# 2noise/ChatTTS

Measured on NVIDIA H100. Metric: speech-tokens/sec (GPT decode loop, 4-codebook tokens; RTF = wall / audio seconds @ 24 kHz), higher is better.
Workload: dtype f32

## Files before the change

chattts_b200/_lib.py:

```python
from __future__ import annotations

import ctypes as C
import os
import threading

from . import build as _build

_lock = threading.Lock()
_lib = None


class GptConfig(C.Structure):
    _fields_ = [(n, C.c_int32) for n in (
        "hidden_size", "intermediate_size", "num_layers", "num_heads", "num_kv_heads", "head_dim", "num_vq",
        "num_audio_tokens", "num_text_tokens", "max_positions")] + [
        ("rms_eps", C.c_float), ("max_batch", C.c_int32), ("max_context", C.c_int32)]


class GptLayout(C.Structure):
    _fields_ = [(n, C.c_int64) for n in (
        "layer0", "layer_stride", "wqkv", "wo", "wgate_up", "wdown", "ln1", "ln2", "final_norm", "head_code",
        "head_text", "emb_code", "emb_text", "rope_cos", "rope_sin", "total")]


class SamplerConfig(C.Structure):
    _fields_ = [
        ("temperature", C.c_float * 8), ("top_p", C.c_float), ("top_k", C.c_int32),
        ("min_tokens_to_keep", C.c_int32), ("penalty_on", C.c_int32), ("penalty_lut", C.c_float * 32),
        ("past_window", C.c_int32), ("penalty_max_ids", C.c_int32), ("greedy", C.c_int32),
        ("eos_token", C.c_int32), ("min_new_token", C.c_int32), ("top_p_removed_max", C.c_float),
        ("has_removed_max", C.c_int32), ("philox_seed", C.c_uint64)]


class GptStatus(C.Structure):
    _fields_ = [("steps_done", C.c_int32), ("all_finished", C.c_int32),
                ("any_finished_first_step", C.c_int32), ("reserved", C.c_int32)]


ENGINE_FP16_WEIGHTS, ENGINE_FP16_KV = 1, 2


def engine_flags(dtype) -> int:
    import torch

    if dtype is None or dtype == torch.float32:
        return 0
    if dtype == torch.float16:
        return ENGINE_FP16_WEIGHTS | ENGINE_FP16_KV
    raise ValueError(f"slot engine dtype must be torch.float32 or torch.float16, not {dtype!r}")


PREFILL_CHUNK_ALIGN = 128


SLOT_IDLE, SLOT_RUNNING, SLOT_FINISHED = 0, 1, 2

ERR_POOL = -5
PAGE_TOKENS = 16


class SlotImage(C.Structure):
    _fields_ = [("magic", C.c_uint32)] + [(n, C.c_int32) for n in (
        "prec", "seq_len", "pos", "end_idx", "finish", "n_gen", "npages", "page_bytes", "num_vq", "hidden_size",
        "noise_floats", "has_hidden")] + [
        ("row", C.c_int32 * 8), ("reserved", C.c_int32 * 3), ("sampler", SamplerConfig)] + [
        (n, C.c_uint64) for n in ("off_noise", "off_ids", "off_hiddens", "off_kv", "bytes")]


class ConvStackConfig(C.Structure):
    _fields_ = [(n, C.c_int32) for n in (
        "idim", "odim", "hidden", "n_layer", "bn_dim", "kernel", "dilation", "out_dim", "vq_dim", "vq_groups",
        "vq_residual", "vq_levels")]


class VocosConfig(C.Structure):
    _fields_ = [(n, C.c_int32) for n in ("input_channels", "dim", "intermediate_dim", "num_layers", "n_fft",
                                         "hop_length")]


EXPORTS = (
    "ctb_abi_version", "ctb_last_error", "ctb_launch_count", "ctb_gpt_layout_query", "ctb_gpt_create",
    "ctb_gpt_destroy", "ctb_gpt_begin", "ctb_gpt_decode", "ctb_gpt_status_query", "ctb_gpt_profile_kernel", "ctb_gpt_debug_trace", "ctb_gpt_embed_prompt", "ctb_sample",
    "ctb_gpt_engine_begin", "ctb_gpt_engine_admit", "ctb_gpt_engine_admit_text", "ctb_gpt_engine_status",
    "ctb_gpt_engine_cancel", "ctb_gpt_engine_begin_ex", "ctb_gpt_engine_prefill_chunk",
    "ctb_gpt_engine_begin_paged", "ctb_gpt_engine_reserve", "ctb_gpt_engine_release", "ctb_gpt_engine_suspend_bytes",
    "ctb_gpt_engine_suspend", "ctb_gpt_engine_resume", "ctb_gpt_engine_share_prompt",
    "ctb_dvae_blob_floats", "ctb_vocos_blob_floats", "ctb_decoder_create", "ctb_decoder_destroy",
    "ctb_dvae_decode", "ctb_vocos_decode", "ctb_decode_rows",
    "ctb_dvae_encoder_blob_floats", "ctb_dvae_encoder_create", "ctb_dvae_encoder_destroy", "ctb_dvae_encode",
    "ctb_dvae_encode_rows",
)


class CtbError(RuntimeError):
    pass


def lib_path() -> str:
    return _build.LIB_PATH


def load(build_if_missing: bool = True):
    global _lib
    with _lock:
        if _lib is not None:
            return _lib
        path = lib_path()
        if build_if_missing:
            try:
                _build.build()
            except Exception:
                if not os.path.exists(path):
                    raise
        if not os.path.exists(path):
            raise CtbError(f"{path} missing: run `python -m chattts_b200.build`")
        lib = C.CDLL(path)
        vp, i32, i64 = C.c_void_p, C.c_int32, C.c_int64
        lib.ctb_abi_version.restype = C.c_int
        lib.ctb_last_error.restype = C.c_char_p
        lib.ctb_launch_count.restype = C.c_uint64
        lib.ctb_gpt_layout_query.argtypes = [C.POINTER(GptConfig), C.POINTER(GptLayout)]
        lib.ctb_gpt_create.argtypes = [C.POINTER(GptConfig), vp, C.POINTER(vp)]
        lib.ctb_gpt_destroy.argtypes = [vp]
        lib.ctb_gpt_begin.argtypes = [vp, i32, i32, vp, vp, C.POINTER(SamplerConfig), vp, i32, i32, vp, vp, vp]
        lib.ctb_gpt_decode.argtypes = [vp, i32, vp]
        lib.ctb_gpt_status_query.argtypes = [vp, C.POINTER(GptStatus), vp, vp, vp]
        lib.ctb_gpt_profile_kernel.argtypes = [vp, i32, vp]
        lib.ctb_gpt_debug_trace.argtypes = [vp, vp, i32]
        lib.ctb_gpt_embed_prompt.argtypes = [vp, vp, vp, i32, i32, vp, vp]
        lib.ctb_gpt_engine_begin.argtypes = [vp, i32, i32, vp, vp, vp]
        lib.ctb_gpt_engine_begin_ex.argtypes = [vp, i32, i32, i32, vp, vp, vp]
        lib.ctb_gpt_engine_admit.argtypes = [vp, i32, vp, i32, vp, vp, C.POINTER(SamplerConfig), vp, vp, vp]
        lib.ctb_gpt_engine_admit_text.argtypes = lib.ctb_gpt_engine_admit.argtypes
        lib.ctb_gpt_engine_status.argtypes = [vp, C.POINTER(GptStatus), vp, vp, vp, vp]
        lib.ctb_gpt_engine_cancel.argtypes = [vp, i32, vp, vp]
        lib.ctb_gpt_engine_prefill_chunk.argtypes = [vp, i32, i32, i32, i32, vp, i32, C.POINTER(SamplerConfig), vp, i32,
                                                     vp]
        lib.ctb_gpt_engine_begin_paged.argtypes = [vp, i32, i32, i32, i32, vp, vp, vp]
        lib.ctb_gpt_engine_reserve.argtypes = [vp, i32, vp, vp, vp]
        lib.ctb_gpt_engine_release.argtypes = [vp, i32, vp, vp]
        lib.ctb_gpt_engine_suspend_bytes.argtypes = [vp, i32, C.POINTER(C.c_uint64), vp]
        lib.ctb_gpt_engine_suspend.argtypes = [vp, i32, vp, C.c_uint64, vp]
        lib.ctb_gpt_engine_resume.argtypes = [vp, i32, vp, C.c_uint64, vp]
        lib.ctb_gpt_engine_share_prompt.argtypes = [vp, i32, i32, i32, i32, vp]
        lib.ctb_sample.argtypes = [vp, i32, i32, i32, C.POINTER(SamplerConfig), vp, vp, i32, i32, i32, vp, vp]
        lib.ctb_dvae_blob_floats.argtypes = [C.POINTER(ConvStackConfig)]
        lib.ctb_dvae_blob_floats.restype = i64
        lib.ctb_vocos_blob_floats.argtypes = [C.POINTER(VocosConfig)]
        lib.ctb_vocos_blob_floats.restype = i64
        lib.ctb_decoder_create.argtypes = [C.POINTER(ConvStackConfig), vp, C.POINTER(VocosConfig), vp, i32, i32,
                                           C.POINTER(vp)]
        lib.ctb_decoder_destroy.argtypes = [vp]
        lib.ctb_dvae_decode.argtypes = [vp, vp, i32, i32, i32, vp, vp]
        lib.ctb_vocos_decode.argtypes = [vp, vp, i32, i32, vp, vp]
        lib.ctb_decode_rows.argtypes = [vp, i32, i32, C.POINTER(vp), C.POINTER(i32), vp, i64, vp]
        lib.ctb_dvae_encoder_blob_floats.argtypes = [C.POINTER(ConvStackConfig)]
        lib.ctb_dvae_encoder_blob_floats.restype = i64
        lib.ctb_dvae_encoder_create.argtypes = [C.POINTER(ConvStackConfig), vp, i64, C.POINTER(vp)]
        lib.ctb_dvae_encoder_destroy.argtypes = [vp]
        lib.ctb_dvae_encode.argtypes = [vp, vp, i64, vp, i32, C.POINTER(i32), vp, vp, vp]
        lib.ctb_dvae_encode_rows.argtypes = [vp, i32, C.POINTER(vp), C.POINTER(i64), vp, i32, C.POINTER(i32), vp, vp]
        if lib.ctb_abi_version() != 3:
            raise CtbError("ABI version mismatch")
        _lib = lib
        return lib


def check(rc: int) -> None:
    if rc != 0:
        raise CtbError(f"chattts_b200 error {rc}: {load().ctb_last_error().decode()}")


def require_cuda():
    import torch

    if not torch.cuda.is_available():
        raise CtbError("chattts_b200 needs a CUDA device (sm_90a); there is no CPU path")
```

chattts_b200/csrc/flow.cuh:

```cuda
#pragma once
#include "gpt_kernels.cuh"
#include "tc_common.cuh"

namespace ctb {

constexpr int FL_THREADS = 256;
constexpr int FL_LAUNCH_THREADS = FL_THREADS;
constexpr int FL_WARPS = 8;
constexpr int FL_SLOTS = 4;
constexpr int FL_SLOT_BYTES = 6144;
constexpr int FL_SLOT_FLOATS = FL_SLOT_BYTES / 4;
constexpr int FL_RING_BYTES = FL_WARPS * FL_SLOTS * FL_SLOT_BYTES;
constexpr int FL_SMAX = 6;
constexpr int FL_CH = 64;
constexpr int FL_PW = 66;
constexpr int FL_BMAX = 4;
constexpr int FL_ROWS = 6;
constexpr int FL_GU = 3;
constexpr int FL_QR = 2;
constexpr int FL_HEADS = 12;
constexpr int FL_RMAX = 16;

constexpr int FL_A_X = 0;
constexpr int FL_A_XO = FL_A_X + FL_BMAX * KC;
constexpr int FL_A_ACT = FL_A_XO + FL_BMAX * KC;
constexpr int FL_A_P = FL_A_ACT + FL_BMAX * 4 * KC;
constexpr int FL_A_END = FL_A_P + FL_BMAX * FL_HEADS * FL_SMAX * FL_PW;
constexpr int FL_REP_STRIDE = ((FL_A_END + 1023) / 1024) * 1024;
constexpr int FL_A_Q = 0, FL_A_KN = FL_BMAX * KC, FL_A_VN = 2 * FL_BMAX * KC;
constexpr int FL_QKV_WORDS = 3 * FL_BMAX * KC;
constexpr int FL_SROWS = 16, FL_VPAD = 1024;
constexpr int FL_A_LOGITS = FL_QKV_WORDS, FL_A_IDX = FL_A_LOGITS + FL_SROWS * FL_VPAD;
constexpr int FL_TAIL_WORDS = FL_A_IDX + 64;
constexpr size_t FL_PARITY_WORDS = (size_t)FL_RMAX * FL_REP_STRIDE + FL_TAIL_WORDS;
constexpr size_t FL_ARENA_WORDS = 2 * FL_PARITY_WORDS;
constexpr unsigned FL_EPOCH_STEP = 256;
constexpr int FL_TR_EV = 4096, FL_TR_EVN = 32, FL_TR_WORDS = FL_TR_EV + 192 * FL_TR_EVN;

enum FlowTagKind { FT_X = 0, FT_QKV = 1, FT_P = 2, FT_XO = 3, FT_ACT = 4, FT_LOGITS = 5, FT_IDX = 6 };
enum FlowStage { FS_Q0 = 0, FS_Q1 = 1, FS_KV = 2, FS_O = 3, FS_GU0 = 4, FS_GU1 = 5, FS_GU2 = 6, FS_D0 = 7, FS_D1 = 8, FS_NLAYER = 9 };

__device__ __forceinline__ void fl_bar() { asm volatile("bar.sync 1, 256;" ::: "memory"); }

struct FlowP {
  const float* W;
  int64_t layer0, layer_stride, o_wqkv, o_wo, o_wgu, o_wd, o_ln1, o_ln2, o_final_norm, o_head, o_emb_code, o_emb_text,
      o_cos, o_sin;
  int L, I, Hq, hd;
  float eps, scaling;
  float *logits, *kv;
  size_t kv_layer_floats;
  const int* block_table; int pages_per_row;
  int* seq_len;
  LoopState* st;
  int decode, col, T0, sample;
  const float* emb; const uint8_t* mask; const int32_t* ids_out;
  int max_new, num_vq, num_audio, infer_text, B;
  float* hidden_out; int hidden_stride, rows_per_item, V;
  unsigned long long* arena;
  unsigned* epoch;
  int R;
  int l2_ahead;
  unsigned long long* trace;
  int nsteps;
  int ink;
  ctb_sampler_config samp;
  const float* q_noise;
  uint8_t* finish;
  int* end_idx;
  int32_t* ids_w;
};

__device__ __forceinline__ void ll_st(unsigned long long* p, float v, uint32_t tag) {
  const unsigned long long x = ((unsigned long long)tag << 32) | (unsigned long long)__float_as_uint(v);
  asm volatile("st.relaxed.gpu.global.u64 [%0], %1;" ::"l"(p), "l"(x) : "memory");
}
__device__ __forceinline__ unsigned long long ll_ld(const unsigned long long* p) {
  unsigned long long x;
  asm volatile("ld.global.cg.u64 %0, [%1];" : "=l"(x) : "l"(p) : "memory");
  return x;
}
__device__ __forceinline__ void ll_ld2(const unsigned long long* p, unsigned long long& a, unsigned long long& b) {
  asm volatile("ld.global.cg.v2.u64 {%0,%1}, [%2];" : "=l"(a), "=l"(b) : "l"(p) : "memory");
}
__device__ __forceinline__ uint32_t ll_tag(unsigned long long x) { return (uint32_t)(x >> 32); }
__device__ __forceinline__ float ll_val(unsigned long long x) { return __uint_as_float((uint32_t)x); }

struct FlowWd {
  int* err;
  int dead;
  int spins;
};
__device__ __forceinline__ bool fl_giveup(FlowWd& wd, int code) {
  if (wd.dead) return true;
  if (++wd.spins < (1 << 20)) {
    if ((wd.spins & 8191) == 0 && __ldcg(wd.err) != 0) { wd.dead = 1; return true; }
    return false;
  }
  atomicCAS(wd.err, 0, code);
  wd.dead = 1;
  return true;
}

__device__ __forceinline__ void fl_bulk(uint32_t dst, const void* src, uint32_t bytes, uint32_t bar, uint64_t pol) {
  asm volatile(
      "cp.async.bulk.shared::cluster.global.mbarrier::complete_tx::bytes.L2::cache_hint [%0], [%1], %2, [%3], %4;" ::"r"(dst),
      "l"(src), "r"(bytes), "r"(bar), "l"(pol)
      : "memory");
}
__device__ __forceinline__ bool fl_elect() {
  uint32_t pred;
  asm volatile("{\n\t.reg .pred p;\n\telect.sync _|p, 0xffffffff;\n\tselp.u32 %0, 1, 0, p;\n\t}" : "=r"(pred));
  return pred != 0;
}
__device__ __forceinline__ void fl_expect(uint32_t bar, uint32_t bytes) {
  asm volatile("mbarrier.arrive.expect_tx.shared::cta.b64 _, [%0], %1;" ::"r"(bar), "r"(bytes) : "memory");
}
__device__ __forceinline__ bool fl_try_wait(uint32_t bar, uint32_t parity) {
  uint32_t ok;
  asm volatile("{\n\t.reg .pred p;\n\tmbarrier.try_wait.parity.shared::cta.b64 p, [%1], %2;\n\tselp.u32 %0, 1, 0, p;\n\t}"
               : "=r"(ok) : "r"(bar), "r"(parity) : "memory");
  return ok != 0;
}

struct FlowGeo {
  int G, NW, gw, cta, warp, lane;
  int S;
  int u_on, u_b, u_h, u_split, u_n, u_nchunk;
  int nheads_tasks;
};

__device__ __forceinline__ bool fl_q_valid(const FlowGeo& g, int j) { return g.gw + j * g.NW < 3 * KC / 2; }
__device__ __forceinline__ bool fl_kv_more(const FlowGeo& g, int sub, int& chunk) {
  chunk = g.u_split + sub * g.S;
  return g.u_on && chunk < g.u_nchunk;
}
__device__ __forceinline__ bool fl_kv_valid(const FlowGeo& g, int chunk) { return FL_CH * chunk + 8 * g.warp < g.u_n; }
__device__ __forceinline__ bool fl_o_valid(const FlowGeo& g) { return g.warp < FL_ROWS && g.cta + g.G * g.warp < KC; }
__device__ __forceinline__ bool fl_gu_valid(const FlowGeo& g, int j, int I) { return g.gw + j * g.NW < I; }
__device__ __forceinline__ int fl_d_rows(const FlowGeo& g, int j0, int j1) {
  int n = 0;
  for (int j = j0; j < j1; ++j) n += (g.cta + g.G * j < KC);
  return n;
}
__device__ __forceinline__ bool fl_h_valid(const FlowGeo& g, int j) { return g.gw + j * g.NW < g.nheads_tasks; }

__device__ __forceinline__ void fl_qkv_rows(const FlowP& p, int task, int& r0, int& r1) {
  const int half = p.hd / 2, nq = p.Hq * half;
  int t = task, base = 0;
  if (t >= 2 * nq) { t -= 2 * nq; base = 2 * p.Hq * p.hd; }
  else if (t >= nq) { t -= nq; base = p.Hq * p.hd; }
  r0 = base + (t / half) * p.hd + (t % half);
  r1 = r0 + half;
}

constexpr int FL_TMAX = 40;
struct FlowIss {
  int l, k, n, ntab, hsub;
};

__device__ __noinline__ int fl_build_table(const FlowP& p, const FlowGeo* gs, int4* tab) {
  FlowGeo g = *gs;
  g.warp = threadIdx.x >> 5; g.lane = threadIdx.x & 31; g.gw = g.cta * FL_WARPS + g.warp;
  int n = 0;
  auto put = [&](int64_t off0, int64_t stride, int bytes, int ncopy, int kind) {
    if (g.lane == 0 && n < FL_TMAX) tab[n] = make_int4((int)off0, (int)stride, bytes | (ncopy << 16) | (kind << 20), 0);
    n++;
  };
  for (int j = 0; j < FL_QR; ++j)
    if (fl_q_valid(g, j)) {
      int r0, r1;
      fl_qkv_rows(p, g.gw + j * g.NW, r0, r1);
      put(p.o_wqkv + (int64_t)r0 * KC, (int64_t)(r1 - r0) * KC, KC * 4, 2, 0);
    }
  for (int sub = 0;; ++sub) {
    int chunk;
    if (!fl_kv_more(g, sub, chunk)) break;
    if (!fl_kv_valid(g, chunk)) continue;
    const int t0 = FL_CH * chunk + 8 * g.warp;
    const int page = __ldg(p.block_table + g.u_b * p.pages_per_row + t0 / kPageTokens);
    const int64_t k0 = (int64_t)kv_off(page, 0, g.u_h, t0 % kPageTokens, p.Hq, p.hd);
    const int64_t v0 = (int64_t)kv_off(page, 1, g.u_h, t0 % kPageTokens, p.Hq, p.hd);
    put(k0, v0 - k0, 8 * 64 * 4, 2, 1);
  }
  if (fl_o_valid(g)) put(p.o_wo + (int64_t)(g.cta + g.G * g.warp) * KC, 0, KC * 4, 1, 0);
  for (int j = 0; j < FL_GU; ++j)
    if (fl_gu_valid(g, j, p.I)) put(p.o_wgu + (int64_t)(g.gw + j * g.NW) * KC, (int64_t)p.I * KC, KC * 4, 2, 0);
  for (int half = 0; half < 2; ++half) {
    const int j0 = half ? 4 : 0, j1 = half ? FL_ROWS : 4;
    const int nr = fl_d_rows(g, j0, j1);
    if (nr > 0)
      put(p.o_wd + (int64_t)(g.cta + g.G * j0) * p.I + g.warp * (p.I / FL_WARPS), (int64_t)g.G * p.I, (p.I / FL_WARPS) * 4, nr, 0);
  }
  return n;
}

__device__ __forceinline__ void fl_issue_heads(const FlowP& p, const FlowGeo* gs, int w, int hsub, uint32_t dst, uint32_t bar, uint64_t pol_w) {
  const int gw = gs->cta * FL_WARPS + w;
  const int t = gw + hsub * gs->NW, nrows = p.rows_per_item * p.V;
  if (fl_elect()) {
    fl_expect(bar, 2u * KC * 4u);
    fl_bulk(dst, p.W + p.o_head + (size_t)(2 * t) * KC, KC * 4, bar, pol_w);
    fl_bulk(dst + KC * 4, p.W + p.o_head + (size_t)min(2 * t + 1, nrows - 1) * KC, KC * 4, bar, pol_w);
  }
}

__device__ __forceinline__ bool fl_issue(const FlowP& p, const FlowGeo* gs, const int4* tab, FlowIss& it, int w, uint32_t ring,
                                         uint32_t bars, uint64_t pol_w, uint64_t pol_kv) {
  const int slot = it.n % FL_SLOTS;
  const uint32_t bar = bars + slot * 8, dst = ring + slot * FL_SLOT_BYTES;
  if (it.l < p.L) {
    const int4 e = tab[it.k];
    if (fl_elect()) {
      const int bytes = e.z & 0xffff, ncopy = (e.z >> 16) & 0xf, kind = e.z >> 20;
      const float* src = (kind ? p.kv + (size_t)it.l * p.kv_layer_floats : p.W + p.layer0 + (int64_t)it.l * p.layer_stride) + e.x;
      fl_expect(bar, (uint32_t)(bytes * ncopy));
#pragma unroll
      for (int k = 0; k < 4; ++k)
        if (k < ncopy) fl_bulk(dst + k * bytes, src + (int64_t)k * e.y, (uint32_t)bytes, bar, kind ? pol_kv : pol_w);
      if (p.l2_ahead && kind == 0) {
        const float* nsrc = it.l + 1 < p.L ? src + p.layer_stride : src - (int64_t)(p.L - 1) * p.layer_stride;
#pragma unroll
        for (int k = 0; k < 4; ++k)
          if (k < ncopy)
            asm volatile("cp.async.bulk.prefetch.L2.global [%0], %1;" ::"l"(nsrc + (int64_t)k * e.y), "r"((uint32_t)bytes) : "memory");
      }
    }
    if (++it.k == it.ntab) { it.k = 0; it.l++; }
    it.n++;
    return true;
  }
  if (gs->cta * FL_WARPS + w + it.hsub * gs->NW < gs->nheads_tasks) {
    fl_issue_heads(p, gs, w, it.hsub, dst, bar, pol_w);
    it.hsub++;
    it.n++;
    return true;
  }
  return false;
}

struct FlowW {
  float* base;
  uint32_t ring;
  uint32_t bars;
  int n;
  int owed;
  FlowIss it;
  const int4* tab;
  const FlowGeo* gs;
  uint64_t pol_w, pol_kv;
};
__device__ __forceinline__ void fl_refill(const FlowP& p, FlowW& w) {
  if (w.owed > 0) {
    __syncwarp();
    fl_issue(p, w.gs, w.tab, w.it, (int)(threadIdx.x >> 5), w.ring, w.bars, w.pol_w, w.pol_kv);
    w.owed--;
  }
}
__device__ __forceinline__ const float* fl_ring_slot_at(const FlowW& w, int k) { return w.base + ((w.n + k) % FL_SLOTS) * FL_SLOT_FLOATS; }
__device__ __forceinline__ bool fl_ring_peek_n(const FlowP& p, FlowW& w, int cnt) {
  while (w.owed > FL_SLOTS - cnt) fl_refill(p, w);
  bool ok = true;
#pragma unroll
  for (int k = 0; k < 3; ++k)
    if (k < cnt) { const int n = w.n + k; ok = fl_try_wait(w.bars + (n % FL_SLOTS) * 8, (uint32_t)(n / FL_SLOTS) & 1u) && ok; }
  return ok;
}
__device__ __forceinline__ void fl_ring_wait_n(const FlowP& p, FlowW& w, int cnt, FlowWd& wd) {
  while (w.owed > FL_SLOTS - cnt) fl_refill(p, w);
  uint32_t bar[3], par[3];
#pragma unroll
  for (int k = 0; k < 3; ++k) {
    const int n = w.n + k;
    bar[k] = w.bars + (n % FL_SLOTS) * 8;
    par[k] = (uint32_t)(n / FL_SLOTS) & 1u;
  }
  wd.spins = 0;
  while (true) {
    bool ok[3];
#pragma unroll
    for (int k = 0; k < 3; ++k) ok[k] = k < cnt ? fl_try_wait(bar[k], par[k]) : true;
    if (ok[0] && ok[1] && ok[2]) break;
    if (__any_sync(0xffffffffu, fl_giveup(wd, 0x120))) { wd.dead = 1; break; }
  }
}
__device__ __forceinline__ const float* fl_ring_wait(const FlowP& p, FlowW& w, FlowWd& wd) {
  fl_ring_wait_n(p, w, 1, wd);
  return fl_ring_slot_at(w, 0);
}
__device__ __forceinline__ void fl_ring_release(const FlowP& p, FlowW& w) { w.n++; w.owed++; fl_refill(p, w); }
__device__ __forceinline__ void fl_refill_all(const FlowP& p, FlowW& w) {
  while (w.owed > 0) fl_refill(p, w);
}

template <int BT>
__device__ __forceinline__ void fl_stage768(const FlowP& p, const unsigned long long* src, uint32_t tag, float* xs, FlowWd& wd, FlowW& fw) {
  const int tid = threadIdx.x;
  unsigned long long v[BT][3];
  wd.spins = 0;
  while (true) {
    bool ok = true;
#pragma unroll
    for (int b = 0; b < BT; ++b)
      if (b < p.B) {
#pragma unroll
        for (int k = 0; k < 3; ++k) v[b][k] = ll_ld(src + b * KC + tid + 256 * k);
      }
#pragma unroll
    for (int b = 0; b < BT; ++b)
      if (b < p.B) {
#pragma unroll
        for (int k = 0; k < 3; ++k) ok = ok && (ll_tag(v[b][k]) == tag);
      }
    if (__all_sync(0xffffffffu, ok)) break;
    if (__any_sync(0xffffffffu, fl_giveup(wd, 0x200 + (tag & 0xff)))) { wd.dead = 1; break; }
  }
#pragma unroll
  for (int b = 0; b < BT; ++b) {
#pragma unroll
    for (int k = 0; k < 3; ++k) xs[b * KC + tid + 256 * k] = b < p.B ? ll_val(v[b][k]) : 0.f;
  }
  fl_bar();
}

template <int BT>
__device__ __forceinline__ void fl_stage_attn(const FlowP& p, const unsigned long long* P, uint32_t tag, float* xs, FlowWd& wd, int S,
                                              const int* s_pos, const int* s_active) {
  const int tid = threadIdx.x, lane = tid & 31, warp = tid >> 5;
  const int pk = lane / FL_SMAX, ps = lane % FL_SMAX, pbase = min(pk, 2) * FL_SMAX;
#pragma unroll 1
  for (int b = 0; b < BT; ++b) {
    if (b >= p.B) break;
    float v[3] = {0.f, 0.f, 0.f};
    if (s_active[b]) {
      const int ns = min((s_pos[b] + FL_CH) / FL_CH, S);
      const unsigned long long* Pb = P + (size_t)b * FL_HEADS * FL_SMAX * FL_PW + (size_t)(warp >> 1) * FL_SMAX * FL_PW;
      const bool pl = pk < 3 && ps < ns;
      float m = -INFINITY, lv = 0.f;
      wd.spins = 0;
      while (true) {
        bool ok = true;
        if (pl) {
          unsigned long long w1, w2;
          ll_ld2(Pb + (size_t)(4 * pk * FL_SMAX + ps) * FL_PW + 64, w1, w2);
          ok = ll_tag(w1) == tag && ll_tag(w2) == tag;
          m = ll_val(w1); lv = ll_val(w2);
        }
        if (__all_sync(0xffffffffu, ok)) break;
        if (__any_sync(0xffffffffu, fl_giveup(wd, 0x400))) { wd.dead = 1; break; }
      }
      float GM = -INFINITY;
#pragma unroll
      for (int s = 0; s < FL_SMAX; ++s) {
        const float ms = __shfl_sync(0xffffffffu, m, pbase + s);
        if (s < ns) GM = fmaxf(GM, ms);
      }
      const float wgt = pl ? expf(m - GM) : 0.f;
      unsigned long long w[3][FL_SMAX];
      while (true) {
        bool ok = true;
#pragma unroll
        for (int k = 0; k < 3; ++k)
#pragma unroll
          for (int s = 0; s < FL_SMAX; ++s)
            if (s < ns) w[k][s] = ll_ld(Pb + (size_t)(4 * k * FL_SMAX + s) * FL_PW + (tid & 63));
#pragma unroll
        for (int k = 0; k < 3; ++k)
#pragma unroll
          for (int s = 0; s < FL_SMAX; ++s)
            if (s < ns) ok = ok && ll_tag(w[k][s]) == tag;
        if (__all_sync(0xffffffffu, ok)) break;
        if (__any_sync(0xffffffffu, fl_giveup(wd, 0x401))) { wd.dead = 1; break; }
      }
#pragma unroll
      for (int k = 0; k < 3; ++k) {
        float GL = 0.f, GO = 0.f;
#pragma unroll
        for (int s = 0; s < FL_SMAX; ++s) {
          const float ws = __shfl_sync(0xffffffffu, wgt, k * FL_SMAX + s);
          const float ls = __shfl_sync(0xffffffffu, lv, k * FL_SMAX + s);
          if (s < ns) {
            GL = fmaf(ws, ls, GL);
            GO = fmaf(ws, ll_val(w[k][s]), GO);
          }
        }
        v[k] = GO / GL;
      }
    }
#pragma unroll
    for (int k = 0; k < 3; ++k) xs[b * KC + tid + 256 * k] = v[k];
  }
#pragma unroll
  for (int b = 0; b < BT; ++b)
    if (b >= p.B)
      for (int k = 0; k < 3; ++k) xs[b * KC + tid + 256 * k] = 0.f;
  fl_bar();
}

template <int BT>
__device__ __forceinline__ void fl_load_x(const float* xs, float (&x)[BT][24], int lane) {
#pragma unroll
  for (int b = 0; b < BT; ++b) {
#pragma unroll
    for (int i = 0; i < 6; ++i) {
      const float4 v = reinterpret_cast<const float4*>(xs)[b * (KC / 4) + i * 32 + lane];
      x[b][4 * i] = v.x; x[b][4 * i + 1] = v.y; x[b][4 * i + 2] = v.z; x[b][4 * i + 3] = v.w;
    }
  }
}

template <int BT>
__device__ __forceinline__ void fl_norm(float (&x)[BT][24], const float4 (&nw)[6], float eps) {
#pragma unroll
  for (int b = 0; b < BT; ++b) {
    float s4[4] = {0.f, 0.f, 0.f, 0.f};
#pragma unroll
    for (int j = 0; j < 24; ++j) s4[j & 3] = fmaf(x[b][j], x[b][j], s4[j & 3]);
    float ss = warp_sum((s4[0] + s4[1]) + (s4[2] + s4[3]));
    const float rinv = __fdiv_rn(1.0f, __fsqrt_rn(__fadd_rn(__fdiv_rn(ss, (float)KC), eps)));
#pragma unroll
    for (int i = 0; i < 6; ++i) {
      x[b][4 * i] = __fmul_rn(nw[i].x, __fmul_rn(x[b][4 * i], rinv));
      x[b][4 * i + 1] = __fmul_rn(nw[i].y, __fmul_rn(x[b][4 * i + 1], rinv));
      x[b][4 * i + 2] = __fmul_rn(nw[i].z, __fmul_rn(x[b][4 * i + 2], rinv));
      x[b][4 * i + 3] = __fmul_rn(nw[i].w, __fmul_rn(x[b][4 * i + 3], rinv));
    }
  }
}
__device__ __forceinline__ void fl_nw_fetch(float* dst, const float* src, uint64_t* bar, uint64_t pol) {
  if (threadIdx.x == 0) {
    fl_expect(smem_u32(bar), KC * 4);
    fl_bulk(smem_u32(dst), src, KC * 4, smem_u32(bar), pol);
  }
}
__device__ __forceinline__ void fl_nw_wait(uint64_t* bar, int& count, FlowWd& wd) {
  const uint32_t b = smem_u32(bar), parity = (uint32_t)count & 1u;
  wd.spins = 0;
  while (!fl_try_wait(b, parity))
    if (__any_sync(0xffffffffu, fl_giveup(wd, 0x800))) { wd.dead = 1; break; }
  count++;
}
__device__ __forceinline__ void fl_load_nw_s(const float* s_nw, float4 (&nw)[6], int lane) {
#pragma unroll
  for (int i = 0; i < 6; ++i) nw[i] = reinterpret_cast<const float4*>(s_nw)[i * 32 + lane];
}
__device__ __forceinline__ void fl_load_nw(const float* normw, float4 (&nw)[6], int lane) {
#pragma unroll
  for (int i = 0; i < 6; ++i) nw[i] = ldg_stream(reinterpret_cast<const float4*>(normw) + i * 32 + lane);
}

template <int BT>
__device__ __forceinline__ void fl_dot2(const float* slot, const float (&x)[BT][24], float (&a0)[BT], float (&a1)[BT], int lane) {
  const float4* w0 = reinterpret_cast<const float4*>(slot) + lane;
  const float4* w1 = w0 + KC / 4;
#pragma unroll
  for (int b = 0; b < BT; ++b) { a0[b] = 0.f; a1[b] = 0.f; }
#pragma unroll
  for (int i = 0; i < 6; ++i) {
    const float4 u = w0[i * 32], v = w1[i * 32];
#pragma unroll
    for (int b = 0; b < BT; ++b) {
      a0[b] = fmaf(u.x, x[b][4 * i], a0[b]); a0[b] = fmaf(u.y, x[b][4 * i + 1], a0[b]);
      a0[b] = fmaf(u.z, x[b][4 * i + 2], a0[b]); a0[b] = fmaf(u.w, x[b][4 * i + 3], a0[b]);
      a1[b] = fmaf(v.x, x[b][4 * i], a1[b]); a1[b] = fmaf(v.y, x[b][4 * i + 1], a1[b]);
      a1[b] = fmaf(v.z, x[b][4 * i + 2], a1[b]); a1[b] = fmaf(v.w, x[b][4 * i + 3], a1[b]);
    }
  }
}
template <int BT>
__device__ __forceinline__ void fl_dot1(const float* slot, const float (&x)[BT][24], float (&a0)[BT], int lane) {
  const float4* w0 = reinterpret_cast<const float4*>(slot) + lane;
#pragma unroll
  for (int b = 0; b < BT; ++b) a0[b] = 0.f;
#pragma unroll
  for (int i = 0; i < 6; ++i) {
    const float4 u = w0[i * 32];
#pragma unroll
    for (int b = 0; b < BT; ++b) {
      a0[b] = fmaf(u.x, x[b][4 * i], a0[b]); a0[b] = fmaf(u.y, x[b][4 * i + 1], a0[b]);
      a0[b] = fmaf(u.z, x[b][4 * i + 2], a0[b]); a0[b] = fmaf(u.w, x[b][4 * i + 3], a0[b]);
    }
  }
}

template <int BT>
__device__ __forceinline__ void fl_bcast_store(unsigned long long* rep0, int R, size_t idx, float v, uint32_t tag, int nb, int lane) {
  constexpr int LPB = 32 / BT;
  const float vb = __shfl_sync(0xffffffffu, v, (lane / LPB) * LPB);
  if (lane / LPB < nb)
    for (int r = lane % LPB; r < R; r += LPB) ll_st(rep0 + (size_t)r * FL_REP_STRIDE + idx, vb, tag);
}

struct __align__(16) FlowSamp {
  float x[FL_VPAD];
  uint32_t key[2][1024];
  double redd[32];
  double pre[32];
  int redi[8];
  float redf[8];
  float bv[8];
  int bi[8];
  int win[32];
  uint32_t thr;
  int out;
};
__device__ __forceinline__ double fl_vsum_d(const double (&v)[4], double* redd) {
  const int lane = threadIdx.x & 31, warp = threadIdx.x >> 5;
  double r[4];
#pragma unroll
  for (int k = 0; k < 4; ++k) r[k] = warp_sum_d(v[k]);
  fl_bar();
  if (lane == 0) {
#pragma unroll
    for (int k = 0; k < 4; ++k) redd[warp + 8 * k] = r[k];
  }
  fl_bar();
  double t = 0.0;
#pragma unroll 8
  for (int w = 0; w < 32; ++w) t += redd[w];
  return t;
}
__device__ __forceinline__ float fl_bmax(float v, float* redf) {
  const int lane = threadIdx.x & 31, warp = threadIdx.x >> 5;
  v = warp_max(v);
  fl_bar();
  if (lane == 0) redf[warp] = v;
  fl_bar();
  float t = -INFINITY;
#pragma unroll
  for (int w = 0; w < FL_WARPS; ++w) t = fmaxf(t, redf[w]);
  return t;
}
__device__ __forceinline__ int fl_bsum_i(int v, int* redi) {
  const int lane = threadIdx.x & 31, warp = threadIdx.x >> 5;
  v = __reduce_add_sync(0xffffffffu, v);
  fl_bar();
  if (lane == 0) redi[warp] = v;
  fl_bar();
  int t = 0;
#pragma unroll
  for (int w = 0; w < FL_WARPS; ++w) t += redi[w];
  return t;
}
__device__ __forceinline__ void fl_cx(uint32_t& a, uint32_t& b, bool up) {
  const uint32_t lo = min(a, b), hi = max(a, b);
  a = up ? lo : hi; b = up ? hi : lo;
}
__device__ __forceinline__ void fl_bitonic1024(uint32_t (&key)[4], uint32_t* buf0, uint32_t* buf1) {
  const int tid = threadIdx.x;
  int sb = 0;
#pragma unroll 1
  for (int k = 2; k <= 1024; k <<= 1) {
#pragma unroll 1
    for (int j = k >> 1; j > 0; j >>= 1) {
      if (j == 1) {
        fl_cx(key[0], key[1], ((4 * tid) & k) == 0);
        fl_cx(key[2], key[3], ((4 * tid + 2) & k) == 0);
      } else if (j == 2) {
        fl_cx(key[0], key[2], ((4 * tid) & k) == 0);
        fl_cx(key[1], key[3], ((4 * tid + 1) & k) == 0);
      } else {
        const int d = j >> 2;
        uint32_t other[4];
        if (d >= 32) {
          uint32_t* buf = sb ? buf1 : buf0;
          *reinterpret_cast<uint4*>(buf + 4 * tid) = make_uint4(key[0], key[1], key[2], key[3]);
          fl_bar();
          const uint4 o = *reinterpret_cast<const uint4*>(buf + 4 * (tid ^ d));
          other[0] = o.x; other[1] = o.y; other[2] = o.z; other[3] = o.w;
          sb ^= 1;
        } else {
#pragma unroll
          for (int e = 0; e < 4; ++e) other[e] = __shfl_xor_sync(0xffffffffu, key[e], d);
        }
        const bool up = ((4 * tid) & k) == 0, lower = (tid & d) == 0;
#pragma unroll
        for (int e = 0; e < 4; ++e) key[e] = (lower == up) ? min(key[e], other[e]) : max(key[e], other[e]);
      }
    }
  }
}

__device__ __noinline__ int fl_sample_row(const ctb_sampler_config& c, const float* q_noise, FlowSamp& sm, int V, int row, int qi,
                                          int nwin, int step, unsigned long long* dbg) {
  int dk = 0;
#define FL_SK() do { if (dbg && threadIdx.x == 0) dbg[dk++] = (unsigned long long)clock64(); } while (0)
  FL_SK();
  const int tid = threadIdx.x, lane = tid & 31, warp = tid >> 5;
  const bool pen = c.penalty_on && row < c.penalty_max_ids;
  const float temp = c.temperature[qi];
  float qn[4];
#pragma unroll
  for (int k = 0; k < 4; ++k) {
    const int v = tid + 256 * k;
    qn[k] = (q_noise != nullptr && v < V) ? __ldg(q_noise + (size_t)row * V + v) : 1.f;
  }
  {
    float xr[4];
    int cnt[4] = {0, 0, 0, 0};
#pragma unroll
    for (int k = 0; k < 4; ++k) { const int v = tid + 256 * k; xr[k] = v < V ? __fdiv_rn(sm.x[v], temp) : 0.f; }
    if (pen) {
#pragma unroll 4
      for (int w = 0; w < nwin; ++w) {
        const int id = sm.win[w];
#pragma unroll
        for (int k = 0; k < 4; ++k) cnt[k] += (id == tid + 256 * k);
      }
    }
    fl_bar();
#pragma unroll
    for (int k = 0; k < 4; ++k) {
      const int v = tid + 256 * k;
      if (v < V) {
        float x = xr[k];
        if (pen) { const float a = c.penalty_lut[cnt[k]]; x = (x < 0.f) ? __fmul_rn(x, a) : __fdiv_rn(x, a); }
        sm.x[v] = x;
      }
    }
  }
  fl_bar();
  float mx = -INFINITY;
  for (int v = tid; v < V; v += FL_THREADS) mx = fmaxf(mx, sm.x[v]);
  mx = fl_bmax(mx, sm.redf);
  FL_SK();

  const bool use_p = c.top_p >= 0.f;
  const int kk = c.top_k > 0 ? min(max(c.top_k, c.min_tokens_to_keep), V) : 0;
  const int min_keep = min(c.min_tokens_to_keep, V);
  uint32_t thr_key = 0;
  if (!c.greedy && (use_p || kk > 0)) {
    double den = 0.0;
    if (use_p) {
      double dv[4];
#pragma unroll
      for (int k = 0; k < 4; ++k) { const int vt = tid + 256 * k; dv[k] = vt < V ? (double)expf(sm.x[vt] - mx) : 0.0; }
      den = fl_vsum_d(dv, sm.redd);
    }
    FL_SK();
    const float denf = (float)den;
    const float pthr = c.has_removed_max ? c.top_p_removed_max : (float)(1.0 - (double)c.top_p);
    uint32_t key[4];
#pragma unroll
    for (int k = 0; k < 4; ++k) { const int vt = tid + 256 * k; key[k] = vt < V ? float_key(sm.x[vt]) : 0u; }
    fl_bitonic1024(key, sm.key[0], sm.key[1]);
    FL_SK();
    fl_bar();
    uint32_t* skey = sm.key[0];
    *reinterpret_cast<uint4*>(skey + 4 * tid) = make_uint4(key[0], key[1], key[2], key[3]);
    fl_bar();
#pragma unroll
    for (int k = 0; k < 4; ++k) key[k] = skey[tid + 256 * k];
    uint32_t t_p = 0;
    if (use_p) {
      double inc[4];
#pragma unroll
      for (int k = 0; k < 4; ++k) {
        const uint32_t ky = key[k];
        double a = ky ? (double)__fdiv_rn(expf(key_float(ky) - mx), denf) : 0.0;
#pragma unroll
        for (int o = 1; o < 32; o <<= 1) {
          const double n = __shfl_up_sync(0xffffffffu, a, o);
          if (lane >= o) a += n;
        }
        inc[k] = a;
      }
      fl_bar();
      if (lane == 31) {
#pragma unroll
        for (int k = 0; k < 4; ++k) sm.redd[warp + 8 * k] = inc[k];
      }
      fl_bar();
      if (tid == 0) {
        double run = 0.0;
        for (int w = 0; w < 32; ++w) { const double t = sm.redd[w]; sm.pre[w] = run; run += t; }
      }
      fl_bar();
      int removed = 0;
#pragma unroll
      for (int k = 0; k < 4; ++k) {
        const int vw = warp + 8 * k, vt = tid + 256 * k;
        const double base = sm.pre[vw];
        const float cum = (float)(base + inc[k]);
        removed += ((cum <= pthr) && (vt < 1024 - min_keep)) ? 1 : 0;
      }
      const int nrem = fl_bsum_i(removed, sm.redi);
      t_p = skey[nrem];
      FL_SK();
    }
    const uint32_t t_k = kk > 0 ? skey[1024 - kk] : 0u;
    thr_key = max(t_p, t_k);
  }
  if (c.greedy) {
    float gm = -INFINITY;
    for (int v = tid; v < V; v += FL_THREADS)
      if (!(c.greedy == 2 && v == c.eos_token)) gm = fmaxf(gm, sm.x[v]);
    gm = fl_bmax(gm, sm.redf);
    thr_key = float_key(gm);
  }
  fl_bar();
  const bool ban = step < c.min_new_token;
  float mx2 = -INFINITY;
  for (int v = tid; v < V; v += FL_THREADS) {
    float x = sm.x[v];
    if (float_key(x) < thr_key || ((ban || c.greedy == 2) && v == c.eos_token)) x = -INFINITY;
    sm.x[v] = x;
    mx2 = fmaxf(mx2, x);
  }
  mx2 = fl_bmax(mx2, sm.redf);
  double dv2[4];
#pragma unroll
  for (int k = 0; k < 4; ++k) { const int vt = tid + 256 * k; dv2[k] = vt < V ? (double)expf(sm.x[vt] - mx2) : 0.0; }
  const float den2f = (float)fl_vsum_d(dv2, sm.redd);
  FL_SK();
  float best = -1.f;
  int besti = 0x7fffffff;
#pragma unroll
  for (int k = 0; k < 4; ++k) {
    const int v = tid + 256 * k;
    if (v < V) {
      const float pr = __fdiv_rn(expf(sm.x[v] - mx2), den2f);
      const float qv = q_noise ? qn[k] : philox_exp1(c.philox_seed, (uint32_t)row, (uint32_t)v, (uint32_t)step);
      const float r = __fdiv_rn(pr, qv);
      if (r > best) { best = r; besti = v; }
    }
  }
  for (int o = 16; o > 0; o >>= 1) {
    const float ob = __shfl_xor_sync(0xffffffffu, best, o);
    const int oi = __shfl_xor_sync(0xffffffffu, besti, o);
    if (ob > best || (ob == best && oi < besti)) { best = ob; besti = oi; }
  }
  fl_bar();
  if (lane == 0) { sm.bv[warp] = best; sm.bi[warp] = besti; }
  fl_bar();
  if (tid == 0) {
    for (int w = 1; w < FL_WARPS; ++w)
      if (sm.bv[w] > best || (sm.bv[w] == best && sm.bi[w] < besti)) { best = sm.bv[w]; besti = sm.bi[w]; }
    sm.out = besti < V ? besti : 0;
  }
  fl_bar();
  FL_SK();
#undef FL_SK
  return sm.out;
}

template <int BT>
__global__ void __launch_bounds__(FL_THREADS, 1) k_flow(const __grid_constant__ FlowP p) {
  extern __shared__ __align__(128) unsigned char fl_smem[];
  float* xs = reinterpret_cast<float*>(fl_smem + FL_RING_BYTES);
  __shared__ __align__(8) uint64_t s_bar[FL_WARPS * FL_SLOTS];
  __shared__ __align__(8) uint64_t s_nwbar[2];
  __shared__ int s_pos[BT], s_active[BT], s_page[BT];
  __shared__ float s_cos[BT * 64], s_sin[BT * 64];
  __shared__ float s_red[FL_ROWS][FL_WARPS][BT];
  __shared__ float s_resd[FL_ROWS * BT];
  __shared__ float s_am[FL_WARPS], s_al[FL_WARPS];
  __shared__ __align__(16) float s_ao[FL_WARPS][64];
  __shared__ FlowGeo s_geo;
  __shared__ __align__(16) float s_nw1[KC], s_nw2[KC];
  __shared__ int4 s_tab[FL_WARPS][FL_TMAX];
  __shared__ FlowSamp s_samp_store[BT <= 2 ? 1 : 0 + (BT > 2)];
  FlowSamp& s_samp = s_samp_store[0];

  const int tid = threadIdx.x, lane = tid & 31, warp = tid >> 5;
  constexpr int LPB = 32 / BT;
  if (tid < FL_WARPS * FL_SLOTS) mbar_init(&s_bar[tid], 1);
  if (tid < 2) mbar_init(&s_nwbar[tid], 1);
  asm volatile("fence.mbarrier_init.release.cluster;" ::: "memory");
  __syncthreads();
  pdl_trigger();
  pdl_wait();
  if (p.decode && ldg_cg(&p.st->all_finished)) return;

  constexpr bool INK = BT <= 2;
  __shared__ int s_ids[BT * 8];
  __shared__ int s_fin[BT], s_end[BT];
  __shared__ int s_allfin;
  FlowWd wd{&p.st->err, 0, 0};
  uint32_t base = (uint32_t)ldg_cg(reinterpret_cast<const int*>(p.epoch));
  int tr = 0;
#define FL_TRACE() do { if (p.trace && blockIdx.x == 0 && tid == 0 && tr < 250) p.trace[tr++] = globaltimer_ns(); } while (0)
#define FL_EV(k) do { if (p.trace && l == 10 && tid == 0) p.trace[FL_TR_EV + blockIdx.x * FL_TR_EVN + (k)] = globaltimer_ns(); } while (0)
#define FL_CK(k) do { if (p.trace && l == 10 && tid == 0 && blockIdx.x == 0) p.trace[3000 + (k)] = (unsigned long long)clock64(); } while (0)

  int ngen = p.decode ? ldg_cg(&p.st->n_gen) : 0;
  int lstep = p.decode ? ldg_cg(&p.st->step) : 0;
  if (tid < BT) {
    int act = 0, pos = 0;
    if (tid < p.B) {
      pos = ldg_cg(&p.seq_len[tid]);
      act = p.decode ? 1 : (p.mask[(size_t)tid * p.T0 + p.col] != 0);
    }
    s_pos[tid] = pos; s_active[tid] = act;
    s_fin[tid] = (tid < p.B && p.ink) ? (int)p.finish[tid] : 0;
    s_end[tid] = (tid < p.B && p.ink) ? ldg_cg(&p.end_idx[tid]) : 0;
  }
  const bool ink = INK && p.ink != 0;
  const int nrows_s = p.B * p.rows_per_item;
  const int R = p.R;
  uint64_t pol_w, pol_kv;
  asm volatile("createpolicy.fractional.L2::evict_first.b64 %0, 1.0;" : "=l"(pol_w));
  asm volatile("createpolicy.fractional.L2::evict_normal.b64 %0, 1.0;" : "=l"(pol_kv));
  int nw1_cnt = 0, nw2_cnt = 0;
  FlowW fw;
  fw.base = reinterpret_cast<float*>(fl_smem) + (size_t)warp * FL_SLOTS * FL_SLOT_FLOATS;
  fw.ring = smem_u32(fw.base);
  fw.bars = smem_u32(&s_bar[warp * FL_SLOTS]);
  fw.n = 0; fw.owed = 0;
  fw.it = FlowIss{0, 0, 0, 0, 0};
  fw.tab = s_tab[warp]; fw.gs = &s_geo; fw.pol_w = pol_w; fw.pol_kv = pol_kv;
  FlowGeo g;
  g.G = gridDim.x; g.NW = g.G * FL_WARPS; g.cta = blockIdx.x; g.warp = warp; g.lane = lane; g.gw = g.cta * FL_WARPS + warp;
  g.S = max(1, min(FL_SMAX, g.G / (p.Hq * p.B)));
  g.nheads_tasks = p.sample ? (p.rows_per_item * p.V + 1) / 2 : 0;
  const int myrep = g.cta % R;
  const int o_row = g.cta + g.G * warp;
  unsigned long long* tailw = p.arena + (size_t)FL_RMAX * FL_REP_STRIDE;
  fl_bar();

  int nwin = 0;
  if constexpr (INK) {
    if (ink && g.cta < nrows_s) {
      const int item = g.cta / p.rows_per_item, qi = g.cta % p.rows_per_item;
      const bool pen = p.samp.penalty_on && g.cta < p.samp.penalty_max_ids;
      nwin = pen ? min(ngen, p.samp.past_window) : 0;
      if (tid < nwin) s_samp.win[tid] = ldg_cg(&p.ids_out[((size_t)item * p.max_new + (ngen - nwin + tid)) * p.num_vq + qi]);
    }
  }

#define FL_PREP_STEP()                                                                                                  \
  do {                                                                                                                  \
    if (tid < BT) s_page[tid] = tid < p.B ? __ldg(p.block_table + tid * p.pages_per_row + s_pos[tid] / kPageTokens) : 0; \
    {                                                                                                                   \
      const int u = g.cta;                                                                                              \
      g.u_on = 0; g.u_b = 0; g.u_h = 0; g.u_split = 0; g.u_n = 0; g.u_nchunk = 0;                                       \
      if (u < p.B * p.Hq * g.S) {                                                                                       \
        g.u_split = u % g.S; g.u_h = (u / g.S) % p.Hq; g.u_b = u / (g.S * p.Hq);                                        \
        g.u_n = s_pos[g.u_b] + 1;                                                                                       \
        g.u_nchunk = (g.u_n + FL_CH - 1) / FL_CH;                                                                       \
        g.u_on = s_active[g.u_b] && g.u_split < min(g.u_nchunk, g.S);                                                   \
      }                                                                                                                 \
    }                                                                                                                   \
    if (tid == 0) s_geo = g;                                                                                            \
    fl_bar();                                                                                                           \
    fw.it.l = 0; fw.it.k = 0; fw.it.hsub = 0; fw.owed = 0;                                                              \
    fw.it.ntab = fl_build_table(p, &s_geo, s_tab[warp]);                                                                \
    __syncwarp();                                                                                                       \
    for (int k_ = 0; k_ < FL_SLOTS; ++k_) fl_issue(p, fw.gs, fw.tab, fw.it, warp, fw.ring, fw.bars, pol_w, pol_kv);     \
    for (int i = tid; i < BT * 64; i += FL_THREADS) {                                                                   \
      const int b = i / 64;                                                                                             \
      s_cos[i] = b < p.B ? __ldg(p.W + p.o_cos + (size_t)s_pos[b] * 64 + (i % 64)) : 0.f;                               \
      s_sin[i] = b < p.B ? __ldg(p.W + p.o_sin + (size_t)s_pos[b] * 64 + (i % 64)) : 0.f;                               \
    }                                                                                                                   \
  } while (0)

  FL_PREP_STEP();
  FL_TRACE();
#pragma unroll 1
  for (int sidx = 0;; ++sidx) {
  FL_TRACE();
  fl_nw_fetch(s_nw1, p.W + p.layer0 + p.o_ln1, &s_nwbar[0], pol_w);
  fl_nw_fetch(s_nw2, p.W + p.layer0 + p.o_ln2, &s_nwbar[1], pol_w);
  {
    float ev[BT * 3][8];
#pragma unroll
    for (int it_ = 0; it_ < BT * 3; ++it_) {
      const int i = tid + it_ * FL_THREADS, b = i / KC, k = i % KC;
#pragma unroll
      for (int q = 0; q < 8; ++q) ev[it_][q] = 0.f;
      if (b < p.B) {
        if (!p.decode) {
          ev[it_][0] = s_active[b] ? p.emb[((size_t)b * p.T0 + p.col) * KC + k] : 0.f;
        } else if (p.infer_text) {
          const int id0 = ldg_cg(p.ids_out + ((size_t)b * p.max_new + (ngen - 1)) * p.num_vq);
          ev[it_][0] = p.W[p.o_emb_text + (size_t)id0 * KC + k];
        } else {
#pragma unroll
          for (int q = 0; q < 8; ++q)
            if (q < p.num_vq) {
              const int id = sidx > 0 ? s_ids[b * 8 + q] : ldg_cg(p.ids_out + ((size_t)b * p.max_new + (ngen - 1)) * p.num_vq + q);
              ev[it_][q] = p.W[p.o_emb_code + ((size_t)q * p.num_audio + id) * KC + k];
            }
        }
      }
    }
#pragma unroll
    for (int it_ = 0; it_ < BT * 3; ++it_) {
      float v = 0.f;
#pragma unroll
      for (int q = 0; q < 8; ++q) v += ev[it_][q];
      xs[tid + it_ * FL_THREADS] = v;
    }
  }
  fl_bar();
  FL_TRACE();

  for (int l = 0; l < p.L; ++l) {
    const float* Wl = p.W + p.layer0 + (int64_t)l * p.layer_stride;
    unsigned long long* par = p.arena + (size_t)(l & 1) * FL_PARITY_WORDS;
    unsigned long long* parn = p.arena + (size_t)((l + 1) & 1) * FL_PARITY_WORDS;
    unsigned long long* qkvw = par + (size_t)FL_RMAX * FL_REP_STRIDE;
    const unsigned long long* myr = par + (size_t)myrep * FL_REP_STRIDE;
    const uint32_t tagl = base + 8u * (uint32_t)l;

    {
      float4 nw[6];
      FL_EV(0);
      fl_nw_wait(&s_nwbar[0], nw1_cnt, wd);
      const bool q_rdy = fl_ring_peek_n(p, fw, 1);
      if (l > 0) fl_stage768<BT>(p, myr + FL_A_X, tagl + FT_X, xs, wd, fw);
      else fl_bar();
      FL_EV(1);
      fl_refill_all(p, fw);
      fl_load_nw_s(s_nw1, nw, lane);
      float x[BT][24];
      fl_load_x<BT>(xs, x, lane);
      float res_o = 0.f;
      if (fl_o_valid(g)) res_o = xs[(lane / LPB) * KC + o_row];
      fl_norm<BT>(x, nw, p.eps);
      float res_keep = res_o;
#pragma unroll 1
      for (int j = 0; j < FL_QR; ++j) {
        if (!fl_q_valid(g, j)) continue;
        if (!(j == 0 && q_rdy)) fl_ring_wait_n(p, fw, 1, wd);
        const float* slot = fl_ring_slot_at(fw, 0);
        FL_EV(2);
        float a0[BT], a1[BT];
        fl_dot2<BT>(slot, x, a0, a1, lane);
        warp_reduce_scatter<BT>(a0);
        warp_reduce_scatter<BT>(a1);
        const int b = lane / LPB;
        if ((lane % LPB) == 0 && b < p.B && s_active[b]) {
          const int half = p.hd / 2, nq = p.Hq * half;
          int t = g.gw + j * g.NW, which = 0;
          if (t >= 2 * nq) { which = 2; t -= 2 * nq; }
          else if (t >= nq) { which = 1; t -= nq; }
          const int h = t / half, jj = t % half;
          const float v0 = a0[0], v1 = a1[0];
          float o0 = v0, o1 = v1;
          if (which < 2) {
            const float* cs = s_cos + b * 64;
            const float* sn = s_sin + b * 64;
            o0 = __fadd_rn(__fmul_rn(v0, cs[jj]), __fmul_rn(-v1, sn[jj]));
            o1 = __fadd_rn(__fmul_rn(v1, cs[jj + half]), __fmul_rn(v0, sn[jj + half]));
          }
          unsigned long long* dst = qkvw + (which == 0 ? FL_A_Q : which == 1 ? FL_A_KN : FL_A_VN) + b * KC + h * 64;
          ll_st(dst + jj, o0, tagl + FT_QKV);
          ll_st(dst + jj + half, o1, tagl + FT_QKV);
          if (which > 0) {
            float* kd = p.kv + (size_t)l * p.kv_layer_floats + kv_off(s_page[b], which - 1, h, s_pos[b] % kPageTokens, p.Hq, p.hd);
            kd[jj] = o0; kd[jj + half] = o1;
          }
        }
        fl_ring_release(p, fw);
      }
      FL_TRACE();
      FL_EV(3);

      if (g.u_on) {
        const int sub = lane & 7, grp = lane >> 3;
        const int b = g.u_b, h = g.u_h, n = g.u_n, pos = n - 1;
        float q[8];
        float M = -INFINITY, L = 0.f, O = 0.f;
        int pend_kv = 0;
        for (int sb = 0;; ++sb) {
          int chunk;
          if (!fl_kv_more(g, sb, chunk)) break;
          const bool have = fl_kv_valid(g, chunk);
          const float* slot = have ? fl_ring_wait(p, fw, wd) : nullptr;
          const int tbase = chunk * FL_CH + warp * 8 + grp;
          float4 k0[2], k1[2], v0[2], v1[2];
#pragma unroll
          for (int i = 0; i < 2; ++i) {
            const int t = tbase + 4 * i;
            k0[i] = k1[i] = v0[i] = v1[i] = make_float4(0.f, 0.f, 0.f, 0.f);
            if (have && t < pos) {
              const float* kr = slot + (grp + 4 * i) * 64 + sub * 8;
              const float* vr = kr + 8 * 64;
              k0[i] = *reinterpret_cast<const float4*>(kr); k1[i] = *reinterpret_cast<const float4*>(kr + 4);
              v0[i] = *reinterpret_cast<const float4*>(vr); v1[i] = *reinterpret_cast<const float4*>(vr + 4);
            }
          }
          if (sb == 0) {
            const unsigned long long* qp = qkvw + FL_A_Q + b * KC + h * 64 + sub * 8;
            unsigned long long w[8];
            wd.spins = 0;
            while (true) {
              bool ok = true;
#pragma unroll
              for (int k = 0; k < 4; ++k) ll_ld2(qp + 2 * k, w[2 * k], w[2 * k + 1]);
#pragma unroll
              for (int k = 0; k < 8; ++k) ok = ok && (ll_tag(w[k]) == tagl + FT_QKV);
              if (__all_sync(0xffffffffu, ok)) break;
              if (__any_sync(0xffffffffu, fl_giveup(wd, 0x300))) { wd.dead = 1; break; }
            }
#pragma unroll
            for (int k = 0; k < 8; ++k) q[k] = ll_val(w[k]);
          }
          if (sb == 0) { FL_EV(4); fl_refill_all(p, fw); }
          {
            const bool mine0 = (tbase == pos), mine1 = (tbase + 4 == pos);
            if (__any_sync(0xffffffffu, mine0 || mine1)) {
              const unsigned long long* kp = qkvw + FL_A_KN + b * KC + h * 64 + sub * 8;
              const unsigned long long* vp = qkvw + FL_A_VN + b * KC + h * 64 + sub * 8;
              unsigned long long kw[8], vw[8];
              wd.spins = 0;
              while (true) {
                bool ok = true;
                if (mine0 || mine1) {
#pragma unroll
                  for (int k = 0; k < 4; ++k) { ll_ld2(kp + 2 * k, kw[2 * k], kw[2 * k + 1]); ll_ld2(vp + 2 * k, vw[2 * k], vw[2 * k + 1]); }
#pragma unroll
                  for (int k = 0; k < 8; ++k) ok = ok && (ll_tag(kw[k]) == tagl + FT_QKV) && (ll_tag(vw[k]) == tagl + FT_QKV);
                }
                if (__all_sync(0xffffffffu, ok)) break;
                if (__any_sync(0xffffffffu, fl_giveup(wd, 0x301))) { wd.dead = 1; break; }
              }
              if (mine0 || mine1) {
                const int i = mine0 ? 0 : 1;
                const float4 a = make_float4(ll_val(kw[0]), ll_val(kw[1]), ll_val(kw[2]), ll_val(kw[3]));
                const float4 bq = make_float4(ll_val(kw[4]), ll_val(kw[5]), ll_val(kw[6]), ll_val(kw[7]));
                const float4 cq = make_float4(ll_val(vw[0]), ll_val(vw[1]), ll_val(vw[2]), ll_val(vw[3]));
                const float4 dq = make_float4(ll_val(vw[4]), ll_val(vw[5]), ll_val(vw[6]), ll_val(vw[7]));
                if (i == 0) { k0[0] = a; k1[0] = bq; v0[0] = cq; v1[0] = dq; }
                else { k0[1] = a; k1[1] = bq; v0[1] = cq; v1[1] = dq; }
              }
            }
          }
          float sc[2], m = -INFINITY;
#pragma unroll
          for (int i = 0; i < 2; ++i) {
            float s = q[0] * k0[i].x + q[1] * k0[i].y + q[2] * k0[i].z + q[3] * k0[i].w + q[4] * k1[i].x + q[5] * k1[i].y +
                      q[6] * k1[i].z + q[7] * k1[i].w;
            s += __shfl_xor_sync(0xffffffffu, s, 1);
            s += __shfl_xor_sync(0xffffffffu, s, 2);
            s += __shfl_xor_sync(0xffffffffu, s, 4);
            sc[i] = (tbase + 4 * i < n) ? s * p.scaling : -INFINITY;
            m = fmaxf(m, sc[i]);
          }
          m = fmaxf(m, __shfl_xor_sync(0xffffffffu, m, 8));
          m = fmaxf(m, __shfl_xor_sync(0xffffffffu, m, 16));
          float lsum = 0.f, o[8] = {0.f, 0.f, 0.f, 0.f, 0.f, 0.f, 0.f, 0.f};
          if (m > -INFINITY) {
#pragma unroll
            for (int i = 0; i < 2; ++i) {
              const float e = expf(sc[i] - m);
              lsum += e;
              o[0] = fmaf(e, v0[i].x, o[0]); o[1] = fmaf(e, v0[i].y, o[1]); o[2] = fmaf(e, v0[i].z, o[2]);
              o[3] = fmaf(e, v0[i].w, o[3]); o[4] = fmaf(e, v1[i].x, o[4]); o[5] = fmaf(e, v1[i].y, o[5]);
              o[6] = fmaf(e, v1[i].z, o[6]); o[7] = fmaf(e, v1[i].w, o[7]);
            }
          }
          lsum += __shfl_xor_sync(0xffffffffu, lsum, 8);
          lsum += __shfl_xor_sync(0xffffffffu, lsum, 16);
#pragma unroll
          for (int j = 0; j < 8; ++j) {
            o[j] += __shfl_xor_sync(0xffffffffu, o[j], 8);
            o[j] += __shfl_xor_sync(0xffffffffu, o[j], 16);
          }
          if (have) {
            int nxt;
            if (fl_kv_more(g, sb + 1, nxt)) fl_ring_release(p, fw);
            else pend_kv = 1;
          }
          fl_bar();
          if (lane < 8) {
            *reinterpret_cast<float4*>(&s_ao[warp][lane * 8]) = make_float4(o[0], o[1], o[2], o[3]);
            *reinterpret_cast<float4*>(&s_ao[warp][lane * 8 + 4]) = make_float4(o[4], o[5], o[6], o[7]);
            if (lane == 0) { s_am[warp] = m; s_al[warp] = lsum; }
          }
          fl_bar();
          if (tid < 64) {
            float cm = M;
#pragma unroll
            for (int w = 0; w < FL_WARPS; ++w) cm = fmaxf(cm, s_am[w]);
            const float fo = (M > -INFINITY) ? expf(M - cm) : 0.f;
            L *= fo; O *= fo;
#pragma unroll
            for (int w = 0; w < FL_WARPS; ++w) {
              const float f = (s_am[w] > -INFINITY) ? expf(s_am[w] - cm) : 0.f;
              L = fmaf(f, s_al[w], L);
              O = fmaf(f, s_ao[w][tid], O);
            }
            M = cm;
          }
        }
        FL_EV(14);
        if (tid < 64) {
          unsigned long long* P = par + FL_A_P + ((size_t)(b * FL_HEADS + h) * FL_SMAX + g.u_split) * FL_PW;
          for (int r = 0; r < R; ++r) {
            unsigned long long* Pr = P + (size_t)r * FL_REP_STRIDE;
            ll_st(Pr + tid, O, tagl + FT_P);
            if (tid == 0) { ll_st(Pr + 64, M, tagl + FT_P); ll_st(Pr + 65, L, tagl + FT_P); }
          }
        }
        FL_EV(15);
        if (pend_kv) fl_ring_release(p, fw);
      }
      FL_TRACE();
      FL_EV(5);

      fl_bar();
      if (l + 1 < p.L || p.sample) fl_nw_fetch(s_nw1, l + 1 < p.L ? Wl + p.layer_stride + p.o_ln1 : p.W + p.o_final_norm, &s_nwbar[0], pol_w);
      const bool o_rdy = fl_o_valid(g) ? fl_ring_peek_n(p, fw, 1) : true;
      fl_stage_attn<BT>(p, myr + FL_A_P, tagl + FT_P, xs, wd, g.S, s_pos, s_active);
      fl_refill_all(p, fw);
      FL_EV(6);
      if (fl_o_valid(g)) {
        fl_load_x<BT>(xs, x, lane);
        if (!o_rdy) fl_ring_wait_n(p, fw, 1, wd);
        const float* slot = fl_ring_slot_at(fw, 0);
        FL_EV(7);
        float a0[BT];
        fl_dot1<BT>(slot, x, a0, lane);
        warp_reduce_scatter<BT>(a0);
        const float out = __fadd_rn(res_keep, a0[0]);
        fl_bcast_store<BT>(par, R, FL_A_XO + (size_t)(lane / LPB) * KC + o_row, out, tagl + FT_XO, p.B, lane);
        fl_ring_release(p, fw);
      }
      FL_TRACE();
      FL_EV(8);
    }

    {
      float4 nw[6];
      fl_nw_wait(&s_nwbar[1], nw2_cnt, wd);
      int ngu = 0;
#pragma unroll
      for (int j = 0; j < FL_GU; ++j) ngu += fl_gu_valid(g, j, p.I) ? 1 : 0;
      const bool gu_rdy = fl_ring_peek_n(p, fw, ngu);
      fl_bar();
      FL_CK(8);
      fl_stage768<BT>(p, myr + FL_A_XO, tagl + FT_XO, xs, wd, fw);
      fl_refill_all(p, fw);
      fl_load_nw_s(s_nw2, nw, lane);
      FL_EV(9);
      FL_CK(9);
      if (tid < FL_ROWS * BT) {
        const int b = tid % BT, j = tid / BT, row = g.cta + g.G * j;
        s_resd[tid] = row < KC ? xs[b * KC + row] : 0.f;
      }
      float x[BT][24];
      fl_load_x<BT>(xs, x, lane);
      FL_CK(10);
      fl_norm<BT>(x, nw, p.eps);
      FL_CK(11);
      {
        FL_CK(0);
        const float4* sl[FL_GU];
#pragma unroll
        for (int j = 0; j < FL_GU; ++j) sl[j] = reinterpret_cast<const float4*>(fl_ring_slot_at(fw, j)) + lane;
        if (!gu_rdy) fl_ring_wait_n(p, fw, ngu, wd);
        FL_EV(16);
        FL_CK(1);
        float acc[8 * BT];
#pragma unroll
        for (int k = 0; k < 8 * BT; ++k) acc[k] = 0.f;
#pragma unroll
        for (int i = 0; i < 6; ++i) {
#pragma unroll
          for (int j = 0; j < FL_GU; ++j)
            if (j < ngu) {
              const float4 u = sl[j][i * 32], v = sl[j][KC / 4 + i * 32];
#pragma unroll
              for (int b = 0; b < BT; ++b) {
                float& a0 = acc[(2 * j) * BT + b];
                float& a1 = acc[(2 * j + 1) * BT + b];
                a0 = fmaf(u.x, x[b][4 * i], a0); a0 = fmaf(u.y, x[b][4 * i + 1], a0);
                a0 = fmaf(u.z, x[b][4 * i + 2], a0); a0 = fmaf(u.w, x[b][4 * i + 3], a0);
                a1 = fmaf(v.x, x[b][4 * i], a1); a1 = fmaf(v.y, x[b][4 * i + 1], a1);
                a1 = fmaf(v.z, x[b][4 * i + 2], a1); a1 = fmaf(v.w, x[b][4 * i + 3], a1);
              }
            }
        }
        FL_CK(2);
        warp_reduce_scatter<8 * BT>(acc);
        FL_CK(3);
        constexpr int LPV = 32 / (8 * BT);
        const int gl = lane & 7, b = (gl / LPV) % BT, base8 = lane & ~7;
        const float gv = __shfl_sync(0xffffffffu, acc[0], base8 + b * LPV);
        const float uv = __shfl_sync(0xffffffffu, acc[0], base8 + BT * LPV + b * LPV);
        if ((lane >> 3) < ngu && b < p.B) {
          const float sg = __fdiv_rn(gv, __fadd_rn(1.0f, expf(-gv)));
          const float act = __fmul_rn(sg, uv);
          unsigned long long* d = par + FL_A_ACT + (size_t)b * p.I + (g.gw + (lane >> 3) * g.NW);
          for (int rr = (gl % LPV) + (gl >= BT * LPV ? LPV : 0); rr < R; rr += 2 * LPV) ll_st(d + (size_t)rr * FL_REP_STRIDE, act, tagl + FT_ACT);
        }
        FL_CK(5);
        for (int j = 0; j < ngu; ++j) fl_ring_release(p, fw);
        FL_CK(6);
      }
      FL_TRACE();
      FL_EV(10);
    }

    {
      float xd[BT][12];
      const int nr0_ = fl_d_rows(g, 0, 4), nr1_ = fl_d_rows(g, 4, FL_ROWS);
      const bool d_rdy = fl_ring_peek_n(p, fw, nr1_ > 0 ? 2 : 1);
      {
        const int kslice = p.I / FL_WARPS;
#pragma unroll
        for (int b = 0; b < BT; ++b) {
#pragma unroll
          for (int k = 0; k < 12; ++k) xd[b][k] = 0.f;
          if (b < p.B) {
            const unsigned long long* ap = myr + FL_A_ACT + (size_t)b * p.I + warp * kslice;
            unsigned long long w[12];
            wd.spins = 0;
            bool sentinel_ok = false;
            int it_s = 0, it_f = 0;
            if (b == 0) FL_CK(12);
            while (true) {
              ++it_s;
              ll_ld2(ap + lane * 4, w[0], w[1]);
              if (sentinel_ok || __all_sync(0xffffffffu, ll_tag(w[0]) == tagl + FT_ACT && ll_tag(w[1]) == tagl + FT_ACT)) {
                if (!sentinel_ok && b == 0) FL_CK(13);
                sentinel_ok = true;
                ++it_f;
                bool ok = ll_tag(w[0]) == tagl + FT_ACT && ll_tag(w[1]) == tagl + FT_ACT;
                ll_ld2(ap + lane * 4 + 2, w[2], w[3]);
#pragma unroll
                for (int i = 1; i < 3; ++i) {
                  ll_ld2(ap + (i * 32 + lane) * 4, w[4 * i], w[4 * i + 1]);
                  ll_ld2(ap + (i * 32 + lane) * 4 + 2, w[4 * i + 2], w[4 * i + 3]);
                }
#pragma unroll
                for (int k = 2; k < 12; ++k) ok = ok && (ll_tag(w[k]) == tagl + FT_ACT);
                if (__all_sync(0xffffffffu, ok)) break;
              }
              if (__any_sync(0xffffffffu, fl_giveup(wd, 0x500))) { wd.dead = 1; break; }
            }
            if (b == 0) { FL_CK(14); if (p.trace && l == 10 && tid == 0 && blockIdx.x == 0) { p.trace[3015] = it_s; p.trace[3016] = it_f; } }
#pragma unroll
            for (int k = 0; k < 12; ++k) xd[b][k] = ll_val(w[k]);
          }
        }
      }
      FL_EV(11);
      fl_refill_all(p, fw);
      int e_tasks = 0;
      {
        const int nr0 = nr0_, nr1 = nr1_;
        const float* s0 = fl_ring_slot_at(fw, 0);
        const float* s1 = nr1 > 0 ? fl_ring_slot_at(fw, 1) : s0;
        if (!d_rdy) fl_ring_wait_n(p, fw, nr1 > 0 ? 2 : 1, wd);
        FL_EV(17);
        float acc[8 * BT];
#pragma unroll
        for (int k = 0; k < 8 * BT; ++k) acc[k] = 0.f;
#pragma unroll
        for (int i = 0; i < 3; ++i) {
#pragma unroll
          for (int k = 0; k < FL_ROWS; ++k) {
            const bool valid = k < 4 ? (k < nr0) : (k - 4 < nr1);
            if (valid) {
              const float4 u = (reinterpret_cast<const float4*>((k < 4 ? s0 : s1) + (k & 3) * (3072 / FL_WARPS)) + lane)[i * 32];
#pragma unroll
              for (int b = 0; b < BT; ++b) {
                float& a = acc[k * BT + b];
                a = fmaf(u.x, xd[b][4 * i], a); a = fmaf(u.y, xd[b][4 * i + 1], a);
                a = fmaf(u.z, xd[b][4 * i + 2], a); a = fmaf(u.w, xd[b][4 * i + 3], a);
              }
            }
          }
        }
        warp_reduce_scatter<8 * BT>(acc);
        constexpr int LPV = 32 / (8 * BT);
        const int vi = lane / LPV, k = vi / BT, b = vi % BT;
        if ((lane % LPV) == 0 && k < FL_ROWS) s_red[k][warp][b] = acc[0];
        e_tasks = nr1 > 0 ? 2 : 1;
      }
      FL_EV(12);
      fl_bar();
      if (l + 1 < p.L) fl_nw_fetch(s_nw2, Wl + p.layer_stride + p.o_ln2, &s_nwbar[1], pol_w);
      if (tid < FL_ROWS * BT * 8) {
        const int e = tid >> 3, b = e % BT, j = e / BT, row = g.cta + g.G * j;
        if (row < KC && b < p.B) {
          float v = s_red[j][0][b];
#pragma unroll
          for (int w = 1; w < FL_WARPS; ++w) v = __fadd_rn(v, s_red[j][w][b]);
          const float out = __fadd_rn(s_resd[e], v);
          for (int r = tid & 7; r < R; r += 8)
            ll_st(parn + (size_t)r * FL_REP_STRIDE + FL_A_X + (size_t)b * KC + row, out, tagl + 8u + FT_X);
        }
      }
      for (int k = 0; k < e_tasks; ++k) fl_ring_release(p, fw);
      FL_TRACE();
      FL_EV(13);
    }
  }

  if (p.sample) {
    const unsigned long long* myr = p.arena + (size_t)(p.L & 1) * FL_PARITY_WORDS + (size_t)myrep * FL_REP_STRIDE;
    float4 nw[6];
    fl_nw_wait(&s_nwbar[0], nw1_cnt, wd);
    fl_bar();
    fl_stage768<BT>(p, myr + FL_A_X, base + 8u * (uint32_t)p.L + FT_X, xs, wd, fw);
    fl_refill_all(p, fw);
    fl_load_nw_s(s_nw1, nw, lane);
    float x[BT][24];
    fl_load_x<BT>(xs, x, lane);
    fl_norm<BT>(x, nw, p.eps);
    if (p.hidden_out != nullptr && blockIdx.x == 0 && warp == 0) {
#pragma unroll
      for (int b = 0; b < BT; ++b)
        if (b < p.B) {
          float4* dst = reinterpret_cast<float4*>(p.hidden_out + (size_t)b * p.hidden_stride + (size_t)ngen * KC);
#pragma unroll
          for (int i = 0; i < 6; ++i) dst[i * 32 + lane] = make_float4(x[b][4 * i], x[b][4 * i + 1], x[b][4 * i + 2], x[b][4 * i + 3]);
        }
    }
    const int nrows = p.rows_per_item * p.V;
    const uint32_t tagh = base + 8u * (uint32_t)p.L + FT_LOGITS;
    for (int j = 0; fl_h_valid(g, j); ++j) {
      const int t = g.gw + j * g.NW;
      const float* slot = fl_ring_wait(p, fw, wd);
      float a0[BT], a1[BT];
      fl_dot2<BT>(slot, x, a0, a1, lane);
      warp_reduce_scatter<BT>(a0);
      warp_reduce_scatter<BT>(a1);
      const int b = lane / LPB;
      if ((lane % LPB) == 0 && b < p.B) {
        const int r0 = 2 * t, q0 = r0 / p.V, c0 = r0 % p.V;
        const int q1 = (r0 + 1) / p.V, c1 = (r0 + 1) % p.V;
        if (ink) {
          ll_st(tailw + FL_A_LOGITS + (size_t)(b * p.rows_per_item + q0) * FL_VPAD + c0, a0[0], tagh);
          if (r0 + 1 < nrows) ll_st(tailw + FL_A_LOGITS + (size_t)(b * p.rows_per_item + q1) * FL_VPAD + c1, a1[0], tagh);
        } else {
          p.logits[((size_t)b * p.rows_per_item + q0) * p.V + c0] = a0[0];
          if (r0 + 1 < nrows) p.logits[((size_t)b * p.rows_per_item + q1) * p.V + c1] = a1[0];
        }
      }
      fl_ring_release(p, fw);
    }
  }
  FL_TRACE();
  fl_bar();
  if (tid < p.B && s_active[tid]) s_pos[tid]++;
  fl_bar();
  const bool more = ink && sidx + 1 < p.nsteps;
  if (more) FL_PREP_STEP();
  if constexpr (INK) {
    if (ink) {
      const uint32_t tagi = base + 8u * (uint32_t)p.L + FT_IDX;
      if (g.cta < nrows_s) {
        const int row = g.cta, qi = row % p.rows_per_item;
        const unsigned long long* lw = tailw + FL_A_LOGITS + (size_t)row * FL_VPAD;
        unsigned long long w[4];
        wd.spins = 0;
        while (true) {
          bool ok = true;
#pragma unroll
          for (int k = 0; k < 4; ++k)
            if (tid + 256 * k < p.V) { w[k] = ll_ld(lw + tid + 256 * k); ok = ok && ll_tag(w[k]) == base + 8u * (uint32_t)p.L + FT_LOGITS; }
          if (__all_sync(0xffffffffu, ok)) break;
          if (__any_sync(0xffffffffu, fl_giveup(wd, 0x600))) { wd.dead = 1; break; }
        }
#pragma unroll
        for (int k = 0; k < 4; ++k)
          if (tid + 256 * k < p.V) s_samp.x[tid + 256 * k] = ll_val(w[k]);
        fl_bar();
        const int id = fl_sample_row(p.samp, p.q_noise, s_samp, p.V, row, qi, nwin, lstep, (p.trace && row == 0) ? p.trace + 3100 : nullptr);
        if (tid == 0) {
          ll_st(tailw + FL_A_IDX + row, __int_as_float(id), tagi);
          const bool pen = p.samp.penalty_on && row < p.samp.penalty_max_ids;
          if (pen) {
            if (nwin < p.samp.past_window) s_samp.win[nwin] = id;
            else { for (int k = 0; k + 1 < nwin; ++k) s_samp.win[k] = s_samp.win[k + 1]; if (nwin > 0) s_samp.win[nwin - 1] = id; }
          }
        }
        if (p.samp.penalty_on && row < p.samp.penalty_max_ids && nwin < p.samp.past_window) nwin++;
        fl_bar();
      }
      FL_TRACE();
      if (tid < nrows_s) {
        unsigned long long w;
        wd.spins = 0;
        while (true) {
          w = ll_ld(tailw + FL_A_IDX + tid);
          if (ll_tag(w) == tagi) break;
          if (fl_giveup(wd, 0x601)) break;
        }
        s_ids[(tid / p.rows_per_item) * 8 + tid % p.rows_per_item] = __float_as_int(ll_val(w));
      }
      fl_bar();
      if (tid == 0) {
        int notall = 0;
        for (int b = 0; b < p.B; ++b) {
          bool eos = false;
          for (int q = 0; q < p.rows_per_item; ++q) eos |= (s_ids[b * 8 + q] == p.samp.eos_token);
          const int fin = s_fin[b] || eos;
          s_fin[b] = fin;
          if (!fin) { s_end[b]++; notall = 1; }
          if (blockIdx.x == 0) {
            int32_t* dst = p.ids_w + ((size_t)b * p.max_new + ngen) * p.num_vq;
            for (int q = 0; q < p.num_vq; ++q) dst[q] = s_ids[b * 8 + q];
            p.finish[b] = (uint8_t)fin;
            p.end_idx[b] = s_end[b];
          }
        }
        s_allfin = !notall;
        if (blockIdx.x == 0) {
          if (!notall) p.st->all_finished = 1;
          p.st->n_gen = ngen + 1;
          p.st->step = lstep + 1;
        }
      }
      fl_bar();
      FL_TRACE();
    }
  }
  ngen++; lstep++;
  base += FL_EPOCH_STEP;
  if (!more || s_allfin) {
    if (more) {
      const int outst = fw.it.n - fw.n;
      for (int k = 0; k < outst; ++k) {
        const int n = fw.n + k;
        wd.spins = 0;
        while (!fl_try_wait(fw.bars + (n % FL_SLOTS) * 8, (uint32_t)(n / FL_SLOTS) & 1u))
          if (__any_sync(0xffffffffu, fl_giveup(wd, 0x700))) { wd.dead = 1; break; }
      }
    }
    break;
  }
  }
  if (blockIdx.x == 0) {
    if (tid < p.B) p.seq_len[tid] = s_pos[tid];
    if (tid == 0) *p.epoch = base;
  }
#undef FL_TRACE
#undef FL_EV
#undef FL_CK
#undef FL_PREP_STEP
}

}
```

chattts_b200/csrc/gpt_api.cu:

```cuda
#include <stdarg.h>

#include <map>
#include <mutex>
#include <vector>

#include <cudaTypedefs.h>

#define CTB_GPT_KERNELS_IMPL
#include "gpt_kernels.cuh"
#include "tc_decode.cuh"
#include "mega.cuh"
#include "flow.cuh"
#include "prefill.cuh"
#include "tc_gemm.cuh"
#include "kv_pool.cuh"

namespace ctb {

thread_local char g_err[512] = {0};
std::atomic<uint64_t> g_launches{0};

int set_err(int code, const char* fmt, ...) {
  va_list ap;
  va_start(ap, fmt);
  vsnprintf(g_err, sizeof(g_err), fmt, ap);
  va_end(ap);
  return code;
}

int g_num_sms = 132;


static int bt_for(int B) {
  int bt = 1;
  while (bt < B && bt < 32) bt <<= 1;
  return bt;
}

}

using namespace ctb;
using ctb::g_num_sms;

struct ctb_gpt {
  ctb_gpt_config cfg;
  ctb_gpt_layout lay;
  const float* W;
  int pages_per_row, nsplit_max, bpad_max;
  float *x, *qbuf, *attn, *mlp, *logits, *kv, *part;
  int *block_table, *seq_len, *pos, *counter, *end_idx;
  int32_t* idx;
  uint8_t *active, *finish;
  LoopState* st;
  size_t kv_layer_elems;
  size_t kv_bytes;
  int bt_B; size_t bt_per_row;
  int B, T0, max_new, infer_text, started;
  ctb_sampler_config sampler;
  const float* q_noise;
  const float* emb;
  const uint8_t* mask;
  int32_t* ids_out;
  float* hiddens_out;
  cudaGraphExec_t graph_exec;
  uint64_t graph_kernels;
  cudaStream_t cap_stream;
  bool use_tc, tc_ready;
  int tc_min_batch;
  bool pf_enabled;
  float *gw_hi, *gw_lo;
  float *pf_resid, *pf_xn, *pf_qkv, *pf_q, *pf_attn, *pf_gu, *pf_h, *pf_ones, *pf_zeros;
  int *pf_npre, *pf_nvalid;
  uint8_t* pf_mask;
  size_t pf_rows;
  bool mega_ok;
  int mega_max_batch;
  unsigned* bar;
  unsigned long long* trace;
  bool flow_ok;
  int flow_R;
  int flow_l2_ahead;
  int flow_max_batch;
  unsigned long long* flow_arena;
  unsigned* flow_epoch;
  int steps_enqueued;
  float *tc_wqkv, *tc_wgu, *tc_heads_code, *tc_heads_text;
  float *x_hi, *x_lo, *attn_hi, *attn_lo, *h_hi, *h_lo;
  int tc_rows;
  CUtensorMap *m_wqkv, *m_wo, *m_wgu, *m_wd;
  CUtensorMap m_hcode, m_htext;
  CUtensorMap m_x[3][2], m_attn[3][2], m_h[3][2];
  bool use_graph;
  int engine;
  int phase;
  RowState* rows;
  ctb_sampler_config* cfgs;
  float* eng_noise;
  int* eng_slot;
  float* eng_text_logits;
  int32_t* eng_text_idx;
  int eng_text;
  cudaGraphExec_t graph_exec_text;
  uint64_t graph_kernels_text;
  std::vector<int> chunk_T0, chunk_done;
  std::vector<int> pr_len, pr_W;
  int prec;
  bool tc_base;
  __half *w16_qkv, *w16_wo, *w16_gu, *w16_wd;
  CUtensorMap *m16_wqkv, *m16_wo, *m16_wgu, *m16_wd;
  float* gw16;
  float* pf_wzero;
  int pg_pages;
  bool pg_poison;
  std::vector<int> pg_free;
  std::vector<int> pg_bt;
  std::vector<int> pg_map, pg_hi, pg_cap;
  std::vector<int> pg_ref;
  char* pg_stage;
};

static size_t kv_elem_bytes(const ctb_gpt* h) { return (h->prec & CTB_ENGINE_FP16_KV) ? 2 : 4; }
static float* kv_layer(const ctb_gpt* h, int l) {
  return reinterpret_cast<float*>(reinterpret_cast<char*>(h->kv) + (size_t)l * h->kv_layer_elems * kv_elem_bytes(h));
}

static size_t noise_stride(const ctb_gpt* h) {
  return std::max((size_t)h->cfg.num_vq * h->cfg.num_audio_tokens, (size_t)h->cfg.num_text_tokens);
}

static int check_private(const ctb_gpt* h, int b, int lo, int hi) {
  if (!h->pg_pages) return CTB_OK;
  for (int k = lo / kPageTokens; k * kPageTokens < hi && k < h->pg_map[b]; ++k)
    if (h->pg_ref[h->pg_bt[(size_t)b * h->pages_per_row + k]] > 1)
      return set_err(CTB_ERR_STATE, "slot %d: positions [%d,%d) reach page entry %d, which is shared", b, lo, hi, k);
  return CTB_OK;
}

extern "C" int ctb_abi_version(void) { return CTB_ABI_VERSION; }
extern "C" const char* ctb_last_error(void) { return g_err; }
extern "C" uint64_t ctb_launch_count(void) { return g_launches.load(); }

extern "C" int ctb_gpt_layout_query(const ctb_gpt_config* c, ctb_gpt_layout* o) {
  if (!c || !o) return set_err(CTB_ERR_ARG, "null argument");
  const int64_t d = c->hidden_size, I = c->intermediate_size, hd = c->head_dim;
  const int64_t nq = (int64_t)c->num_heads * hd, nkv = (int64_t)c->num_kv_heads * hd;
  int64_t off = 0;
  o->wqkv = off; off += (nq + 2 * nkv) * d;
  o->wo = off; off += d * nq;
  o->wgate_up = off; off += 2 * I * d;
  o->wdown = off; off += d * I;
  o->ln1 = off; off += d;
  o->ln2 = off; off += d;
  o->layer_stride = off;
  o->layer0 = 0;
  off = o->layer_stride * c->num_layers;
  o->final_norm = off; off += d;
  o->head_code = off; off += (int64_t)c->num_vq * c->num_audio_tokens * d;
  o->head_text = off; off += (int64_t)c->num_text_tokens * d;
  o->emb_code = off; off += (int64_t)c->num_vq * c->num_audio_tokens * d;
  o->emb_text = off; off += (int64_t)c->num_text_tokens * d;
  o->rope_cos = off; off += (int64_t)c->max_positions * hd;
  o->rope_sin = off; off += (int64_t)c->max_positions * hd;
  o->total = off;
  return CTB_OK;
}

template <typename T>
static int dalloc(T** p, size_t n) {
  CTB_CUDA(cudaMalloc(reinterpret_cast<void**>(p), n * sizeof(T)));
  CTB_CUDA(cudaMemset(*p, 0, n * sizeof(T)));
  return CTB_OK;
}

namespace ctb {
__global__ void k_build_tc_weight(const float* __restrict__ W, const float* __restrict__ scale, float* __restrict__ out,
                                  int rows, int K, int mode, int qk_rows, int hd, int I) {
  const int r = blockIdx.x;
  if (r >= rows) return;
  int pr = r;
  if (mode == 1 && r < qk_rows) {
    const int h = r / hd, j = r % hd, half = hd / 2;
    pr = h * hd + (j < half ? 2 * j : 2 * (j - half) + 1);
  } else if (mode == 2) {
    pr = (r < I) ? 2 * r : 2 * (r - I) + 1;
  }
  for (int k = threadIdx.x; k < K; k += blockDim.x)
    out[(size_t)pr * K + k] = scale ? __fmul_rn(W[(size_t)r * K + k], scale[k]) : W[(size_t)r * K + k];
}

__global__ void k_build_tc_weight16(const float* __restrict__ W, const float* __restrict__ scale, __half* __restrict__ out16,
                                    float* __restrict__ out32, int rows, int K, int mode, int qk_rows, int hd, int I,
                                    int* __restrict__ bad) {
  const int r = blockIdx.x;
  if (r >= rows) return;
  int pr = r;
  if (mode == 1 && r < qk_rows) {
    const int h = r / hd, j = r % hd, half = hd / 2;
    pr = h * hd + (j < half ? 2 * j : 2 * (j - half) + 1);
  } else if (mode == 2) {
    pr = (r < I) ? 2 * r : 2 * (r - I) + 1;
  }
  for (int k = threadIdx.x; k < K; k += blockDim.x) {
    const float v = scale ? __fmul_rn(W[(size_t)r * K + k], scale[k]) : W[(size_t)r * K + k];
    if (fabsf(v) > 65504.f) *bad = 1;
    const __half w = __float2half_rn(v);
    out16[(size_t)pr * K + k] = w;
    out32[(size_t)r * K + k] = __half2float(w);
  }
}
}

static int encode_map_2d(CUtensorMap* m, const void* base, uint64_t rows, uint64_t K, uint32_t box_rows,
                         bool f16 = false) {
  static PFN_cuTensorMapEncodeTiled_v12000 enc = nullptr;
  if (!enc) {
    void* fp = nullptr;
    cudaDriverEntryPointQueryResult q;
    if (cudaGetDriverEntryPoint("cuTensorMapEncodeTiled", &fp, cudaEnableDefault, &q) != cudaSuccess ||
        q != cudaDriverEntryPointSuccess)
      return set_err(CTB_ERR_CUDA, "cuTensorMapEncodeTiled unavailable");
    enc = reinterpret_cast<PFN_cuTensorMapEncodeTiled_v12000>(fp);
  }
  const cuuint64_t dims[2] = {K, rows};
  const cuuint64_t strides[1] = {K * (f16 ? 2 : 4)};
  const cuuint32_t box[2] = {32, box_rows};
  const cuuint32_t estr[2] = {1, 1};
  CUresult r = enc(m, f16 ? CU_TENSOR_MAP_DATA_TYPE_FLOAT16 : CU_TENSOR_MAP_DATA_TYPE_FLOAT32, 2, const_cast<void*>(base),
                   dims, strides, box, estr, CU_TENSOR_MAP_INTERLEAVE_NONE,
                   f16 ? CU_TENSOR_MAP_SWIZZLE_NONE : CU_TENSOR_MAP_SWIZZLE_128B, CU_TENSOR_MAP_L2_PROMOTION_L2_128B,
                   CU_TENSOR_MAP_FLOAT_OOB_FILL_NONE);
  if (r != CUDA_SUCCESS) return set_err(CTB_ERR_CUDA, "cuTensorMapEncodeTiled failed (%d)", (int)r);
  return CTB_OK;
}

template <int EPI, int CS, int PREC = 0>
static int set_tc_attr() {
  constexpr bool w16 = (PREC & TD_W16) != 0;
// ... 76 lines not shown
}

static void fp16_free(ctb_gpt* h) {
  void* ptrs[] = {h->w16_qkv, h->w16_wo, h->w16_gu, h->w16_wd, h->gw16, h->pf_wzero};
  for (void* p : ptrs) if (p) cudaFree(p);
  h->w16_qkv = h->w16_wo = h->w16_gu = h->w16_wd = nullptr; h->gw16 = h->pf_wzero = nullptr;
  delete[] h->m16_wqkv; delete[] h->m16_wo; delete[] h->m16_wgu; delete[] h->m16_wd;
  h->m16_wqkv = h->m16_wo = h->m16_wgu = h->m16_wd = nullptr;
}

static int fp16_setup(ctb_gpt* h) {
  if (h->w16_qkv) return CTB_OK;
  const ctb_gpt_config& c = h->cfg;
  const ctb_gpt_layout& L = h->lay;
  const size_t d = c.hidden_size, I = c.intermediate_size, nq = (size_t)c.num_heads * c.head_dim;
  const size_t nqkv = (size_t)(c.num_heads + 2 * c.num_kv_heads) * c.head_dim;
  const int nl = c.num_layers, qk_rows = (c.num_heads + c.num_kv_heads) * c.head_dim;
  int rc;
  if ((rc = tc_setup_base(h))) return rc;
  int* bad = nullptr;
  if ((rc = dalloc(&h->w16_qkv, nl * nqkv * d)) || (rc = dalloc(&h->w16_wo, nl * d * nq)) ||
      (rc = dalloc(&h->w16_gu, nl * 2 * I * d)) || (rc = dalloc(&h->w16_wd, nl * d * I)) ||
      (rc = dalloc(&h->gw16, (size_t)L.layer_stride * nl)) ||
      (rc = dalloc(&h->pf_wzero, std::max(std::max(nqkv * d, d * nq), std::max(2 * I * d, d * I)))) ||
      (rc = dalloc(&bad, (size_t)4 * nl))) {
    fp16_free(h);
    if (bad) cudaFree(bad);
    return rc;
  }
  for (int l = 0; l < nl; ++l) {
    const float* Wl = h->W + L.layer0 + (int64_t)l * L.layer_stride;
    float* gl = h->gw16 + (int64_t)l * L.layer_stride;
    k_build_tc_weight16<<<(unsigned)nqkv, 256>>>(Wl + L.wqkv, Wl + L.ln1, h->w16_qkv + l * nqkv * d, gl + L.wqkv,
                                                 (int)nqkv, (int)d, 1, qk_rows, c.head_dim, 0, bad + 4 * l);
    k_build_tc_weight16<<<(unsigned)d, 256>>>(Wl + L.wo, nullptr, h->w16_wo + l * d * nq, gl + L.wo, (int)d, (int)nq, 0,
                                              0, 0, 0, bad + 4 * l + 1);
    k_build_tc_weight16<<<(unsigned)(2 * I), 256>>>(Wl + L.wgate_up, Wl + L.ln2, h->w16_gu + l * 2 * I * d,
                                                    gl + L.wgate_up, (int)(2 * I), (int)d, 2, 0, 0, (int)I, bad + 4 * l + 2);
    k_build_tc_weight16<<<(unsigned)d, 256>>>(Wl + L.wdown, nullptr, h->w16_wd + l * d * I, gl + L.wdown, (int)d, (int)I,
                                              0, 0, 0, 0, bad + 4 * l + 3);
  }
  std::vector<int> hbad((size_t)4 * nl);
  const cudaError_t e = cudaMemcpy(hbad.data(), bad, hbad.size() * sizeof(int), cudaMemcpyDeviceToHost);
  cudaFree(bad);
  if (e != cudaSuccess) { fp16_free(h); return set_err(CTB_ERR_CUDA, "fp16 weight copies: %s", cudaGetErrorString(e)); }
  static const char* names[4] = {"self_attn.qkv (x input_layernorm)", "self_attn.o_proj",
                                 "mlp.gate_up (x post_attention_layernorm)", "mlp.down_proj"};
  for (int i = 0; i < 4 * nl; ++i)
    if (hbad[i]) {
      fp16_free(h);
      return set_err(CTB_ERR_ARG, "fp16 engine: layer %d %s has a weight with |w| > 65504 (outside fp16's range)", i / 4,
                     names[i % 4]);
    }
  h->m16_wqkv = new CUtensorMap[nl]; h->m16_wo = new CUtensorMap[nl];
  h->m16_wgu = new CUtensorMap[nl]; h->m16_wd = new CUtensorMap[nl];
  for (int l = 0; l < nl; ++l) {
    if ((rc = encode_map_2d(&h->m16_wqkv[l], h->w16_qkv + l * nqkv * d, nqkv, d, 128, true)) ||
        (rc = encode_map_2d(&h->m16_wo[l], h->w16_wo + l * d * nq, d, nq, 128, true)) ||
        (rc = encode_map_2d(&h->m16_wgu[l], h->w16_gu + l * 2 * I * d, 2 * I, d, 128, true)) ||
        (rc = encode_map_2d(&h->m16_wd[l], h->w16_wd + l * d * I, d, I, 128, true))) {
      fp16_free(h);
      return rc;
    }
  }
  if ((rc = set_tc_attr<DE_QKV, CS_QKV, 1>()) || (rc = set_tc_attr<DE_QKV, CS_QKV, 3>()) ||
      (rc = set_tc_attr<DE_OPROJ, CS_O, 1>()) || (rc = set_tc_attr<DE_GATEUP, CS_GU, 1>()))
    return rc;
  return set_tc_attr<DE_DOWN, CS_DOWN, 1>();
}

extern "C" int ctb_gpt_create(const ctb_gpt_config* c, const float* weights_dev, ctb_gpt** out) {
  if (!c || !weights_dev || !out) return set_err(CTB_ERR_ARG, "null argument");
  if (c->hidden_size != KC) return set_err(CTB_ERR_ARG, "hidden_size must be %d", KC);
  if (c->intermediate_size % KC) return set_err(CTB_ERR_ARG, "intermediate_size must be a multiple of %d", KC);
  if (c->head_dim != 64) return set_err(CTB_ERR_ARG, "head_dim must be 64");
  if (c->num_heads % c->num_kv_heads) return set_err(CTB_ERR_ARG, "num_heads %% num_kv_heads != 0");
  if (c->num_vq > 8 || c->num_vq < 1) return set_err(CTB_ERR_ARG, "num_vq out of range");
  if (c->max_batch < 1 || c->max_context < 1 || c->max_context > c->max_positions)
    return set_err(CTB_ERR_ARG, "bad max_batch/max_context");
  int dev_count = 0;
  CTB_CUDA(cudaGetDeviceCount(&dev_count));
  if (dev_count < 1) return set_err(CTB_ERR_CUDA, "no CUDA device: chattts_b200 has no CPU path");
  {
    int dev = 0, sms = 0;
    CTB_CUDA(cudaGetDevice(&dev));
    CTB_CUDA(cudaDeviceGetAttribute(&sms, cudaDevAttrMultiProcessorCount, dev));
    g_num_sms = sms;
  }
  ctb_gpt* h = new ctb_gpt();
  memset(h, 0, sizeof(*h));
  h->cfg = *c;
  ctb_gpt_layout_query(c, &h->lay);
  h->W = weights_dev;
  h->pages_per_row = (c->max_context + kPageTokens - 1) / kPageTokens;
  h->nsplit_max = (c->max_context + ATT_SPLIT_UNIT - 1) / ATT_SPLIT_UNIT;
  const int bt = bt_for(c->max_batch);
  h->bpad_max = ((c->max_batch + bt - 1) / bt) * bt;
  const size_t Bp = h->bpad_max, d = c->hidden_size;
  const size_t nq = (size_t)c->num_heads * c->head_dim;
  int rc;
#define TRY(e) if ((rc = (e)) != CTB_OK) { ctb_gpt_destroy(h); return rc; }
  TRY(dalloc(&h->x, Bp * d));
  TRY(dalloc(&h->qbuf, Bp * nq));
  TRY(dalloc(&h->attn, Bp * nq));
  TRY(dalloc(&h->mlp, Bp * c->intermediate_size));
  const size_t nlog = std::max((size_t)c->num_vq * c->num_audio_tokens, (size_t)c->num_text_tokens);
  TRY(dalloc(&h->logits, Bp * nlog));
  h->kv = nullptr; h->kv_layer_elems = 0; h->kv_bytes = 0;
  TRY(dalloc(&h->part, (size_t)c->max_batch * c->num_heads * h->nsplit_max * (c->head_dim + 2)));
  TRY(dalloc(&h->block_table, (size_t)c->max_batch * h->pages_per_row));
  TRY(dalloc(&h->seq_len, Bp));
  TRY(dalloc(&h->pos, Bp));
  TRY(dalloc(&h->counter, (size_t)c->max_batch * c->num_heads));
  TRY(dalloc(&h->end_idx, Bp));
  TRY(dalloc(&h->idx, Bp * c->num_vq));
  TRY(dalloc(&h->active, Bp));
  TRY(dalloc(&h->finish, Bp));
  TRY(dalloc(&h->st, 1));
  TRY(dalloc(&h->bar, 4));
  if (getenv("CTB_MEGA_TRACE")) TRY(dalloc(&h->trace, FL_TR_WORDS));
  h->flow_ok = getenv("CTB_NO_FLOW") == nullptr && g_num_sms >= 128 && g_num_sms <= 191 && c->intermediate_size == 4 * KC &&
               c->num_heads == c->num_kv_heads && c->num_heads * c->head_dim == KC && c->num_heads <= FL_HEADS;
  if (h->flow_ok) {
    TRY(dalloc(&h->flow_arena, FL_ARENA_WORDS));
    TRY(dalloc(&h->flow_epoch, 4));
    const unsigned e0 = FL_EPOCH_STEP;
    cudaMemcpy(h->flow_epoch, &e0, sizeof(e0), cudaMemcpyHostToDevice);
    h->flow_R = getenv("CTB_FLOW_R") ? std::max(1, std::min(FL_RMAX, atoi(getenv("CTB_FLOW_R")))) : 1;
    h->flow_l2_ahead = getenv("CTB_FLOW_L2_AHEAD") ? atoi(getenv("CTB_FLOW_L2_AHEAD")) : 0;
    h->flow_max_batch = getenv("CTB_FLOW_MAX_BATCH") ? std::max(0, std::min(FL_BMAX, atoi(getenv("CTB_FLOW_MAX_BATCH")))) : 1;
  }
#undef TRY
  h->use_graph = getenv("CTB_NO_GRAPH") == nullptr;
  h->pf_enabled = getenv("CTB_NO_BATCHED_PREFILL") == nullptr;
  h->mega_ok = getenv("CTB_NO_MEGA") == nullptr && g_num_sms >= 128 && c->intermediate_size == 4 * KC &&
               (c->hidden_size / 2 + g_num_sms - 1) / g_num_sms <= MG_DOWN_PAIRS;
  h->mega_max_batch = getenv("CTB_MEGA_MAX_BATCH") ? std::min(8, atoi(getenv("CTB_MEGA_MAX_BATCH"))) : 4;
  constexpr int kTcMinBatch = 9;
  h->tc_ready = getenv("CTB_GPT_FMA") == nullptr && c->max_batch <= 32 &&
                (getenv("CTB_GPT_TC") != nullptr || c->max_batch >= kTcMinBatch);
  h->tc_min_batch = getenv("CTB_GPT_TC") != nullptr ? 1 : kTcMinBatch;
  if (h->tc_ready && (rc = tc_setup(h)) != CTB_OK) { ctb_gpt_destroy(h); return rc; }
  *out = h;
  return CTB_OK;
}

extern "C" int ctb_gpt_destroy(ctb_gpt* h) {
  if (!h) return CTB_OK;
  if (h->graph_exec) cudaGraphExecDestroy(h->graph_exec);
  if (h->graph_exec_text) cudaGraphExecDestroy(h->graph_exec_text);
  if (h->cap_stream) cudaStreamDestroy(h->cap_stream);
  void* ptrs[] = {h->x, h->qbuf, h->attn, h->mlp, h->logits, h->kv, h->part, h->block_table, h->seq_len,
                  h->pos, h->counter, h->end_idx, h->idx, h->active, h->finish, h->st, h->tc_wqkv, h->tc_wgu,
                  h->tc_heads_code, h->tc_heads_text, h->x_hi, h->x_lo, h->attn_hi, h->attn_lo, h->h_hi, h->h_lo, h->bar, h->trace, h->flow_arena, h->flow_epoch, h->gw_hi, h->gw_lo, h->pf_resid, h->pf_xn, h->pf_qkv, h->pf_q,
                  h->pf_attn, h->pf_gu, h->pf_h, h->pf_ones, h->pf_zeros, h->pf_npre, h->pf_nvalid,
                  h->pf_mask, h->rows, h->cfgs, h->eng_noise, h->eng_slot, h->eng_text_logits, h->eng_text_idx,
                  h->pg_stage};
  delete[] h->m_wqkv; delete[] h->m_wo; delete[] h->m_wgu; delete[] h->m_wd;
  for (void* p : ptrs) if (p) cudaFree(p);
  fp16_free(h);
  delete h;
  return CTB_OK;
}

template <int BT, int EPI>
static int launch_gemv_t(const GemvP& p, int ntiles, cudaStream_t s) {
  const size_t smem = (size_t)BT * KC * sizeof(float);
  { int rc = ensure_smem_attr((const void*)k_gemv<BT, EPI>, (int)smem); if (rc) return rc; }
  int ctas = std::min(g_num_sms, (p.ntasks + GEMV_WARPS - 1) / GEMV_WARPS);
  unsigned cluster = 1;
  if (EPI == EPI_DOWN) {
    cluster = DOWN_SPLIT;
    static int max_groups = 0;
    if (!max_groups) {
      cudaLaunchConfig_t qc{};
      qc.gridDim = dim3(DOWN_SPLIT * (g_num_sms / DOWN_SPLIT)); qc.blockDim = dim3(GEMV_WARPS * 32); qc.dynamicSmemBytes = smem;
      cudaLaunchAttribute qa[1];
      qa[0].id = cudaLaunchAttributeClusterDimension;
      qa[0].val.clusterDim.x = DOWN_SPLIT; qa[0].val.clusterDim.y = 1; qa[0].val.clusterDim.z = 1;
      qc.attrs = qa; qc.numAttrs = 1;
      CTB_CUDA(cudaOccupancyMaxActiveClusters(&max_groups, k_gemv<BT, EPI>, &qc));
      if (max_groups < 1) return set_err(CTB_ERR_STATE, "DOWN kernel: no cluster of %d CTAs fits the device", DOWN_SPLIT);
    }
    const int groups = std::max(1, std::min(max_groups, (p.ntasks + GEMV_WARPS - 1) / GEMV_WARPS));
    if ((p.ntasks + groups * GEMV_WARPS - 1) / (groups * GEMV_WARPS) > DOWN_MAX_TASKS)
      return set_err(CTB_ERR_STATE, "DOWN kernel: too few SMs (%d) for %d tasks", g_num_sms, p.ntasks);
    ctas = groups * DOWN_SPLIT;
  }
  dim3 grid(ctas, ntiles);
  CTB_CUDA(launch_pdl_cluster(k_gemv<BT, EPI>, grid, dim3(GEMV_WARPS * 32), smem, s, cluster, p));
  CTB_LAUNCH_CHECK();
  return CTB_OK;
}

template <int EPI>
static int launch_gemv(int bt, const GemvP& p, int ntiles, cudaStream_t s) {
  switch (bt) {
    case 1: return launch_gemv_t<1, EPI>(p, ntiles, s);
    case 2: return launch_gemv_t<2, EPI>(p, ntiles, s);
    case 4: return launch_gemv_t<4, EPI>(p, ntiles, s);
    case 8: return launch_gemv_t<8, EPI>(p, ntiles, s);
    case 16: return launch_gemv_t<16, EPI>(p, ntiles, s);
    default: return launch_gemv_t<32, EPI>(p, ntiles, s);
  }
}

template <int BT>
static int launch_gateup_small_t(const GemvP& p, cudaStream_t s) {
  const size_t smem = ((size_t)BT * KC + GU_ZONE_FLOATS) * sizeof(float);
  { int rc = ensure_smem_attr((const void*)k_gateup_small<BT>, (int)smem); if (rc) return rc; }
  CTB_CUDA(launch_pdl(k_gateup_small<BT>, dim3(g_num_sms), dim3(GEMV_WARPS * 32), smem, s, p));
  CTB_LAUNCH_CHECK();
  return CTB_OK;
}
static int launch_gateup_small(int bt, const GemvP& p, cudaStream_t s) {
  switch (bt) {
    case 1: return launch_gateup_small_t<1>(p, s);
    case 2: return launch_gateup_small_t<2>(p, s);
    case 4: return launch_gateup_small_t<4>(p, s);
    case 8: return launch_gateup_small_t<8>(p, s);
    default: return launch_gateup_small_t<16>(p, s);
  }
}

template <int BT>
static int launch_down_small_t(const GemvP& p, cudaStream_t s) {
  const size_t smem = (size_t)BT * p.K * sizeof(float);
  { int rc = ensure_smem_attr((const void*)k_down_small<BT>, (int)smem); if (rc) return rc; }
  CTB_CUDA(launch_pdl(k_down_small<BT>, dim3(g_num_sms), dim3(GEMV_WARPS * 32), smem, s, p));
  CTB_LAUNCH_CHECK();
  return CTB_OK;
}
static int launch_down_small(int bt, const GemvP& p, cudaStream_t s) {
  switch (bt) {
    case 1: return launch_down_small_t<1>(p, s);
    case 2: return launch_down_small_t<2>(p, s);
    case 4: return launch_down_small_t<4>(p, s);
    case 8: return launch_down_small_t<8>(p, s);
    default: return launch_down_small_t<16>(p, s);
  }
}

template <bool ENGINE>
static int launch_sample_t(const SampleP& sp, cudaStream_t s) {
  const size_t smem = (size_t)sp.V * sizeof(float) + 2 * 1024 * sizeof(uint32_t);
  { int rc = ensure_smem_attr((const void*)k_sample<ENGINE>, (int)smem); if (rc) return rc; }
  CTB_CUDA(launch_pdl(k_sample<ENGINE>, dim3(sp.rows), dim3(SAMPLE_THREADS), smem, s, sp));
  CTB_LAUNCH_CHECK();
  return CTB_OK;
}
static int launch_sample(const SampleP& sp, cudaStream_t s) {
  return sp.rstate != nullptr ? launch_sample_t<true>(sp, s) : launch_sample_t<false>(sp, s);
}

struct StepCtx {
  GemvP g;
  AttnP a;
  int bt, ntiles, decode;
};

static StepCtx make_ctx(ctb_gpt* h, int decode) {
  const ctb_gpt_config& c = h->cfg;
  const ctb_gpt_layout& L = h->lay;
  StepCtx x{};
  x.decode = decode;
  x.bt = bt_for(h->B);
  x.ntiles = (h->B + x.bt - 1) / x.bt;
  GemvP& g = x.g;
  g.B = h->B; g.st = h->st; g.check_finished = decode; g.eps = c.rms_eps;
  g.block_table = h->block_table; g.pages_per_row = h->pages_per_row; g.pos = h->pos; g.active = h->active;
  g.rope_cos = h->W + L.rope_cos; g.rope_sin = h->W + L.rope_sin;
  g.Hq = c.num_heads; g.Hkv = c.num_kv_heads; g.hd = c.head_dim; g.I = c.intermediate_size; g.xres = h->x;
  AttnP& a = x.a;
  a.st = h->st; a.check_finished = decode; a.q = h->qbuf; a.block_table = h->block_table;
  a.pages_per_row = h->pages_per_row; a.pos = h->pos; a.active = h->active; a.out = h->attn; a.part = h->part;
  a.out_hi = h->use_tc ? h->attn_hi : nullptr; a.out_lo = h->use_tc ? h->attn_lo : nullptr;
  a.counter = h->counter; a.Hq = c.num_heads; a.Hkv = c.num_kv_heads; a.hd = c.head_dim;
  a.nsplit_max = h->nsplit_max; a.scaling = 1.0f / sqrtf((float)c.head_dim);
  return x;
}

static int launch_layer_kernel(ctb_gpt* h, const StepCtx& x, int l, int kind, cudaStream_t s) {
  const ctb_gpt_config& c = h->cfg;
  const ctb_gpt_layout& L = h->lay;
  const int d = c.hidden_size, I = c.intermediate_size, hd = c.head_dim;
  const float* Wl = h->W + L.layer0 + (int64_t)l * L.layer_stride;
  float* kvl = kv_layer(h, l);
  GemvP p = x.g;
  switch (kind) {
    case 0:
      p.W = Wl + L.wqkv; p.K = d; p.nrows = (c.num_heads + 2 * c.num_kv_heads) * hd; p.ntasks = p.nrows / 2;
      p.xin = h->x; p.normw = Wl + L.ln1; p.out = h->qbuf; p.kv = kvl;
      return launch_gemv<EPI_QKV>(x.bt, p, x.ntiles, s);
    case 1: {
      AttnP a = x.a;
      a.kv = kvl;
      const int max_ctx = h->engine ? c.max_context : std::min(c.max_context, h->T0 + h->max_new);
      const int want = (2 * g_num_sms + c.num_heads * h->B - 1) / (c.num_heads * h->B);
      dim3 agrid(std::max(1, std::min(want, (max_ctx + ATT_CHUNK - 1) / ATT_CHUNK)), c.num_heads, h->B);
      if (h->prec & CTB_ENGINE_FP16_KV)
        CTB_CUDA(launch_pdl(k_attn<__half>, agrid, dim3(ATT_THREADS), 0, s, a));
      else
        CTB_CUDA(launch_pdl(k_attn<float>, agrid, dim3(ATT_THREADS), 0, s, a));
      CTB_LAUNCH_CHECK();
      return CTB_OK;
    }
    case 2:
// ... 42 lines not shown
  sp.V = h->infer_text ? c.num_text_tokens : c.num_audio_tokens;
  sp.rows_per_item = rpi; sp.cfg = h->sampler; sp.q_noise = h->q_noise; sp.gen_ids = h->ids_out;
  sp.gen_stride = h->max_new; sp.gen_inner = c.num_vq; sp.out_idx = h->idx;
  if (!h->engine) return launch_sample(sp, s);
  sp.rstate = h->rows; sp.cfgs = h->cfgs; sp.want = h->phase; sp.q_noise = h->eng_noise;
  sp.noise_stride = (int)noise_stride(h);
  const int rc = launch_sample(sp, s);
  if (rc || !h->eng_text) return rc;
  sp.logits = h->eng_text_logits; sp.rows = h->B; sp.V = c.num_text_tokens; sp.rows_per_item = 1;
  sp.out_idx = h->eng_text_idx; sp.want = h->phase | WANT_TEXT;
  return launch_sample(sp, s);
}

static int tc_npad_index(int B) { return B > 32 ? 2 : (B > 16 ? 1 : 0); }

template <int EPI, int CS, int PREC = 0>
static int launch_tc(int npad, const CUtensorMap& mw, const CUtensorMap& mxh, const CUtensorMap& mxl, const TcDecP& p,
                     cudaStream_t s) {
  constexpr bool W16 = (PREC & TD_W16) != 0;
  const int tiles = (p.nrows + 127) / 128;
  dim3 grid(tiles * CS);
  if (npad == 16)
    CTB_CUDA(launch_pdl_cluster(k_tc_dec<EPI, 16, CS, PREC>, grid, dim3(TD_THREADS), (size_t)TdCfg<16, W16>::SMEM_BYTES, s, (unsigned)CS, mw, mxh, mxl, p));
  else if (npad == 32)
    CTB_CUDA(launch_pdl_cluster(k_tc_dec<EPI, 32, CS, PREC>, grid, dim3(TD_THREADS), (size_t)TdCfg<32, W16>::SMEM_BYTES, s, (unsigned)CS, mw, mxh, mxl, p));
  else
    CTB_CUDA(launch_pdl_cluster(k_tc_dec<EPI, 64, CS, PREC>, grid, dim3(TD_THREADS), (size_t)TdCfg<64, W16>::SMEM_BYTES, s, (unsigned)CS, mw, mxh, mxl, p));
  CTB_LAUNCH_CHECK();
  return CTB_OK;
}

static TcDecP make_tc(ctb_gpt* h) {
  const ctb_gpt_config& c = h->cfg;
  TcDecP p{};
  p.B = h->B; p.eps = c.rms_eps; p.d = c.hidden_size; p.xres = h->x; p.x_hi = h->x_hi; p.x_lo = h->x_lo;
  p.qbuf = h->qbuf; p.block_table = h->block_table; p.pages_per_row = h->pages_per_row; p.pos = h->pos;
  p.active = h->active; p.rope_cos = h->W + h->lay.rope_cos; p.rope_sin = h->W + h->lay.rope_sin;
  p.Hq = c.num_heads; p.Hkv = c.num_kv_heads; p.hd = c.head_dim; p.h_hi = h->h_hi; p.h_lo = h->h_lo;
  p.I = c.intermediate_size; p.st = h->st;
  return p;
}

template <int PREC>
static int launch_layer_kernel_tc_t(ctb_gpt* h, int l, int kind, cudaStream_t s) {
  constexpr int PW = PREC & TD_W16;
  const ctb_gpt_config& c = h->cfg;
  const int n = tc_npad_index(h->B), npad = 16 << n;
  const int d = c.hidden_size, I = c.intermediate_size;
  TcDecP p = make_tc(h);
  switch (kind) {
    case 0:
      p.K = d; p.kslice = d / CS_QKV; p.nrows = (c.num_heads + 2 * c.num_kv_heads) * c.head_dim; p.xraw = h->x;
      p.kv = kv_layer(h, l);
      return launch_tc<DE_QKV, CS_QKV, PREC>(npad, PW ? h->m16_wqkv[l] : h->m_wqkv[l], h->m_x[n][0], h->m_x[n][1], p, s);
    case 2:
      p.K = c.num_heads * c.head_dim; p.kslice = p.K / CS_O; p.nrows = d; p.xraw = nullptr;
      return launch_tc<DE_OPROJ, CS_O, PW>(npad, PW ? h->m16_wo[l] : h->m_wo[l], h->m_attn[n][0], h->m_attn[n][1], p, s);
    case 3:
      p.K = d; p.kslice = d / CS_GU; p.nrows = 2 * I; p.xraw = h->x;
      return launch_tc<DE_GATEUP, CS_GU, PW>(npad, PW ? h->m16_wgu[l] : h->m_wgu[l], h->m_x[n][0], h->m_x[n][1], p, s);
    case 4:
      p.K = I; p.kslice = I / CS_DOWN; p.nrows = d; p.xraw = nullptr;
      return launch_tc<DE_DOWN, CS_DOWN, PW>(npad, PW ? h->m16_wd[l] : h->m_wd[l], h->m_h[n][0], h->m_h[n][1], p, s);
  }
  return set_err(CTB_ERR_ARG, "bad tc kernel kind %d", kind);
}

static int launch_layer_kernel_tc(ctb_gpt* h, int l, int kind, cudaStream_t s) {
  switch (h->prec) {
    case 0: return launch_layer_kernel_tc_t<0>(h, l, kind, s);
    case CTB_ENGINE_FP16_WEIGHTS: return launch_layer_kernel_tc_t<CTB_ENGINE_FP16_WEIGHTS>(h, l, kind, s);
    case CTB_ENGINE_FP16_KV: return launch_layer_kernel_tc_t<CTB_ENGINE_FP16_KV>(h, l, kind, s);
    default: return launch_layer_kernel_tc_t<CTB_ENGINE_FP16_WEIGHTS | CTB_ENGINE_FP16_KV>(h, l, kind, s);
  }
}

static int launch_heads_tc(ctb_gpt* h, cudaStream_t s) {
  const ctb_gpt_config& c = h->cfg;
  const int n = tc_npad_index(h->B), npad = 16 << n;
  TcDecP p = make_tc(h);
  const int rpi = h->infer_text ? 1 : c.num_vq;
  const int V = h->infer_text ? c.num_text_tokens : c.num_audio_tokens;
  p.K = c.hidden_size; p.kslice = p.K / CS_HEADS; p.nrows = rpi * V; p.xraw = h->x;
  p.logits = h->logits; p.rows_per_item = rpi; p.V = V; p.hidden_out = h->hiddens_out;
  p.hidden_stride = h->max_new * c.hidden_size; p.final_norm_w = h->W + h->lay.final_norm;
  p.rows = h->engine ? h->rows : nullptr; p.want = h->phase;
  const int rc = launch_tc<DE_HEADS, CS_HEADS>(npad, h->infer_text ? h->m_htext : h->m_hcode, h->m_x[n][0], h->m_x[n][1], p, s);
  if (rc || !h->engine || !h->eng_text) return rc;
  p.nrows = c.num_text_tokens; p.logits = h->eng_text_logits; p.rows_per_item = 1; p.V = c.num_text_tokens;
  p.hidden_out = nullptr; p.want = h->phase | WANT_TEXT;
  return launch_tc<DE_HEADS, CS_HEADS>(npad, h->m_htext, h->m_x[n][0], h->m_x[n][1], p, s);
}

template <int BT>
static int launch_step_mega_t(const MegaP& mp, cudaStream_t s) {
  const size_t smem = (size_t)BT * KC * sizeof(float) + (size_t)MG_GW_FLOATS * sizeof(float);
  { int rc = ensure_smem_attr((const void*)k_step<BT>, (int)smem); if (rc) return rc; }
  cudaLaunchConfig_t cfg{};
  cfg.gridDim = dim3(g_num_sms); cfg.blockDim = dim3(MG_THREADS); cfg.dynamicSmemBytes = smem; cfg.stream = s;
  cudaLaunchAttribute attr[1];
  attr[0].id = cudaLaunchAttributeCooperative;
  attr[0].val.cooperative = 1;
  cfg.attrs = attr; cfg.numAttrs = 1;
  CTB_CUDA(cudaLaunchKernelEx(&cfg, k_step<BT>, mp));
  CTB_LAUNCH_CHECK();
  return CTB_OK;
}

static int launch_step_mega(ctb_gpt* h, int col, bool sample, cudaStream_t s) {
  const ctb_gpt_config& c = h->cfg;
  const ctb_gpt_layout& L = h->lay;
  MegaP m{};
  m.W = h->W; m.layer0 = L.layer0; m.layer_stride = L.layer_stride; m.o_wqkv = L.wqkv; m.o_wo = L.wo; m.o_wgu = L.wgate_up;
  m.o_wd = L.wdown; m.o_ln1 = L.ln1; m.o_ln2 = L.ln2; m.o_final_norm = L.final_norm;
  m.o_head = h->infer_text ? L.head_text : L.head_code; m.o_emb_code = L.emb_code; m.o_emb_text = L.emb_text;
  m.o_cos = L.rope_cos; m.o_sin = L.rope_sin;
  m.L = c.num_layers; m.d = c.hidden_size; m.I = c.intermediate_size; m.Hq = c.num_heads; m.Hkv = c.num_kv_heads;
  m.hd = c.head_dim; m.eps = c.rms_eps; m.scaling = 1.0f / sqrtf((float)c.head_dim);
  m.x = h->x; m.qbuf = h->qbuf; m.attn = h->attn; m.mlp = h->mlp; m.logits = h->logits; m.kv = h->kv; m.part = h->part;
  m.kv_layer_floats = h->kv_layer_elems; m.block_table = h->block_table; m.pages_per_row = h->pages_per_row;
  m.seq_len = h->seq_len; m.counter = h->counter; m.nsplit_max = h->nsplit_max; m.st = h->st; m.bar = h->bar;
  m.decode = col < 0; m.col = col < 0 ? 0 : col; m.T0 = h->T0; m.sample = sample ? 1 : 0;
  m.emb = h->emb; m.mask = h->mask; m.ids_out = h->ids_out; m.max_new = h->max_new; m.num_vq = c.num_vq;
  m.num_audio = c.num_audio_tokens; m.infer_text = h->infer_text; m.B = h->B;
  m.hidden_out = h->hiddens_out; m.hidden_stride = h->max_new * c.hidden_size;
  m.rows_per_item = h->infer_text ? 1 : c.num_vq; m.V = h->infer_text ? c.num_text_tokens : c.num_audio_tokens;
  m.trace = h->trace;
  CTB_CUDA(cudaMemsetAsync(h->bar, 0, sizeof(unsigned), s));
  switch (bt_for(h->B)) {
    case 1: return launch_step_mega_t<1>(m, s);
    case 2: return launch_step_mega_t<2>(m, s);
    case 4: return launch_step_mega_t<4>(m, s);
    default: return launch_step_mega_t<8>(m, s);
  }
}

template <int BT>
static int launch_step_flow_t(const FlowP& fp, cudaStream_t s) {
  const size_t smem = (size_t)FL_RING_BYTES + (size_t)BT * KC * sizeof(float);
  { int rc = ensure_smem_attr((const void*)k_flow<BT>, (int)smem); if (rc) return rc; }
  cudaLaunchConfig_t cfg{};
  cfg.gridDim = dim3(g_num_sms); cfg.blockDim = dim3(FL_LAUNCH_THREADS); cfg.dynamicSmemBytes = smem; cfg.stream = s;
  cudaLaunchAttribute attr[1];
  attr[0].id = cudaLaunchAttributeCooperative;
  attr[0].val.cooperative = 1;
  cfg.attrs = attr; cfg.numAttrs = 1;
  CTB_CUDA(cudaLaunchKernelEx(&cfg, k_flow<BT>, fp));
  CTB_LAUNCH_CHECK();
  return CTB_OK;
}

static bool flow_ink(const ctb_gpt* h);

static int launch_step_flow(ctb_gpt* h, int col, bool sample, cudaStream_t s, int nsteps = 0) {
  const ctb_gpt_config& c = h->cfg;
  const ctb_gpt_layout& L = h->lay;
  FlowP m{};
  m.W = h->W; m.layer0 = L.layer0; m.layer_stride = L.layer_stride; m.o_wqkv = L.wqkv; m.o_wo = L.wo; m.o_wgu = L.wgate_up;
  m.o_wd = L.wdown; m.o_ln1 = L.ln1; m.o_ln2 = L.ln2; m.o_final_norm = L.final_norm;
  m.o_head = h->infer_text ? L.head_text : L.head_code; m.o_emb_code = L.emb_code; m.o_emb_text = L.emb_text;
  m.o_cos = L.rope_cos; m.o_sin = L.rope_sin;
  m.L = c.num_layers; m.I = c.intermediate_size; m.Hq = c.num_heads; m.hd = c.head_dim; m.eps = c.rms_eps;
  m.scaling = 1.0f / sqrtf((float)c.head_dim);
  m.logits = h->logits; m.kv = h->kv; m.kv_layer_floats = h->kv_layer_elems; m.block_table = h->block_table;
  m.pages_per_row = h->pages_per_row; m.seq_len = h->seq_len; m.st = h->st;
  m.decode = col < 0; m.col = col < 0 ? 0 : col; m.T0 = h->T0; m.sample = sample ? 1 : 0;
  m.emb = h->emb; m.mask = h->mask; m.ids_out = h->ids_out; m.max_new = h->max_new; m.num_vq = c.num_vq;
  m.num_audio = c.num_audio_tokens; m.infer_text = h->infer_text; m.B = h->B;
  m.hidden_out = h->hiddens_out; m.hidden_stride = h->max_new * c.hidden_size;
  m.rows_per_item = h->infer_text ? 1 : c.num_vq; m.V = h->infer_text ? c.num_text_tokens : c.num_audio_tokens;
  m.arena = h->flow_arena; m.epoch = h->flow_epoch; m.R = h->flow_R; m.trace = h->trace;
  m.l2_ahead = h->flow_l2_ahead;
  m.ink = nsteps > 0 ? 1 : 0; m.nsteps = nsteps > 0 ? nsteps : 1; m.samp = h->sampler; m.q_noise = h->q_noise;
  m.finish = h->finish; m.end_idx = h->end_idx; m.ids_w = h->ids_out;
  switch (bt_for(h->B)) {
    case 1: return launch_step_flow_t<1>(m, s);
    case 2: return launch_step_flow_t<2>(m, s);
    default: return launch_step_flow_t<4>(m, s);
  }
}

static bool use_flow(const ctb_gpt* h) { return h->flow_ok && !h->engine && !h->use_tc && h->B <= h->flow_max_batch; }
static bool flow_ink(const ctb_gpt* h) {
  static const bool off = getenv("CTB_FLOW_NO_INK") != nullptr;
  return !off && use_flow(h) && !h->infer_text && h->B <= 2 && h->cfg.num_audio_tokens <= FL_VPAD &&
         h->B * h->cfg.num_vq <= FL_SROWS && h->cfg.num_vq <= 8;
}

static int launch_finalize(ctb_gpt* h, cudaStream_t s) {
  const ctb_gpt_config& c = h->cfg;
  FinalP fp{};
  fp.st = h->st; fp.B = h->B; fp.rows_per_item = h->infer_text ? 1 : c.num_vq; fp.num_vq = c.num_vq;
  fp.max_new = h->max_new; fp.eos = h->sampler.eos_token; fp.idx = h->idx; fp.ids_out = h->ids_out;
  fp.finish = h->finish; fp.end_idx = h->end_idx;
  if (h->engine) {
    fp.rows = h->rows; fp.want = h->phase; fp.idx_text = h->eng_text_idx;
    CTB_CUDA(launch_pdl(k_finalize_rows, dim3(1), dim3(256), 0, s, fp));
  } else {
    CTB_CUDA(launch_pdl(k_finalize, dim3(1), dim3(256), 0, s, fp));
  }
  CTB_LAUNCH_CHECK();
  return CTB_OK;
}

static int enqueue_step(ctb_gpt* h, int col, bool sample, cudaStream_t s) {
  const ctb_gpt_config& c = h->cfg;
  const ctb_gpt_layout& L = h->lay;
  const int decode = col < 0;
  int rc;

  if (use_flow(h) || (h->mega_ok && !h->engine && !h->use_tc && h->B <= h->mega_max_batch)) {
    if ((rc = use_flow(h) ? launch_step_flow(h, col, sample, s) : launch_step_mega(h, col, sample, s))) return rc;
    if (!sample) return CTB_OK;
    const StepCtx xm = make_ctx(h, decode);
    if ((rc = launch_sampler(h, xm, s))) return rc;
    FinalP fm{};
    fm.st = h->st; fm.B = h->B; fm.rows_per_item = h->infer_text ? 1 : c.num_vq; fm.num_vq = c.num_vq;
    fm.max_new = h->max_new; fm.eos = h->sampler.eos_token; fm.idx = h->idx; fm.ids_out = h->ids_out;
    fm.finish = h->finish; fm.end_idx = h->end_idx;
    CTB_CUDA(launch_pdl(k_finalize, dim3(1), dim3(256), 0, s, fm));
    CTB_LAUNCH_CHECK();
    return CTB_OK;
  }

  InputP ip{};
  ip.st = h->st; ip.decode = decode; ip.B = h->B; ip.d = c.hidden_size; ip.col = decode ? 0 : col; ip.T0 = h->T0;
  ip.emb = h->emb; ip.mask = h->mask;
  ip.emb_code = h->W + L.emb_code; ip.emb_text = h->W + L.emb_text;
  ip.ids_out = h->ids_out; ip.max_new = h->max_new; ip.num_vq = c.num_vq; ip.num_audio = c.num_audio_tokens;
  ip.infer_text = h->infer_text;
  ip.x = h->x; ip.seq_len = h->seq_len; ip.pos = h->pos; ip.active = h->active;
  ip.x_hi = h->use_tc ? h->x_hi : nullptr; ip.x_lo = h->use_tc ? h->x_lo : nullptr;
  ip.rows = h->engine ? h->rows : nullptr;
  CTB_CUDA(launch_pdl(k_input, dim3(h->B), dim3(256), 0, s, ip));
  CTB_LAUNCH_CHECK();

  const StepCtx x = make_ctx(h, decode);
  for (int l = 0; l < c.num_layers; ++l)
    for (int kind = 0; kind < 5; ++kind)
      if ((rc = (h->use_tc && kind != 1) ? launch_layer_kernel_tc(h, l, kind, s) : launch_layer_kernel(h, x, l, kind, s)))
        return rc;
  if (!sample) return CTB_OK;
  if ((rc = h->use_tc ? launch_heads_tc(h, s) : launch_heads(h, x, s))) return rc;
  if ((rc = launch_sampler(h, x, s))) return rc;
  return launch_finalize(h, s);
}

extern "C" int ctb_gpt_profile_kernel(ctb_gpt* h, int32_t kind, void* stream) {
  if (!h || !h->started) return set_err(CTB_ERR_STATE, "ctb_gpt_begin has not been called");
  cudaStream_t s = (cudaStream_t)stream;
  StepCtx x = make_ctx(h, 0);
  x.g.check_finished = 0; x.a.check_finished = 0;
  int rc;
  if (kind == 5) return h->use_tc ? launch_heads_tc(h, s) : launch_heads(h, x, s);
  if (kind == 6) return launch_sampler(h, x, s);
  if (kind == 8) {
    if (!flow_ink(h)) return set_err(CTB_ERR_STATE, "multi-step dataflow kernel unavailable for this handle/batch");
    if (h->steps_enqueued + 16 > h->max_new || h->T0 + h->steps_enqueued + 16 > h->cfg.max_context)
      return set_err(CTB_ERR_STATE, "no room for 16 more steps (max_new / max_context reached)");
    h->steps_enqueued += 16;
    return launch_step_flow(h, -1, true, s, 16);
  }
  if (kind == 7) {
    if (h->steps_enqueued >= h->max_new || h->T0 + h->steps_enqueued >= h->cfg.max_context)
      return set_err(CTB_ERR_STATE, "no room for another step (max_new / max_context reached)");
    h->steps_enqueued++;
    if (use_flow(h)) return launch_step_flow(h, -1, true, s, flow_ink(h) ? 1 : 0);
    if (!(h->mega_ok && h->B <= 8)) return set_err(CTB_ERR_STATE, "one-kernel step unavailable for this handle/batch");
    return launch_step_mega(h, -1, true, s);
  }
  for (int l = 0; l < h->cfg.num_layers; ++l)
    if ((rc = (h->use_tc && kind != 1) ? launch_layer_kernel_tc(h, l, kind, s) : launch_layer_kernel(h, x, l, kind, s)))
      return rc;
  return CTB_OK;
}

static int prefill_reserve(ctb_gpt* h, size_t rows) {
  const ctb_gpt_config& c = h->cfg;
  const size_t d = c.hidden_size, I = c.intermediate_size, nqkv = (size_t)(c.num_heads + 2 * c.num_kv_heads) * c.head_dim;
  int rc;
  if (!h->gw_hi && !(h->prec & CTB_ENGINE_FP16_WEIGHTS)) {
    const size_t n = (size_t)h->lay.layer_stride * c.num_layers;
    if ((rc = dalloc(&h->gw_hi, n))) return rc;
    if ((rc = dalloc(&h->gw_lo, n))) return rc;
    k_split_tf32_t<0><<<2048, 256>>>(h->W + h->lay.layer0, h->gw_hi, h->gw_lo, (int64_t)n);
    CTB_CUDA(cudaDeviceSynchronize());
  }
  if (!h->pf_ones) {
    if ((rc = dalloc(&h->pf_ones, 2 * I))) return rc;
    if ((rc = dalloc(&h->pf_zeros, 2 * I))) return rc;
    std::vector<float> ones(2 * I, 1.0f);
    CTB_CUDA(cudaMemcpy(h->pf_ones, ones.data(), ones.size() * sizeof(float), cudaMemcpyHostToDevice));
  }
  if (rows > h->pf_rows) {
    float** bufs[] = {&h->pf_resid, &h->pf_xn, &h->pf_qkv, &h->pf_q, &h->pf_attn, &h->pf_gu, &h->pf_h};
    for (float** b : bufs) if (*b) { cudaFree(*b); *b = nullptr; }
    if (h->pf_npre) { cudaFree(h->pf_npre); h->pf_npre = nullptr; }
    if (h->pf_nvalid) { cudaFree(h->pf_nvalid); h->pf_nvalid = nullptr; }
    if (h->pf_mask) { cudaFree(h->pf_mask); h->pf_mask = nullptr; }
    if ((rc = dalloc(&h->pf_resid, rows * d))) return rc;
    if ((rc = dalloc(&h->pf_xn, rows * d))) return rc;
    if ((rc = dalloc(&h->pf_qkv, rows * nqkv))) return rc;
    if ((rc = dalloc(&h->pf_q, rows * d))) return rc;
    if ((rc = dalloc(&h->pf_attn, rows * d))) return rc;
    if ((rc = dalloc(&h->pf_gu, rows * 2 * I))) return rc;
    if ((rc = dalloc(&h->pf_h, rows * I))) return rc;
    if ((rc = dalloc(&h->pf_npre, rows))) return rc;
    if ((rc = dalloc(&h->pf_nvalid, (size_t)std::max(h->cfg.max_batch, 2)))) return rc;
    if ((rc = dalloc(&h->pf_mask, rows))) return rc;
    h->pf_rows = rows;
  }
  return CTB_OK;
// ... 2 lines not shown
template <typename Attn>
static int prefill_layers(ctb_gpt* h, PrefillP& pp, Attn attn, cudaStream_t s) {
  const ctb_gpt_config& c = h->cfg;
  const ctb_gpt_layout& L = h->lay;
  const int B = pp.B, T0 = pp.T0, M = B * T0;
  const int d = c.hidden_size, I = c.intermediate_size, nqkv = (c.num_heads + 2 * c.num_kv_heads) * c.head_dim;
  int rc;
  pp.Hq = c.num_heads; pp.Hkv = c.num_kv_heads; pp.hd = c.head_dim; pp.d = d;
  pp.npre = h->pf_npre; pp.nvalid = h->pf_nvalid; pp.qkv = h->pf_qkv; pp.q = h->pf_q; pp.block_table = h->block_table;
  pp.pages_per_row = h->pages_per_row; pp.rope_cos = h->W + L.rope_cos; pp.rope_sin = h->W + L.rope_sin;
  pp.permute_qk = h->use_tc ? 1 : 0; pp.attn = h->pf_attn; pp.scaling = 1.0f / sqrtf((float)c.head_dim);
  const int rms_blocks = (M + 7) / 8;
  const bool w16 = (h->prec & CTB_ENGINE_FP16_WEIGHTS) != 0, kv16 = (h->prec & CTB_ENGINE_FP16_KV) != 0;
  for (int l = 0; l < c.num_layers; ++l) {
    const int64_t lo = (int64_t)l * L.layer_stride;
    const float* Wl = h->W + L.layer0 + lo;
    const float *Whi = (w16 ? h->gw16 : h->gw_hi) + lo, *Wlo = w16 ? nullptr : h->gw_lo + lo;
    auto wlo = [&](int64_t off) { return w16 ? h->pf_wzero : Wlo + off; };
    pp.kv = kv_layer(h, l);
    k_rms_rows<<<rms_blocks, 256, 0, s>>>(h->pf_resid, w16 ? h->pf_ones : Wl + L.ln1, h->pf_xn, M, d, c.rms_eps);
    CTB_LAUNCH_CHECK();
    if ((rc = tc_gemm_launch<GE_NONE>(s, h->pf_xn, d, B, T0, nqkv, d, 1, d, 1, 0, Whi + L.wqkv, wlo(L.wqkv), nullptr,
                                      nullptr, nullptr, 0, h->pf_qkv, nqkv))) return rc;
    if (kv16) k_prefill_rope_kv<__half><<<dim3(T0, B), 256, 0, s>>>(pp);
    else k_prefill_rope_kv<float><<<dim3(T0, B), 256, 0, s>>>(pp);
    CTB_LAUNCH_CHECK();
    attn(pp);
    CTB_LAUNCH_CHECK();
    if ((rc = tc_gemm_launch<GE_SCALE_RES>(s, h->pf_attn, d, B, T0, d, d, 1, d, 1, 0, Whi + L.wo, wlo(L.wo), h->pf_zeros,
                                           h->pf_ones, h->pf_resid, d, h->pf_resid, d))) return rc;
    k_rms_rows<<<rms_blocks, 256, 0, s>>>(h->pf_resid, w16 ? h->pf_ones : Wl + L.ln2, h->pf_xn, M, d, c.rms_eps);
    CTB_LAUNCH_CHECK();
    if ((rc = tc_gemm_launch<GE_NONE>(s, h->pf_xn, d, B, T0, 2 * I, d, 1, d, 1, 0, Whi + L.wgate_up, wlo(L.wgate_up),
                                      nullptr, nullptr, nullptr, 0, h->pf_gu, 2 * I))) return rc;
    k_silu_mul<<<(unsigned)(((size_t)M * I + 255) / 256), 256, 0, s>>>(h->pf_gu, h->pf_h, M, I);
    CTB_LAUNCH_CHECK();
    if ((rc = tc_gemm_launch<GE_SCALE_RES>(s, h->pf_h, I, B, T0, d, I, 1, I, 1, 0, Whi + L.wdown, wlo(L.wdown),
                                           h->pf_zeros, h->pf_ones, h->pf_resid, d, h->pf_resid, d))) return rc;
  }
  return CTB_OK;
}

static int prefill_first_token(ctb_gpt* h, int B, int T0, const int* nvalid, const int* slot, cudaStream_t s) {
  int rc;
  k_prefill_finish<<<B, 256, 0, s>>>(h->pf_resid, h->x, h->use_tc ? h->x_hi : nullptr, h->use_tc ? h->x_lo : nullptr,
                                     nvalid, h->seq_len, h->pos, h->active, T0, h->cfg.hidden_size, slot);
  CTB_LAUNCH_CHECK();
  const StepCtx x = make_ctx(h, 0);
  if ((rc = h->use_tc ? launch_heads_tc(h, s) : launch_heads(h, x, s))) return rc;
  if ((rc = launch_sampler(h, x, s))) return rc;
  return launch_finalize(h, s);
}

static int prefill(ctb_gpt* h, int B, int T, int q0, int n, const float* emb, const uint8_t* mask,
                   const int32_t* slots, cudaStream_t s) {
  const ctb_gpt_config& c = h->cfg;
  const int M = B * n;
  int rc;
  if ((rc = prefill_reserve(h, (size_t)M))) return rc;
  CTB_CUDA(cudaMemcpyAsync(h->pf_resid, emb, (size_t)M * c.hidden_size * sizeof(float), cudaMemcpyDeviceToDevice, s));
  if (mask) k_prefill_positions<<<B, 32, 0, s>>>(mask, h->pf_npre, h->pf_nvalid, T);
  else k_prefill_chunk_positions<<<(n + 255) / 256, 256, 0, s>>>(h->pf_mask, h->pf_npre, h->pf_nvalid, h->eng_slot,
                                                                 slots[0], q0, n);
  CTB_LAUNCH_CHECK();
  PrefillP pp{};
  pp.B = B; pp.T0 = n; pp.mask = mask ? mask : h->pf_mask; pp.slot = slots ? h->eng_slot : nullptr;
  const bool kv16 = (h->prec & CTB_ENGINE_FP16_KV) != 0, tiled = T > PF_ATT_MAX_T0;
  if (tiled &&
      (rc = kv16 ? ensure_smem_attr((const void*)k_prefill_attn_tiled<__half>, PftSmem<__half>::BYTES)
                 : ensure_smem_attr((const void*)k_prefill_attn_tiled<float>, PftSmem<float>::BYTES)))
    return rc;
  auto attn = [&](const PrefillP& p) {
    if (tiled) {
      const dim3 tgrid((n + PFT_TILE - 1) / PFT_TILE, c.num_heads, B);
      if (kv16) k_prefill_attn_tiled<__half><<<tgrid, PFT_THREADS, PftSmem<__half>::BYTES, s>>>(p, q0);
      else k_prefill_attn_tiled<float><<<tgrid, PFT_THREADS, PftSmem<float>::BYTES, s>>>(p, q0);
    } else {
      const dim3 agrid((n + PF_ATT_WARPS - 1) / PF_ATT_WARPS, c.num_heads, B);
      const size_t smem = (size_t)PF_ATT_WARPS * (q0 + n) * sizeof(float);
      if (kv16) k_prefill_attn<__half><<<agrid, PF_ATT_WARPS * 32, smem, s>>>(p, q0);
      else k_prefill_attn<float><<<agrid, PF_ATT_WARPS * 32, smem, s>>>(p, q0);
    }
  };
  if ((rc = prefill_layers(h, pp, attn, s))) return rc;
  if (q0 + n < T) return CTB_OK;
  return prefill_first_token(h, B, n, mask ? h->pf_nvalid : h->pf_nvalid + 1, pp.slot, s);
}

static int kv_reserve(ctb_gpt* h, int B, int tokens, cudaStream_t s) {
  const ctb_gpt_config& c = h->cfg;
  const size_t per_row = ((size_t)tokens + kPageTokens - 1) / kPageTokens;
  const size_t need = per_row * (size_t)B;
  const size_t page_elems = (size_t)2 * c.num_kv_heads * kPageTokens * c.head_dim;
  const size_t page_bytes = page_elems * kv_elem_bytes(h) * c.num_layers;
  if (need * page_bytes > h->kv_bytes) {
    CTB_CUDA(cudaStreamSynchronize(s));
    if (h->kv) { cudaFree(h->kv); h->kv = nullptr; h->kv_bytes = 0; }
    const size_t pages = need + need / 8;
    if (cudaMalloc(reinterpret_cast<void**>(&h->kv), pages * page_bytes) != cudaSuccess) {
      cudaGetLastError();
      return set_err(CTB_ERR_NOMEM, "KV pool: %zu pages x %d layers (%.1f GB) do not fit", pages, c.num_layers,
                     (double)(pages * page_bytes) / 1e9);
    }
    CTB_CUDA(cudaMemsetAsync(h->kv, 0, pages * page_bytes, s));
    h->kv_bytes = pages * page_bytes;
    h->bt_B = 0;
  }
  h->kv_layer_elems = h->kv_bytes / page_bytes * page_elems;
  if (h->bt_B == B && h->bt_per_row == per_row) return CTB_OK;
  std::vector<int> bt((size_t)B * h->pages_per_row, 0);
  for (int b = 0; b < B; ++b)
    for (size_t i = 0; i < per_row; ++i) bt[(size_t)b * h->pages_per_row + i] = (int)((size_t)b * per_row + i);
  CTB_CUDA(cudaMemcpyAsync(h->block_table, bt.data(), bt.size() * sizeof(int), cudaMemcpyHostToDevice, s));
  CTB_CUDA(cudaStreamSynchronize(s));
  h->bt_B = B; h->bt_per_row = per_row;
  return CTB_OK;
}

static int check_sampler(const ctb_sampler_config& sc) {
  if (sc.past_window > 31 || sc.past_window < 0) return set_err(CTB_ERR_ARG, "past_window out of range");
  if (sc.min_tokens_to_keep < 1) return set_err(CTB_ERR_ARG, "min_tokens_to_keep must be >= 1");
  return CTB_OK;
}

static int restart_decode(ctb_gpt* h, cudaStream_t s) {
  if (h->graph_exec) { cudaGraphExecDestroy(h->graph_exec); h->graph_exec = nullptr; }
  if (h->graph_exec_text) { cudaGraphExecDestroy(h->graph_exec_text); h->graph_exec_text = nullptr; }
  if (h->use_tc) {
    const size_t d = h->cfg.hidden_size, I = h->cfg.intermediate_size;
    float* z768[] = {h->x_hi, h->x_lo, h->attn_hi, h->attn_lo};
    for (float* zp : z768) CTB_CUDA(cudaMemsetAsync(zp, 0, h->tc_rows * d * sizeof(float), s));
    CTB_CUDA(cudaMemsetAsync(h->h_hi, 0, h->tc_rows * I * sizeof(float), s));
    CTB_CUDA(cudaMemsetAsync(h->h_lo, 0, h->tc_rows * I * sizeof(float), s));
  }
  return CTB_OK;
}

extern "C" int ctb_gpt_begin(ctb_gpt* h, int32_t B, int32_t T0, const float* emb_dev, const uint8_t* mask_dev,
                             const ctb_sampler_config* sampler, const float* q_noise_dev, int32_t max_new_token,
                             int32_t infer_text, int32_t* ids_out_dev, float* hiddens_out_dev, void* stream) {
  if (!h || !emb_dev || !mask_dev || !sampler || !ids_out_dev) return set_err(CTB_ERR_ARG, "null argument");
  if (B < 1 || B > h->cfg.max_batch) return set_err(CTB_ERR_ARG, "B=%d outside [1,%d]", B, h->cfg.max_batch);
  if (T0 < 1 || max_new_token < 1 || T0 + max_new_token > h->cfg.max_context)
    return set_err(CTB_ERR_ARG, "T0=%d + max_new=%d exceeds max_context=%d", T0, max_new_token, h->cfg.max_context);
  int rc;
  if ((rc = check_sampler(*sampler))) return rc;
  cudaStream_t s = (cudaStream_t)stream;
  h->B = B; h->T0 = T0; h->max_new = max_new_token; h->infer_text = infer_text ? 1 : 0;
  h->engine = 0; h->phase = RS_RUNNING; h->prec = 0; h->pg_pages = 0;
  h->use_tc = h->tc_ready && B >= h->tc_min_batch;
  h->sampler = *sampler; h->q_noise = q_noise_dev; h->emb = emb_dev; h->mask = mask_dev;
  h->ids_out = ids_out_dev; h->hiddens_out = hiddens_out_dev;
  if ((rc = restart_decode(h, s)) || (rc = kv_reserve(h, B, T0 + max_new_token, s))) return rc;
  CTB_CUDA(cudaMemsetAsync(h->st, 0, sizeof(LoopState), s));
  CTB_CUDA(cudaMemsetAsync(h->seq_len, 0, sizeof(int) * h->bpad_max, s));
  CTB_CUDA(cudaMemsetAsync(h->finish, 0, h->bpad_max, s));
  CTB_CUDA(cudaMemsetAsync(h->end_idx, 0, sizeof(int) * h->bpad_max, s));
  CTB_CUDA(cudaMemsetAsync(h->counter, 0, sizeof(int) * h->cfg.max_batch * h->cfg.num_heads, s));
  if (h->flow_ok) {
    static const unsigned e0 = FL_EPOCH_STEP;
    CTB_CUDA(cudaMemcpyAsync(h->flow_epoch, &e0, sizeof(e0), cudaMemcpyHostToDevice, s));
    CTB_CUDA(cudaMemsetAsync(h->flow_arena, 0, FL_ARENA_WORDS * sizeof(unsigned long long), s));
  }
  if (h->pf_enabled && T0 >= 8 && T0 <= 1024) {
    if ((rc = prefill(h, B, T0, 0, T0, emb_dev, mask_dev, nullptr, s))) return rc;
  } else {
    for (int col = 0; col < T0; ++col)
      if ((rc = enqueue_step(h, col, col == T0 - 1, s))) return rc;
  }
  h->started = 1;
  h->steps_enqueued = 1;
  return CTB_OK;
}

extern "C" int ctb_gpt_decode(ctb_gpt* h, int32_t n_steps, void* stream) {
  if (!h || !h->started) return set_err(CTB_ERR_STATE, "ctb_gpt_begin has not been called");
  cudaStream_t s = (cudaStream_t)stream;
  int rc;
  if (!h->engine) n_steps = std::min(n_steps, h->max_new - h->steps_enqueued);
  if (n_steps <= 0) return CTB_OK;
  if (h->pg_pages) {
    for (int b = 0; b < h->B; ++b)
      if (h->pg_hi[b] && h->pg_map[b] * kPageTokens < std::min(h->pg_hi[b] + n_steps, h->pg_cap[b]))
        return set_err(CTB_ERR_STATE, "slot %d: its pages hold %d positions, %d decode steps may need %d", b,
                       h->pg_map[b] * kPageTokens, n_steps, std::min(h->pg_hi[b] + n_steps, h->pg_cap[b]));
    for (int b = 0; b < h->B; ++b)
      if (h->pg_hi[b] && (rc = check_private(h, b, h->pg_hi[b], std::min(h->pg_hi[b] + n_steps, h->pg_cap[b]))))
        return rc;
    for (int b = 0; b < h->B; ++b)
      if (h->pg_hi[b]) h->pg_hi[b] = std::min(h->pg_hi[b] + n_steps, h->pg_cap[b]);
  }
  h->steps_enqueued += n_steps;
  if (flow_ink(h)) {
    const int per_launch = h->trace ? 1 : 64;
    for (int done = 0; done < n_steps; done += per_launch)
      if ((rc = launch_step_flow(h, -1, true, s, std::min(per_launch, n_steps - done)))) return rc;
    return CTB_OK;
  }
  cudaGraphExec_t& graph_exec = (h->engine && h->eng_text) ? h->graph_exec_text : h->graph_exec;
  uint64_t& graph_kernels = (h->engine && h->eng_text) ? h->graph_kernels_text : h->graph_kernels;
  if (h->use_graph && !graph_exec) {
    cudaGraph_t graph;
    if (!h->cap_stream) CTB_CUDA(cudaStreamCreateWithFlags(&h->cap_stream, cudaStreamNonBlocking));
    CTB_CUDA(cudaStreamBeginCapture(h->cap_stream, cudaStreamCaptureModeThreadLocal));
    const uint64_t before = g_launches.load();
    rc = enqueue_step(h, -1, true, h->cap_stream);
    graph_kernels = g_launches.load() - before;
    g_launches.store(before);
    cudaError_t e = cudaStreamEndCapture(h->cap_stream, &graph);
    if (rc) return rc;
    if (e != cudaSuccess) return set_err(CTB_ERR_CUDA, "graph capture failed: %s", cudaGetErrorString(e));
    CTB_CUDA(cudaGraphInstantiate(&graph_exec, graph, 0));
    cudaGraphDestroy(graph);
  }
  for (int i = 0; i < n_steps; ++i) {
    if (graph_exec) {
      CTB_CUDA(cudaGraphLaunch(graph_exec, s));
      g_launches.fetch_add(graph_kernels, std::memory_order_relaxed);
    } else if ((rc = enqueue_step(h, -1, true, s))) {
      return rc;
    }
  }
  return CTB_OK;
}

extern "C" int ctb_gpt_engine_begin(ctb_gpt* h, int32_t S, int32_t max_new_cap, int32_t* ids_out_dev,
                                    float* hiddens_out_dev, void* stream) {
  return ctb_gpt_engine_begin_ex(h, S, max_new_cap, 0, ids_out_dev, hiddens_out_dev, stream);
}

static_assert((int)TD_W16 == CTB_ENGINE_FP16_WEIGHTS && (int)TD_KV16 == CTB_ENGINE_FP16_KV, "precision bits");

static int kv_pool_paged(ctb_gpt* h, int S, int pool_pages, cudaStream_t s);

static int engine_begin(ctb_gpt* h, int32_t S, int32_t max_new_cap, int32_t flags, int32_t pool_pages,
                        int32_t* ids_out_dev, float* hiddens_out_dev, void* stream) {
  if (!h || !ids_out_dev) return set_err(CTB_ERR_ARG, "null argument");
  const ctb_gpt_config& c = h->cfg;
  if (S < 2 || S > c.max_batch) return set_err(CTB_ERR_ARG, "S=%d outside [2,%d]", S, c.max_batch);
  if (max_new_cap < 1 || max_new_cap >= c.max_context)
    return set_err(CTB_ERR_ARG, "max_new_cap=%d outside [1,%d)", max_new_cap, c.max_context);
  if (flags & ~(CTB_ENGINE_FP16_WEIGHTS | CTB_ENGINE_FP16_KV)) return set_err(CTB_ERR_ARG, "unknown engine flags 0x%x", flags);
  if (flags && S > 64) return set_err(CTB_ERR_ARG, "S=%d: a half-precision engine serves up to 64 slots", S);
  if (flags && getenv("CTB_GPT_FMA"))
    return set_err(CTB_ERR_ARG, "a half-precision engine runs on the wgmma step, which CTB_GPT_FMA=1 disables");
  cudaStream_t s = (cudaStream_t)stream;
  int rc;
  const bool use_tc = flags ? true : getenv("CTB_GPT_FMA") == nullptr && S >= h->tc_min_batch && S <= 64;
  if (use_tc) {
    if ((flags & CTB_ENGINE_FP16_WEIGHTS) ? (rc = fp16_setup(h)) : (!h->tc_wqkv && (rc = tc_setup(h)))) return rc;
    if ((flags & CTB_ENGINE_FP16_KV) && !(flags & CTB_ENGINE_FP16_WEIGHTS) &&
        (rc = set_tc_attr<DE_QKV, CS_QKV, CTB_ENGINE_FP16_KV>()))
      return rc;
  }
  if (!h->rows) {
    if ((rc = dalloc(&h->rows, (size_t)h->bpad_max))) return rc;
    if ((rc = dalloc(&h->cfgs, (size_t)c.max_batch))) return rc;
    if ((rc = dalloc(&h->eng_noise, (size_t)c.max_batch * noise_stride(h)))) return rc;
    if ((rc = dalloc(&h->eng_slot, (size_t)c.max_batch))) return rc;
    if ((rc = dalloc(&h->eng_text_logits, (size_t)c.max_batch * c.num_text_tokens))) return rc;
    if ((rc = dalloc(&h->eng_text_idx, (size_t)c.max_batch))) return rc;
  }
  h->engine = 1; h->phase = RS_RUNNING; h->prec = flags;
  h->B = S; h->T0 = 0; h->max_new = max_new_cap; h->infer_text = 0;
  h->use_tc = use_tc;
  h->q_noise = h->eng_noise; h->emb = nullptr; h->mask = nullptr;
  h->ids_out = ids_out_dev; h->hiddens_out = hiddens_out_dev; h->eng_text = 0; h->pg_pages = 0;
  if ((rc = restart_decode(h, s)) ||
      (rc = pool_pages ? kv_pool_paged(h, S, pool_pages, s) : kv_reserve(h, S, c.max_context, s)))
    return rc;
  static const LoopState idle_state = {0, 1, 0, 0, 0};
  CTB_CUDA(cudaMemcpyAsync(h->st, &idle_state, sizeof(LoopState), cudaMemcpyHostToDevice, s));
  CTB_CUDA(cudaMemsetAsync(h->rows, 0, sizeof(RowState) * h->bpad_max, s));
  CTB_CUDA(cudaMemsetAsync(h->seq_len, 0, sizeof(int) * h->bpad_max, s));
  CTB_CUDA(cudaMemsetAsync(h->pos, 0, sizeof(int) * h->bpad_max, s));
  CTB_CUDA(cudaMemsetAsync(h->active, 0, h->bpad_max, s));
  CTB_CUDA(cudaMemsetAsync(h->finish, 0, h->bpad_max, s));
  CTB_CUDA(cudaMemsetAsync(h->end_idx, 0, sizeof(int) * h->bpad_max, s));
  CTB_CUDA(cudaMemsetAsync(h->counter, 0, sizeof(int) * c.max_batch * c.num_heads, s));
  CTB_CUDA(cudaMemsetAsync(h->x, 0, sizeof(float) * h->bpad_max * c.hidden_size, s));
  CTB_CUDA(cudaStreamSynchronize(s));
  h->chunk_T0.assign((size_t)S, 0);
  h->chunk_done.assign((size_t)S, 0);
  h->pr_len.assign((size_t)S, 0);
  h->pr_W.assign((size_t)S, 0);
  h->started = 1;
  h->steps_enqueued = 0;
  return CTB_OK;
}

extern "C" int ctb_gpt_engine_begin_ex(ctb_gpt* h, int32_t S, int32_t max_new_cap, int32_t flags, int32_t* ids_out_dev,
                                       float* hiddens_out_dev, void* stream) {
  return engine_begin(h, S, max_new_cap, flags, 0, ids_out_dev, hiddens_out_dev, stream);
}

static int admit(ctb_gpt* h, int n, const int32_t* slots, int T0, int q0, const float* emb_dev, const uint8_t* mask_dev,
                 const ctb_sampler_config* samplers, const float* q_noise_dev, const int32_t* max_new, int text,
                 cudaStream_t s) {
  const ctb_gpt_config& c = h->cfg;
  const int S = h->B;
  int rc;
  std::vector<RowState> rows((size_t)h->bpad_max);
  CTB_CUDA(cudaMemcpyAsync(rows.data(), h->rows, sizeof(RowState) * rows.size(), cudaMemcpyDeviceToHost, s));
  std::vector<uint8_t> mask_h;
  if (mask_dev) {
    mask_h.resize((size_t)n * T0);
// ... 446 lines not shown
  int rc;
  if ((rc = check_paged(h)) || (rc = check_slot(h, slot)) || (rc = check_pinned(host_buf))) return rc;
  if (host_bytes < sizeof(ctb_slot_image)) return set_err(CTB_ERR_ARG, "image buffer of %llu bytes", (unsigned long long)host_bytes);
  const ctb_slot_image* img = static_cast<const ctb_slot_image*>(host_buf);
  RowState r;
  memcpy(&r, img->row, sizeof(r));
  ctb_slot_image want{};
  image_layout(h, img->n_gen, img->seq_len, &want);
  if (img->magic != want.magic || img->prec != want.prec || img->page_bytes != want.page_bytes ||
      img->num_vq != want.num_vq || img->hidden_size != want.hidden_size || img->noise_floats != want.noise_floats ||
      img->has_hidden != want.has_hidden || img->npages != want.npages || img->off_noise != want.off_noise ||
      img->off_ids != want.off_ids || img->off_hiddens != want.off_hiddens || img->off_kv != want.off_kv ||
      img->bytes != want.bytes || img->n_gen < 1 || img->seq_len < 1 || r.state != RS_RUNNING ||
      r.n_gen != img->n_gen || r.max_new > h->max_new)
    return set_err(CTB_ERR_ARG, "the buffer holds no slot image of this engine");
  if (host_bytes < img->bytes)
    return set_err(CTB_ERR_ARG, "image buffer of %llu bytes, the image has %llu", (unsigned long long)host_bytes,
                   (unsigned long long)img->bytes);
  if (img->npages > h->pg_map[slot])
    return set_err(CTB_ERR_STATE, "slot %d: its pages hold %d positions, the image %d", slot,
                   h->pg_map[slot] * kPageTokens, img->seq_len);
  RowState cur;
  CTB_CUDA(cudaMemcpyAsync(&cur, h->rows + slot, sizeof(RowState), cudaMemcpyDeviceToHost, s));
  CTB_CUDA(cudaStreamSynchronize(s));
  if (cur.state == RS_RUNNING || cur.state == RS_PENDING) return set_err(CTB_ERR_STATE, "slot %d is still generating", slot);
  if ((rc = check_private(h, slot, 0, img->seq_len))) return rc;
  h->pr_len[slot] = 0;
  const char* hb = static_cast<const char*>(host_buf);
  const int n_gen = img->n_gen;
  CTB_CUDA(cudaMemcpyAsync(h->cfgs + slot, &img->sampler, sizeof(ctb_sampler_config), cudaMemcpyHostToDevice, s));
  CTB_CUDA(cudaMemcpyAsync(h->eng_noise + slot * noise_stride(h), hb + img->off_noise, img->noise_floats * sizeof(float),
                           cudaMemcpyHostToDevice, s));
  CTB_CUDA(cudaMemcpyAsync(h->ids_out + (size_t)slot * h->max_new * c.num_vq, hb + img->off_ids,
                           (size_t)n_gen * c.num_vq * sizeof(int32_t), cudaMemcpyHostToDevice, s));
  if (img->has_hidden)
    CTB_CUDA(cudaMemcpyAsync(h->hiddens_out + (size_t)slot * h->max_new * c.hidden_size, hb + img->off_hiddens,
                             (size_t)n_gen * c.hidden_size * sizeof(float), cudaMemcpyHostToDevice, s));
  CTB_CUDA(cudaMemcpyAsync(h->seq_len + slot, &img->seq_len, sizeof(int), cudaMemcpyHostToDevice, s));
  CTB_CUDA(cudaMemcpyAsync(h->pos + slot, &img->pos, sizeof(int), cudaMemcpyHostToDevice, s));
  CTB_CUDA(cudaMemcpyAsync(h->end_idx + slot, &img->end_idx, sizeof(int), cudaMemcpyHostToDevice, s));
  CTB_CUDA(cudaMemsetAsync(h->finish + slot, img->finish ? 1 : 0, 1, s));
  if ((rc = kv_move(h, slot, const_cast<char*>(hb) + img->off_kv, img->npages, false, s)) ||
      (rc = launch_set_row(h, slot, r, s)))
    return rc;
  h->pg_hi[slot] = img->seq_len;
  h->pg_cap[slot] = img->seq_len + r.max_new - r.n_gen;
  if (r.text) h->eng_text = 1;
  return CTB_OK;
}

extern "C" int ctb_gpt_engine_share_prompt(ctb_gpt* h, int32_t src, int32_t dst, int32_t T0, int32_t c0, void* stream) {
  if (!h) return set_err(CTB_ERR_ARG, "null argument");
  if (!h->engine) return set_err(CTB_ERR_STATE, "ctb_gpt_engine_begin has not been called");
  const int S = h->B;
  if (src < 0 || src >= S || dst < 0 || dst >= S || src == dst)
    return set_err(CTB_ERR_ARG, "slots %d -> %d: two distinct slots of [0,%d)", src, dst, S);
  if (T0 < 8 || T0 > h->cfg.max_context - 1) return set_err(CTB_ERR_ARG, "T0=%d outside [8,%d]", T0, h->cfg.max_context - 1);
  if (c0 < CTB_PREFILL_CHUNK_ALIGN || c0 % CTB_PREFILL_CHUNK_ALIGN || c0 >= T0)
    return set_err(CTB_ERR_ARG, "c0=%d: a positive multiple of %d below T0=%d", c0, CTB_PREFILL_CHUNK_ALIGN, T0);
  cudaStream_t s = (cudaStream_t)stream;
  RowState rs, rd;
  CTB_CUDA(cudaMemcpyAsync(&rs, h->rows + src, sizeof(RowState), cudaMemcpyDeviceToHost, s));
  CTB_CUDA(cudaMemcpyAsync(&rd, h->rows + dst, sizeof(RowState), cudaMemcpyDeviceToHost, s));
  CTB_CUDA(cudaStreamSynchronize(s));
  if ((rs.state != RS_RUNNING && rs.state != RS_FINISHED) || h->pr_len[src] == 0)
    return set_err(CTB_ERR_STATE, "slot %d holds no admitted prompt (state %d)", src, rs.state);
  if (rd.state == RS_RUNNING || rd.state == RS_PENDING) return set_err(CTB_ERR_STATE, "slot %d is still generating", dst);
  if (h->chunk_T0[dst]) return set_err(CTB_ERR_STATE, "slot %d has a prompt in progress", dst);
  if (h->pg_pages && h->pg_map[dst]) return set_err(CTB_ERR_STATE, "slot %d has pages mapped", dst);
  if (h->pr_len[src] < c0)
    return set_err(CTB_ERR_STATE, "slot %d holds a prompt of %d positions, fewer than c0=%d", src, h->pr_len[src], c0);
  if ((T0 > PF_ATT_MAX_T0) != (h->pr_W[src] > PF_ATT_MAX_T0))
    return set_err(CTB_ERR_ARG, "T0=%d and slot %d's prompt width %d take different prefill attention kernels", T0, src,
                   h->pr_W[src]);
  const int shared = c0 / kPageTokens;
  int rc;
  if (h->pg_pages) {
    const int own = (T0 + kPageTokens - 1) / kPageTokens - shared;
    if ((size_t)own > h->pg_free.size())
      return set_err(CTB_ERR_POOL, "KV pool: %d more pages needed, %zu of %d free", own, h->pg_free.size(),
                     h->pg_pages - 1);
    std::vector<std::pair<int, int>> e;
    for (int k = 0; k < shared + own; ++k) {
      int page;
      if (k < shared) {
        page = h->pg_bt[(size_t)src * h->pages_per_row + k];
        ++h->pg_ref[page];
      } else {
        page = h->pg_free.back();
        h->pg_free.pop_back();
        h->pg_ref[page] = 1;
      }
      const int idx = dst * h->pages_per_row + k;
      h->pg_bt[idx] = page;
      e.emplace_back(idx, page);
    }
    h->pg_map[dst] = shared + own;
    if ((rc = bt_write(h, e, s))) return rc;
  } else {
    KvCopyP p{};
    p.kv = reinterpret_cast<char*>(h->kv); p.layer_bytes = h->kv_layer_elems * kv_elem_bytes(h);
    p.page_words = (int)(page_bytes(h) / 16); p.layers = h->cfg.num_layers; p.npages = shared;
    p.src0 = src * (int)h->bt_per_row; p.dst0 = dst * (int)h->bt_per_row;
    k_kv_copy<<<(unsigned)std::min(p.layers * shared, g_num_sms * 8), 256, 0, s>>>(p);
    CTB_LAUNCH_CHECK();
  }
  h->chunk_T0[dst] = T0; h->chunk_done[dst] = c0;
  h->pr_len[dst] = 0;
  return CTB_OK;
}

namespace ctb {
__global__ void k_embed_prompt(const int64_t* __restrict__ ids, const uint8_t* __restrict__ text_mask,
                               const float* __restrict__ emb_text, const float* __restrict__ emb_code, int num_vq,
                               int num_audio, int num_text, int d, float* __restrict__ out) {
  const size_t pos = blockIdx.x;
  const int64_t* id = ids + pos * num_vq;
  float* o = out + pos * d;
  if (text_mask[pos]) {
    const int64_t t = min(max(id[0], (int64_t)0), (int64_t)num_text - 1);
    const float* e = emb_text + (size_t)t * d;
    for (int k = threadIdx.x; k < d; k += blockDim.x) o[k] = e[k];
  } else {
    for (int k = threadIdx.x; k < d; k += blockDim.x) {
      float s = 0.f;
      for (int q = 0; q < num_vq; ++q) {
        const int64_t c = min(max(id[q], (int64_t)0), (int64_t)num_audio - 1);
        s += emb_code[((size_t)q * num_audio + c) * d + k];
      }
      o[k] = s;
    }
  }
}
}

extern "C" int ctb_gpt_embed_prompt(ctb_gpt* h, const int64_t* ids_dev, const uint8_t* text_mask_dev, int32_t B, int32_t T,
                                    float* out_dev, void* stream) {
  if (!h || !ids_dev || !text_mask_dev || !out_dev) return set_err(CTB_ERR_ARG, "null argument");
  if (B < 1 || T < 1) return set_err(CTB_ERR_ARG, "bad shape");
  const ctb_gpt_config& c = h->cfg;
  k_embed_prompt<<<(unsigned)((size_t)B * T), 256, 0, (cudaStream_t)stream>>>(
      ids_dev, text_mask_dev, h->W + h->lay.emb_text, h->W + h->lay.emb_code, c.num_vq, c.num_audio_tokens,
      c.num_text_tokens, c.hidden_size, out_dev);
  CTB_LAUNCH_CHECK();
  return CTB_OK;
}

extern "C" int ctb_gpt_debug_trace(ctb_gpt* h, unsigned long long* host_out, int n) {
  if (!h || !h->trace) return set_err(CTB_ERR_STATE, "trace disabled (set CTB_MEGA_TRACE=1 before ctb_gpt_create)");
  CTB_CUDA(cudaMemcpy(host_out, h->trace, sizeof(unsigned long long) * (size_t)std::min(n, FL_TR_WORDS), cudaMemcpyDeviceToHost));
  return CTB_OK;
}

extern "C" int ctb_gpt_status_query(ctb_gpt* h, ctb_gpt_status* out, int32_t* end_idx_host, uint8_t* finish_host,
                                    void* stream) {
  if (!h || !out) return set_err(CTB_ERR_ARG, "null argument");
  cudaStream_t s = (cudaStream_t)stream;
  LoopState st;
  CTB_CUDA(cudaMemcpyAsync(&st, h->st, sizeof(st), cudaMemcpyDeviceToHost, s));
  if (end_idx_host) CTB_CUDA(cudaMemcpyAsync(end_idx_host, h->end_idx, sizeof(int) * h->B, cudaMemcpyDeviceToHost, s));
  if (finish_host) CTB_CUDA(cudaMemcpyAsync(finish_host, h->finish, h->B, cudaMemcpyDeviceToHost, s));
  CTB_CUDA(cudaStreamSynchronize(s));
  if (st.err != 0)
    return set_err(CTB_ERR_STATE, "decode kernel reported error 0x%x (watchdog: a cross-CTA wait never completed)", st.err);
  out->steps_done = st.step;
  out->all_finished = st.all_finished;
  out->any_finished_first_step = st.any_first;
  out->reserved = 0;
  return CTB_OK;
}

extern "C" int ctb_sample(const float* logits_dev, int32_t rows, int32_t V, int32_t rows_per_item,
                          const ctb_sampler_config* sampler, const float* q_noise_dev, const int32_t* gen_ids_dev,
                          int32_t gen_stride, int32_t n_gen, int32_t step, int32_t* out_idx_dev, void* stream) {
  if (!logits_dev || !sampler || !out_idx_dev) return set_err(CTB_ERR_ARG, "null argument");
  if (rows < 1 || V < 1 || rows_per_item < 1 || rows % rows_per_item) return set_err(CTB_ERR_ARG, "bad shape");
  if ((size_t)V * 4 + 8192 > 200 * 1024) return set_err(CTB_ERR_ARG, "V=%d too large for the sampler", V);
  if (sampler->penalty_on && n_gen > 0 && !gen_ids_dev) return set_err(CTB_ERR_ARG, "gen_ids required");
  if (int rc = check_sampler(*sampler)) return rc;
  SampleP sp{};
  sp.st = nullptr; sp.check_finished = 0; sp.logits = logits_dev; sp.rows = rows; sp.V = V;
  sp.rows_per_item = rows_per_item; sp.cfg = *sampler; sp.q_noise = q_noise_dev; sp.gen_ids = gen_ids_dev;
  sp.gen_stride = gen_stride; sp.gen_inner = rows_per_item; sp.n_gen_fixed = n_gen; sp.step_fixed = step; sp.out_idx = out_idx_dev;
  return launch_sample(sp, (cudaStream_t)stream);
}
```

include/chattts_b200.h:

```cpp
#ifndef CHATTTS_B200_H
#define CHATTTS_B200_H

#include <stdint.h>

#ifdef __cplusplus
extern "C" {
#endif

#define CTB_OK 0
#define CTB_ERR_ARG (-1)
#define CTB_ERR_CUDA (-2)
#define CTB_ERR_STATE (-3)
#define CTB_ERR_NOMEM (-4)

#define CTB_ABI_VERSION 3

int ctb_abi_version(void);
const char* ctb_last_error(void);
uint64_t ctb_launch_count(void);


typedef struct ctb_gpt_config {
  int32_t hidden_size;
  int32_t intermediate_size;
  int32_t num_layers;
  int32_t num_heads;
  int32_t num_kv_heads;
  int32_t head_dim;
  int32_t num_vq;
  int32_t num_audio_tokens;
  int32_t num_text_tokens;
  int32_t max_positions;
  float rms_eps;
  int32_t max_batch;
  int32_t max_context;
} ctb_gpt_config;

typedef struct ctb_gpt_layout {
  int64_t layer0, layer_stride;
  int64_t wqkv;
  int64_t wo;
  int64_t wgate_up;
  int64_t wdown;
  int64_t ln1, ln2;
  int64_t final_norm;
  int64_t head_code;
  int64_t head_text;
  int64_t emb_code;
  int64_t emb_text;
  int64_t rope_cos;
  int64_t rope_sin;
  int64_t total;
} ctb_gpt_layout;

int ctb_gpt_layout_query(const ctb_gpt_config* cfg, ctb_gpt_layout* out);

typedef struct ctb_sampler_config {
  float temperature[8];
  float top_p;
  int32_t top_k;
  int32_t min_tokens_to_keep;
  int32_t penalty_on;
  float penalty_lut[32];
  int32_t past_window;
  int32_t penalty_max_ids;
  int32_t greedy;
  int32_t eos_token;
  int32_t min_new_token;
  float top_p_removed_max;
  int32_t has_removed_max;
  uint64_t philox_seed;
} ctb_sampler_config;

typedef struct ctb_gpt ctb_gpt;

int ctb_gpt_create(const ctb_gpt_config* cfg, const float* weights_dev, ctb_gpt** out);
int ctb_gpt_destroy(ctb_gpt* h);

int ctb_gpt_begin(ctb_gpt* h, int32_t B, int32_t T0, const float* emb_dev, const uint8_t* mask_dev,
                  const ctb_sampler_config* sampler, const float* q_noise_dev, int32_t max_new_token,
                  int32_t infer_text, int32_t* ids_out_dev, float* hiddens_out_dev, void* stream);

int ctb_gpt_decode(ctb_gpt* h, int32_t n_steps, void* stream);

typedef struct ctb_gpt_status {
  int32_t steps_done;
  int32_t all_finished;
  int32_t any_finished_first_step;
  int32_t reserved;
} ctb_gpt_status;

int ctb_gpt_status_query(ctb_gpt* h, ctb_gpt_status* out, int32_t* end_idx_host, uint8_t* finish_host,
                         void* stream);


#define CTB_SLOT_IDLE 0
#define CTB_SLOT_RUNNING 1
#define CTB_SLOT_FINISHED 2

int ctb_gpt_engine_begin(ctb_gpt* h, int32_t S, int32_t max_new_cap, int32_t* ids_out_dev, float* hiddens_out_dev,
                         void* stream);

#define CTB_ENGINE_FP16_WEIGHTS 1
#define CTB_ENGINE_FP16_KV 2
int ctb_gpt_engine_begin_ex(ctb_gpt* h, int32_t S, int32_t max_new_cap, int32_t flags, int32_t* ids_out_dev,
                            float* hiddens_out_dev, void* stream);

int ctb_gpt_engine_admit(ctb_gpt* h, int32_t n, const int32_t* slots, int32_t T0, const float* emb_dev,
                         const uint8_t* mask_dev, const ctb_sampler_config* samplers, const float* q_noise_dev,
                         const int32_t* max_new, void* stream);

int ctb_gpt_engine_admit_text(ctb_gpt* h, int32_t n, const int32_t* slots, int32_t T0, const float* emb_dev,
                              const uint8_t* mask_dev, const ctb_sampler_config* samplers, const float* q_noise_dev,
                              const int32_t* max_new, void* stream);

#define CTB_PREFILL_CHUNK_ALIGN 128
int ctb_gpt_engine_prefill_chunk(ctb_gpt* h, int32_t slot, int32_t T0, int32_t c0, int32_t n, const float* emb_dev,
                                 int32_t text, const ctb_sampler_config* sampler, const float* q_noise_dev,
                                 int32_t max_new, void* stream);

int ctb_gpt_engine_status(ctb_gpt* h, ctb_gpt_status* out, int32_t* state_host, int32_t* end_idx_host,
                          uint8_t* finish_host, void* stream);

int ctb_gpt_engine_cancel(ctb_gpt* h, int32_t n, const int32_t* slots, void* stream);

#define CTB_ERR_POOL (-5)
int ctb_gpt_engine_begin_paged(ctb_gpt* h, int32_t S, int32_t max_new_cap, int32_t flags, int32_t pool_pages,
                               int32_t* ids_out_dev, float* hiddens_out_dev, void* stream);

int ctb_gpt_engine_reserve(ctb_gpt* h, int32_t n, const int32_t* slots, const int32_t* tokens, void* stream);

int ctb_gpt_engine_release(ctb_gpt* h, int32_t n, const int32_t* slots, void* stream);

#define CTB_SLOT_IMAGE_MAGIC 0x4b565031u
typedef struct ctb_slot_image {
  uint32_t magic;
  int32_t prec;
  int32_t seq_len, pos, end_idx, finish;
  int32_t n_gen;
  int32_t npages;
  int32_t page_bytes;
  int32_t num_vq, hidden_size, noise_floats;
  int32_t has_hidden;
  int32_t row[8];
  int32_t reserved[3];
  ctb_sampler_config sampler;
  uint64_t off_noise;
  uint64_t off_ids;
  uint64_t off_hiddens;
  uint64_t off_kv;
  uint64_t bytes;
} ctb_slot_image;

int ctb_gpt_engine_suspend_bytes(ctb_gpt* h, int32_t slot, uint64_t* bytes, void* stream);

int ctb_gpt_engine_suspend(ctb_gpt* h, int32_t slot, void* host_buf, uint64_t host_bytes, void* stream);

int ctb_gpt_engine_resume(ctb_gpt* h, int32_t slot, const void* host_buf, uint64_t host_bytes, void* stream);

int ctb_gpt_engine_share_prompt(ctb_gpt* h, int32_t src, int32_t dst, int32_t T0, int32_t c0, void* stream);

int ctb_gpt_profile_kernel(ctb_gpt* h, int32_t kind, void* stream);

int ctb_gpt_debug_trace(ctb_gpt* h, unsigned long long* host_out, int n);

int ctb_gpt_embed_prompt(ctb_gpt* h, const int64_t* ids_dev, const uint8_t* text_mask_dev, int32_t B, int32_t T,
                         float* out_dev, void* stream);

int ctb_sample(const float* logits_dev, int32_t rows, int32_t V, int32_t rows_per_item,
               const ctb_sampler_config* sampler, const float* q_noise_dev, const int32_t* gen_ids_dev,
               int32_t gen_stride, int32_t n_gen, int32_t step, int32_t* out_idx_dev, void* stream);


typedef struct ctb_convstack_config {
  int32_t idim, odim, hidden, n_layer, bn_dim, kernel, dilation;
  int32_t out_dim;
  int32_t vq_dim, vq_groups, vq_residual;
  int32_t vq_levels;
} ctb_convstack_config;

typedef struct ctb_vocos_config {
  int32_t input_channels, dim, intermediate_dim, num_layers, n_fft, hop_length;
} ctb_vocos_config;

typedef struct ctb_decoder ctb_decoder;

int64_t ctb_dvae_blob_floats(const ctb_convstack_config* cfg);
int64_t ctb_vocos_blob_floats(const ctb_vocos_config* cfg);

int ctb_decoder_create(const ctb_convstack_config* dvae_cfg, const float* dvae_blob_dev,
                       const ctb_vocos_config* vocos_cfg, const float* vocos_blob_dev, int32_t max_batch,
                       int32_t max_tokens, ctb_decoder** out);
int ctb_decoder_destroy(ctb_decoder* h);

int ctb_dvae_decode(ctb_decoder* h, const void* in_dev, int32_t in_layout, int32_t B, int32_t T, float* mel_dev,
                    void* stream);
int ctb_vocos_decode(ctb_decoder* h, const float* mel_dev, int32_t B, int32_t F, float* wav_dev, void* stream);
int ctb_decode_rows(ctb_decoder* h, int32_t kind, int32_t B, const void* const* rows_dev, const int32_t* n_tokens,
                    float* wav_dev, int64_t wav_ld, void* stream);

typedef struct ctb_encoder ctb_encoder;
int64_t ctb_dvae_encoder_blob_floats(const ctb_convstack_config* enc_cfg);
int ctb_dvae_encoder_create(const ctb_convstack_config* enc_cfg, const float* blob_dev, int64_t max_samples,
                            ctb_encoder** out);
int ctb_dvae_encoder_destroy(ctb_encoder* h);
int ctb_dvae_encode(ctb_encoder* h, const float* wav_dev, int64_t n_samples, int32_t* ids_dev,
                    int32_t ids_capacity_tokens, int32_t* n_tokens_out, float* mel_dev, float* margin_dev, void* stream);
int ctb_dvae_encode_rows(ctb_encoder* h, int32_t B, const float* const* wavs_dev, const int64_t* n_samples,
                         int32_t* ids_dev, int32_t ids_ld, int32_t* n_tokens_out, float* margin_dev, void* stream);

#ifdef __cplusplus
}
#endif
#endif
```

Before: 2268.

## Fold RMSNorm weights into QKV and gate-up weights for flow kernel

Builds per-layer copies of the QKV and gate/up weights with the ln1/ln2 norm weights folded in, so the persistent flow kernel no longer fetches norm weights or applies elementwise normalization per layer. Only the row rsqrt scale is applied after the dot products. The QKV stage is restructured to process all of a warp's rows at once with batched accumulators and a single reduce-scatter, and task assignment is zig-zagged across warps for balance. This costs an extra folded weight copy in device memory, a one-time build step, and a change in rounding order.

After: 2293 (median of 6 runs). 1.01x the previous value.

```diff
diff --git a/chattts_b200/_lib.py b/chattts_b200/_lib.py
--- a/chattts_b200/_lib.py
+++ b/chattts_b200/_lib.py
@@ -80,7 +80,7 @@
 
 EXPORTS = (
     "ctb_abi_version", "ctb_last_error", "ctb_launch_count", "ctb_gpt_layout_query", "ctb_gpt_create",
-    "ctb_gpt_destroy", "ctb_gpt_begin", "ctb_gpt_decode", "ctb_gpt_status_query", "ctb_gpt_profile_kernel", "ctb_gpt_debug_trace", "ctb_gpt_embed_prompt", "ctb_sample",
+    "ctb_gpt_destroy", "ctb_gpt_begin", "ctb_gpt_decode", "ctb_gpt_status_query", "ctb_gpt_profile_kernel", "ctb_gpt_debug_trace", "ctb_gpt_debug_flow_weights", "ctb_gpt_embed_prompt", "ctb_sample",
     "ctb_gpt_engine_begin", "ctb_gpt_engine_admit", "ctb_gpt_engine_admit_text", "ctb_gpt_engine_status",
     "ctb_gpt_engine_cancel", "ctb_gpt_engine_begin_ex", "ctb_gpt_engine_prefill_chunk",
     "ctb_gpt_engine_begin_paged", "ctb_gpt_engine_reserve", "ctb_gpt_engine_release", "ctb_gpt_engine_suspend_bytes",
@@ -127,6 +127,7 @@
         lib.ctb_gpt_status_query.argtypes = [vp, C.POINTER(GptStatus), vp, vp, vp]
         lib.ctb_gpt_profile_kernel.argtypes = [vp, i32, vp]
         lib.ctb_gpt_debug_trace.argtypes = [vp, vp, i32]
+        lib.ctb_gpt_debug_flow_weights.argtypes = [vp, i32, vp, C.c_int64]
         lib.ctb_gpt_embed_prompt.argtypes = [vp, vp, vp, i32, i32, vp, vp]
         lib.ctb_gpt_engine_begin.argtypes = [vp, i32, i32, vp, vp, vp]
         lib.ctb_gpt_engine_begin_ex.argtypes = [vp, i32, i32, i32, vp, vp, vp]
diff --git a/chattts_b200/csrc/flow.cuh b/chattts_b200/csrc/flow.cuh
--- a/chattts_b200/csrc/flow.cuh
+++ b/chattts_b200/csrc/flow.cuh
@@ -44,8 +44,9 @@
 
 struct FlowP {
   const float* W;
-  int64_t layer0, layer_stride, o_wqkv, o_wo, o_wgu, o_wd, o_ln1, o_ln2, o_final_norm, o_head, o_emb_code, o_emb_text,
-      o_cos, o_sin;
+  int64_t layer0, layer_stride, o_wo, o_wd, o_final_norm, o_head, o_emb_code, o_emb_text, o_cos, o_sin;
+  const float* Wf;
+  int64_t f_stride, f_gu;
   int L, I, Hq, hd;
   float eps, scaling;
   float *logits, *kv;
@@ -130,7 +131,8 @@
   int nheads_tasks;
 };
 
-__device__ __forceinline__ bool fl_q_valid(const FlowGeo& g, int j) { return g.gw + j * g.NW < 3 * KC / 2; }
+__device__ __forceinline__ int fl_q_task(const FlowGeo& g, int j) { return j * g.NW + ((j & 1) ? g.NW - 1 - g.gw : g.gw); }
+__device__ __forceinline__ bool fl_q_valid(const FlowGeo& g, int j) { return fl_q_task(g, j) < 3 * KC / 2; }
 __device__ __forceinline__ bool fl_kv_more(const FlowGeo& g, int sub, int& chunk) {
   chunk = g.u_split + sub * g.S;
   return g.u_on && chunk < g.u_nchunk;
@@ -155,6 +157,7 @@
 }
 
 constexpr int FL_TMAX = 40;
+enum FlowTaskKind { FK_W = 0, FK_KV = 1, FK_FOLD = 2 };
 struct FlowIss {
   int l, k, n, ntab, hsub;
 };
@@ -170,8 +173,8 @@
   for (int j = 0; j < FL_QR; ++j)
     if (fl_q_valid(g, j)) {
       int r0, r1;
-      fl_qkv_rows(p, g.gw + j * g.NW, r0, r1);
-      put(p.o_wqkv + (int64_t)r0 * KC, (int64_t)(r1 - r0) * KC, KC * 4, 2, 0);
+      fl_qkv_rows(p, fl_q_task(g, j), r0, r1);
+      put((int64_t)r0 * KC, (int64_t)(r1 - r0) * KC, KC * 4, 2, FK_FOLD);
     }
   for (int sub = 0;; ++sub) {
     int chunk;
@@ -181,16 +184,16 @@
     const int page = __ldg(p.block_table + g.u_b * p.pages_per_row + t0 / kPageTokens);
     const int64_t k0 = (int64_t)kv_off(page, 0, g.u_h, t0 % kPageTokens, p.Hq, p.hd);
     const int64_t v0 = (int64_t)kv_off(page, 1, g.u_h, t0 % kPageTokens, p.Hq, p.hd);
-    put(k0, v0 - k0, 8 * 64 * 4, 2, 1);
-  }
-  if (fl_o_valid(g)) put(p.o_wo + (int64_t)(g.cta + g.G * g.warp) * KC, 0, KC * 4, 1, 0);
+    put(k0, v0 - k0, 8 * 64 * 4, 2, FK_KV);
+  }
+  if (fl_o_valid(g)) put(p.o_wo + (int64_t)(g.cta + g.G * g.warp) * KC, 0, KC * 4, 1, FK_W);
   for (int j = 0; j < FL_GU; ++j)
-    if (fl_gu_valid(g, j, p.I)) put(p.o_wgu + (int64_t)(g.gw + j * g.NW) * KC, (int64_t)p.I * KC, KC * 4, 2, 0);
+    if (fl_gu_valid(g, j, p.I)) put(p.f_gu + (int64_t)(g.gw + j * g.NW) * KC, (int64_t)p.I * KC, KC * 4, 2, FK_FOLD);
   for (int half = 0; half < 2; ++half) {
     const int j0 = half ? 4 : 0, j1 = half ? FL_ROWS : 4;
     const int nr = fl_d_rows(g, j0, j1);
     if (nr > 0)
-      put(p.o_wd + (int64_t)(g.cta + g.G * j0) * p.I + g.warp * (p.I / FL_WARPS), (int64_t)g.G * p.I, (p.I / FL_WARPS) * 4, nr, 0);
+      put(p.o_wd + (int64_t)(g.cta + g.G * j0) * p.I + g.warp * (p.I / FL_WARPS), (int64_t)g.G * p.I, (p.I / FL_WARPS) * 4, nr, FK_W);
   }
   return n;
 }
@@ -213,13 +216,15 @@
     const int4 e = tab[it.k];
     if (fl_elect()) {
       const int bytes = e.z & 0xffff, ncopy = (e.z >> 16) & 0xf, kind = e.z >> 20;
-      const float* src = (kind ? p.kv + (size_t)it.l * p.kv_layer_floats : p.W + p.layer0 + (int64_t)it.l * p.layer_stride) + e.x;
+      const int64_t lstride = kind == FK_FOLD ? p.f_stride : p.layer_stride;
+      const float* src = (kind == FK_KV ? p.kv + (size_t)it.l * p.kv_layer_floats
+                                        : (kind == FK_FOLD ? p.Wf : p.W + p.layer0) + (int64_t)it.l * lstride) + e.x;
       fl_expect(bar, (uint32_t)(bytes * ncopy));
 #pragma unroll
       for (int k = 0; k < 4; ++k)
-        if (k < ncopy) fl_bulk(dst + k * bytes, src + (int64_t)k * e.y, (uint32_t)bytes, bar, kind ? pol_kv : pol_w);
-      if (p.l2_ahead && kind == 0) {
-        const float* nsrc = it.l + 1 < p.L ? src + p.layer_stride : src - (int64_t)(p.L - 1) * p.layer_stride;
+        if (k < ncopy) fl_bulk(dst + k * bytes, src + (int64_t)k * e.y, (uint32_t)bytes, bar, kind == FK_KV ? pol_kv : pol_w);
+      if (p.l2_ahead && kind != FK_KV) {
+        const float* nsrc = it.l + 1 < p.L ? src + lstride : src - (int64_t)(p.L - 1) * lstride;
 #pragma unroll
         for (int k = 0; k < 4; ++k)
           if (k < ncopy)
@@ -409,15 +414,33 @@
   }
 }
 
+__device__ __forceinline__ float fl_rinv(float ss, float eps) {
+  return __fdiv_rn(1.0f, __fsqrt_rn(__fadd_rn(__fdiv_rn(ss, (float)KC), eps)));
+}
+template <int BT>
+__device__ __forceinline__ void fl_row_rinv(const float (&x)[BT][24], float eps, float (&rinv)[BT]) {
+#pragma unroll
+  for (int b = 0; b < BT; ++b) {
+    float s4[4] = {0.f, 0.f, 0.f, 0.f};
+#pragma unroll
+    for (int j = 0; j < 24; ++j) s4[j & 3] = fmaf(x[b][j], x[b][j], s4[j & 3]);
+    rinv[b] = fl_rinv(warp_sum((s4[0] + s4[1]) + (s4[2] + s4[3])), eps);
+  }
+}
+template <int BT>
+__device__ __forceinline__ float fl_pick(const float (&v)[BT], int b) {
+  float r = v[0];
+#pragma unroll
+  for (int k = 1; k < BT; ++k) r = b == k ? v[k] : r;
+  return r;
+}
 template <int BT>
 __device__ __forceinline__ void fl_norm(float (&x)[BT][24], const float4 (&nw)[6], float eps) {
+  float ri[BT];
+  fl_row_rinv<BT>(x, eps, ri);
 #pragma unroll
   for (int b = 0; b < BT; ++b) {
-    float s4[4] = {0.f, 0.f, 0.f, 0.f};
-#pragma unroll
-    for (int j = 0; j < 24; ++j) s4[j & 3] = fmaf(x[b][j], x[b][j], s4[j & 3]);
-    float ss = warp_sum((s4[0] + s4[1]) + (s4[2] + s4[3]));
-    const float rinv = __fdiv_rn(1.0f, __fsqrt_rn(__fadd_rn(__fdiv_rn(ss, (float)KC), eps)));
+    const float rinv = ri[b];
 #pragma unroll
     for (int i = 0; i < 6; ++i) {
       x[b][4 * i] = __fmul_rn(nw[i].x, __fmul_rn(x[b][4 * i], rinv));
@@ -443,10 +466,6 @@
 __device__ __forceinline__ void fl_load_nw_s(const float* s_nw, float4 (&nw)[6], int lane) {
 #pragma unroll
   for (int i = 0; i < 6; ++i) nw[i] = reinterpret_cast<const float4*>(s_nw)[i * 32 + lane];
-}
-__device__ __forceinline__ void fl_load_nw(const float* normw, float4 (&nw)[6], int lane) {
-#pragma unroll
-  for (int i = 0; i < 6; ++i) nw[i] = ldg_stream(reinterpret_cast<const float4*>(normw) + i * 32 + lane);
 }
 
 template <int BT>
@@ -749,7 +768,7 @@
   extern __shared__ __align__(128) unsigned char fl_smem[];
   float* xs = reinterpret_cast<float*>(fl_smem + FL_RING_BYTES);
   __shared__ __align__(8) uint64_t s_bar[FL_WARPS * FL_SLOTS];
-  __shared__ __align__(8) uint64_t s_nwbar[2];
+  __shared__ __align__(8) uint64_t s_nwbar;
   __shared__ int s_pos[BT], s_active[BT], s_page[BT];
   __shared__ float s_cos[BT * 64], s_sin[BT * 64];
   __shared__ float s_red[FL_ROWS][FL_WARPS][BT];
@@ -757,7 +776,7 @@
   __shared__ float s_am[FL_WARPS], s_al[FL_WARPS];
   __shared__ __align__(16) float s_ao[FL_WARPS][64];
   __shared__ FlowGeo s_geo;
-  __shared__ __align__(16) float s_nw1[KC], s_nw2[KC];
+  __shared__ __align__(16) float s_nw[KC];
   __shared__ int4 s_tab[FL_WARPS][FL_TMAX];
   __shared__ FlowSamp s_samp_store[BT <= 2 ? 1 : 0 + (BT > 2)];
   FlowSamp& s_samp = s_samp_store[0];
@@ -765,7 +784,7 @@
   const int tid = threadIdx.x, lane = tid & 31, warp = tid >> 5;
   constexpr int LPB = 32 / BT;
   if (tid < FL_WARPS * FL_SLOTS) mbar_init(&s_bar[tid], 1);
-  if (tid < 2) mbar_init(&s_nwbar[tid], 1);
+  if (tid == 0) mbar_init(&s_nwbar, 1);
   asm volatile("fence.mbarrier_init.release.cluster;" ::: "memory");
   __syncthreads();
   pdl_trigger();
@@ -801,7 +820,7 @@
   uint64_t pol_w, pol_kv;
   asm volatile("createpolicy.fractional.L2::evict_first.b64 %0, 1.0;" : "=l"(pol_w));
   asm volatile("createpolicy.fractional.L2::evict_normal.b64 %0, 1.0;" : "=l"(pol_kv));
-  int nw1_cnt = 0, nw2_cnt = 0;
+  int nw_cnt = 0;
   FlowW fw;
   fw.base = reinterpret_cast<float*>(fl_smem) + (size_t)warp * FL_SLOTS * FL_SLOT_FLOATS;
   fw.ring = smem_u32(fw.base);
@@ -859,8 +878,6 @@
 #pragma unroll 1
   for (int sidx = 0;; ++sidx) {
   FL_TRACE();
-  fl_nw_fetch(s_nw1, p.W + p.layer0 + p.o_ln1, &s_nwbar[0], pol_w);
-  fl_nw_fetch(s_nw2, p.W + p.layer0 + p.o_ln2, &s_nwbar[1], pol_w);
   {
     float ev[BT * 3][8];
 #pragma unroll
@@ -896,7 +913,6 @@
   FL_TRACE();
 
   for (int l = 0; l < p.L; ++l) {
-    const float* Wl = p.W + p.layer0 + (int64_t)l * p.layer_stride;
     unsigned long long* par = p.arena + (size_t)(l & 1) * FL_PARITY_WORDS;
     unsigned long long* parn = p.arena + (size_t)((l + 1) & 1) * FL_PARITY_WORDS;
     unsigned long long* qkvw = par + (size_t)FL_RMAX * FL_REP_STRIDE;
@@ -904,55 +920,82 @@
     const uint32_t tagl = base + 8u * (uint32_t)l;
 
     {
-      float4 nw[6];
       FL_EV(0);
-      fl_nw_wait(&s_nwbar[0], nw1_cnt, wd);
-      const bool q_rdy = fl_ring_peek_n(p, fw, 1);
+      int nqt = 0;
+#pragma unroll
+      for (int j = 0; j < FL_QR; ++j) nqt += fl_q_valid(g, j) ? 1 : 0;
+      const bool q_rdy = fl_ring_peek_n(p, fw, nqt);
       if (l > 0) fl_stage768<BT>(p, myr + FL_A_X, tagl + FT_X, xs, wd, fw);
       else fl_bar();
       FL_EV(1);
+      FL_CK(24);
       fl_refill_all(p, fw);
-      fl_load_nw_s(s_nw1, nw, lane);
+      FL_CK(25);
       float x[BT][24];
       fl_load_x<BT>(xs, x, lane);
-      float res_o = 0.f;
-      if (fl_o_valid(g)) res_o = xs[(lane / LPB) * KC + o_row];
-      fl_norm<BT>(x, nw, p.eps);
-      float res_keep = res_o;
-#pragma unroll 1
-      for (int j = 0; j < FL_QR; ++j) {
-        if (!fl_q_valid(g, j)) continue;
-        if (!(j == 0 && q_rdy)) fl_ring_wait_n(p, fw, 1, wd);
-        const float* slot = fl_ring_slot_at(fw, 0);
+      float res_keep = 0.f;
+      if (fl_o_valid(g)) res_keep = xs[(lane / LPB) * KC + o_row];
+      FL_CK(26);
+      if (nqt > 0) {
+        const float4* sl[FL_QR];
+#pragma unroll
+        for (int j = 0; j < FL_QR; ++j) sl[j] = reinterpret_cast<const float4*>(fl_ring_slot_at(fw, j)) + lane;
+        if (!q_rdy) fl_ring_wait_n(p, fw, nqt, wd);
         FL_EV(2);
-        float a0[BT], a1[BT];
-        fl_dot2<BT>(slot, x, a0, a1, lane);
-        warp_reduce_scatter<BT>(a0);
-        warp_reduce_scatter<BT>(a1);
-        const int b = lane / LPB;
-        if ((lane % LPB) == 0 && b < p.B && s_active[b]) {
+        FL_CK(27);
+        float acc[4 * BT];
+#pragma unroll
+        for (int k = 0; k < 4 * BT; ++k) acc[k] = 0.f;
+#pragma unroll
+        for (int i = 0; i < 6; ++i) {
+#pragma unroll
+          for (int j = 0; j < FL_QR; ++j)
+            if (j < nqt) {
+              const float4 u = sl[j][i * 32], v = sl[j][KC / 4 + i * 32];
+#pragma unroll
+              for (int b = 0; b < BT; ++b) {
+                float& a0 = acc[(2 * j) * BT + b];
+                float& a1 = acc[(2 * j + 1) * BT + b];
+                a0 = fmaf(u.x, x[b][4 * i], a0); a0 = fmaf(u.y, x[b][4 * i + 1], a0);
+                a0 = fmaf(u.z, x[b][4 * i + 2], a0); a0 = fmaf(u.w, x[b][4 * i + 3], a0);
+                a1 = fmaf(v.x, x[b][4 * i], a1); a1 = fmaf(v.y, x[b][4 * i + 1], a1);
+                a1 = fmaf(v.z, x[b][4 * i + 2], a1); a1 = fmaf(v.w, x[b][4 * i + 3], a1);
+              }
+            }
+        }
+        float ri[BT];
+        fl_row_rinv<BT>(x, p.eps, ri);
+        FL_CK(28);
+        warp_reduce_scatter<4 * BT>(acc);
+        FL_CK(29);
+        constexpr int LPV = 32 / (4 * BT);
+        const int gl = lane & 15, b = (gl / LPV) % BT, base16 = lane & ~15, j = lane >> 4;
+        const float rinv = fl_pick<BT>(ri, b);
+        const float v0 = __fmul_rn(__shfl_sync(0xffffffffu, acc[0], base16 + b * LPV), rinv);
+        const float v1 = __fmul_rn(__shfl_sync(0xffffffffu, acc[0], base16 + BT * LPV + b * LPV), rinv);
+        if (j < nqt && (gl % LPV) == 0 && b < p.B && s_active[b]) {
           const int half = p.hd / 2, nq = p.Hq * half;
-          int t = g.gw + j * g.NW, which = 0;
+          int t = fl_q_task(g, j), which = 0;
           if (t >= 2 * nq) { which = 2; t -= 2 * nq; }
           else if (t >= nq) { which = 1; t -= nq; }
           const int h = t / half, jj = t % half;
-          const float v0 = a0[0], v1 = a1[0];
-          float o0 = v0, o1 = v1;
+          const bool second = gl >= BT * LPV;
+          float o = second ? v1 : v0;
           if (which < 2) {
             const float* cs = s_cos + b * 64;
             const float* sn = s_sin + b * 64;
-            o0 = __fadd_rn(__fmul_rn(v0, cs[jj]), __fmul_rn(-v1, sn[jj]));
-            o1 = __fadd_rn(__fmul_rn(v1, cs[jj + half]), __fmul_rn(v0, sn[jj + half]));
-          }
+            o = second ? __fadd_rn(__fmul_rn(v1, cs[jj + half]), __fmul_rn(v0, sn[jj + half]))
+                       : __fadd_rn(__fmul_rn(v0, cs[jj]), __fmul_rn(-v1, sn[jj]));
+          }
+          const int e = second ? jj + half : jj;
           unsigned long long* dst = qkvw + (which == 0 ? FL_A_Q : which == 1 ? FL_A_KN : FL_A_VN) + b * KC + h * 64;
-          ll_st(dst + jj, o0, tagl + FT_QKV);
-          ll_st(dst + jj + half, o1, tagl + FT_QKV);
-          if (which > 0) {
-            float* kd = p.kv + (size_t)l * p.kv_layer_floats + kv_off(s_page[b], which - 1, h, s_pos[b] % kPageTokens, p.Hq, p.hd);
-            kd[jj] = o0; kd[jj + half] = o1;
-          }
-        }
-        fl_ring_release(p, fw);
+          ll_st(dst + e, o, tagl + FT_QKV);
+          if (which > 0)
+            p.kv[(size_t)l * p.kv_layer_floats + kv_off(s_page[b], which - 1, h, s_pos[b] % kPageTokens, p.Hq, p.hd) + e] = o;
+        }
+        FL_CK(30);
+        for (int k = 0; k < nqt; ++k) fl_ring_release(p, fw);
+        FL_CK(31);
       }
       FL_TRACE();
       FL_EV(3);
@@ -1101,7 +1144,7 @@
       FL_EV(5);
 
       fl_bar();
-      if (l + 1 < p.L || p.sample) fl_nw_fetch(s_nw1, l + 1 < p.L ? Wl + p.layer_stride + p.o_ln1 : p.W + p.o_final_norm, &s_nwbar[0], pol_w);
+      if (l + 1 == p.L && p.sample) fl_nw_fetch(s_nw, p.W + p.o_final_norm, &s_nwbar, pol_w);
       const bool o_rdy = fl_o_valid(g) ? fl_ring_peek_n(p, fw, 1) : true;
       fl_stage_attn<BT>(p, myr + FL_A_P, tagl + FT_P, xs, wd, g.S, s_pos, s_active);
       fl_refill_all(p, fw);
@@ -1123,8 +1166,6 @@
     }
 
     {
-      float4 nw[6];
-      fl_nw_wait(&s_nwbar[1], nw2_cnt, wd);
       int ngu = 0;
 #pragma unroll
       for (int j = 0; j < FL_GU; ++j) ngu += fl_gu_valid(g, j, p.I) ? 1 : 0;
@@ -1133,7 +1174,6 @@
       FL_CK(8);
       fl_stage768<BT>(p, myr + FL_A_XO, tagl + FT_XO, xs, wd, fw);
       fl_refill_all(p, fw);
-      fl_load_nw_s(s_nw2, nw, lane);
       FL_EV(9);
       FL_CK(9);
       if (tid < FL_ROWS * BT) {
@@ -1143,8 +1183,6 @@
       float x[BT][24];
       fl_load_x<BT>(xs, x, lane);
       FL_CK(10);
-      fl_norm<BT>(x, nw, p.eps);
-      FL_CK(11);
       {
         FL_CK(0);
         const float4* sl[FL_GU];
@@ -1173,13 +1211,16 @@
               }
             }
         }
+        float ri[BT];
+        fl_row_rinv<BT>(x, p.eps, ri);
         FL_CK(2);
         warp_reduce_scatter<8 * BT>(acc);
         FL_CK(3);
         constexpr int LPV = 32 / (8 * BT);
         const int gl = lane & 7, b = (gl / LPV) % BT, base8 = lane & ~7;
-        const float gv = __shfl_sync(0xffffffffu, acc[0], base8 + b * LPV);
-        const float uv = __shfl_sync(0xffffffffu, acc[0], base8 + BT * LPV + b * LPV);
+        const float rinv = fl_pick<BT>(ri, b);
+        const float gv = __fmul_rn(__shfl_sync(0xffffffffu, acc[0], base8 + b * LPV), rinv);
+        const float uv = __fmul_rn(__shfl_sync(0xffffffffu, acc[0], base8 + BT * LPV + b * LPV), rinv);
         if ((lane >> 3) < ngu && b < p.B) {
           const float sg = __fdiv_rn(gv, __fadd_rn(1.0f, expf(-gv)));
           const float act = __fmul_rn(sg, uv);
@@ -1273,7 +1314,6 @@
       }
       FL_EV(12);
       fl_bar();
-      if (l + 1 < p.L) fl_nw_fetch(s_nw2, Wl + p.layer_stride + p.o_ln2, &s_nwbar[1], pol_w);
       if (tid < FL_ROWS * BT * 8) {
         const int e = tid >> 3, b = e % BT, j = e / BT, row = g.cta + g.G * j;
         if (row < KC && b < p.B) {
@@ -1294,11 +1334,11 @@
   if (p.sample) {
     const unsigned long long* myr = p.arena + (size_t)(p.L & 1) * FL_PARITY_WORDS + (size_t)myrep * FL_REP_STRIDE;
     float4 nw[6];
-    fl_nw_wait(&s_nwbar[0], nw1_cnt, wd);
+    fl_nw_wait(&s_nwbar, nw_cnt, wd);
     fl_bar();
     fl_stage768<BT>(p, myr + FL_A_X, base + 8u * (uint32_t)p.L + FT_X, xs, wd, fw);
     fl_refill_all(p, fw);
-    fl_load_nw_s(s_nw1, nw, lane);
+    fl_load_nw_s(s_nw, nw, lane);
     float x[BT][24];
     fl_load_x<BT>(xs, x, lane);
     fl_norm<BT>(x, nw, p.eps);
diff --git a/chattts_b200/csrc/gpt_api.cu b/chattts_b200/csrc/gpt_api.cu
--- a/chattts_b200/csrc/gpt_api.cu
+++ b/chattts_b200/csrc/gpt_api.cu
@@ -83,6 +83,7 @@
   int flow_max_batch;
   unsigned long long* flow_arena;
   unsigned* flow_epoch;
+  float* flow_w;
   int steps_enqueued;
   float *tc_wqkv, *tc_wgu, *tc_heads_code, *tc_heads_text;
   float *x_hi, *x_lo, *attn_hi, *attn_lo, *h_hi, *h_lo;
@@ -465,7 +466,7 @@
   if (h->cap_stream) cudaStreamDestroy(h->cap_stream);
   void* ptrs[] = {h->x, h->qbuf, h->attn, h->mlp, h->logits, h->kv, h->part, h->block_table, h->seq_len,
                   h->pos, h->counter, h->end_idx, h->idx, h->active, h->finish, h->st, h->tc_wqkv, h->tc_wgu,
-                  h->tc_heads_code, h->tc_heads_text, h->x_hi, h->x_lo, h->attn_hi, h->attn_lo, h->h_hi, h->h_lo, h->bar, h->trace, h->flow_arena, h->flow_epoch, h->gw_hi, h->gw_lo, h->pf_resid, h->pf_xn, h->pf_qkv, h->pf_q,
+                  h->tc_heads_code, h->tc_heads_text, h->x_hi, h->x_lo, h->attn_hi, h->attn_lo, h->h_hi, h->h_lo, h->bar, h->trace, h->flow_arena, h->flow_epoch, h->flow_w, h->gw_hi, h->gw_lo, h->pf_resid, h->pf_xn, h->pf_qkv, h->pf_q,
                   h->pf_attn, h->pf_gu, h->pf_h, h->pf_ones, h->pf_zeros, h->pf_npre, h->pf_nvalid,
                   h->pf_mask, h->rows, h->cfgs, h->eng_noise, h->eng_slot, h->eng_text_logits, h->eng_text_idx,
                   h->pg_stage};
@@ -814,12 +815,43 @@
 
 static bool flow_ink(const ctb_gpt* h);
 
+static size_t flow_w_stride(const ctb_gpt_config& c) {
+  return (size_t)((c.num_heads + 2 * c.num_kv_heads) * c.head_dim + 2 * c.intermediate_size) * c.hidden_size;
+}
+static size_t flow_w_gu(const ctb_gpt_config& c) {
+  return (size_t)(c.num_heads + 2 * c.num_kv_heads) * c.head_dim * c.hidden_size;
+}
+
+static int flow_setup(ctb_gpt* h) {
+  if (h->flow_w) return CTB_OK;
+  const ctb_gpt_config& c = h->cfg;
+  const ctb_gpt_layout& L = h->lay;
+  const size_t d = c.hidden_size, nqkv = (size_t)(c.num_heads + 2 * c.num_kv_heads) * c.head_dim;
+  const size_t rows_gu = 2 * (size_t)c.intermediate_size;
+  int rc;
+  if ((rc = dalloc(&h->flow_w, flow_w_stride(c) * c.num_layers))) {
+    if (h->flow_w) { cudaFree(h->flow_w); h->flow_w = nullptr; }
+    return rc;
+  }
+  for (int l = 0; l < c.num_layers; ++l) {
+    const float* Wl = h->W + L.layer0 + (int64_t)l * L.layer_stride;
+    float* fl = h->flow_w + (size_t)l * flow_w_stride(c);
+    k_build_tc_weight<<<(unsigned)nqkv, 256>>>(Wl + L.wqkv, Wl + L.ln1, fl, (int)nqkv, (int)d, 0, 0, 0, 0);
+    k_build_tc_weight<<<(unsigned)rows_gu, 256>>>(Wl + L.wgate_up, Wl + L.ln2, fl + flow_w_gu(c), (int)rows_gu, (int)d, 0, 0,
+                                                 0, 0);
+  }
+  CTB_CUDA(cudaDeviceSynchronize());
+  return CTB_OK;
+}
+
 static int launch_step_flow(ctb_gpt* h, int col, bool sample, cudaStream_t s, int nsteps = 0) {
   const ctb_gpt_config& c = h->cfg;
   const ctb_gpt_layout& L = h->lay;
+  if (!h->flow_w) return set_err(CTB_ERR_STATE, "k_flow's norm-folded weights were not built");
   FlowP m{};
-  m.W = h->W; m.layer0 = L.layer0; m.layer_stride = L.layer_stride; m.o_wqkv = L.wqkv; m.o_wo = L.wo; m.o_wgu = L.wgate_up;
-  m.o_wd = L.wdown; m.o_ln1 = L.ln1; m.o_ln2 = L.ln2; m.o_final_norm = L.final_norm;
+  m.W = h->W; m.layer0 = L.layer0; m.layer_stride = L.layer_stride; m.o_wo = L.wo; m.o_wd = L.wdown;
+  m.o_final_norm = L.final_norm;
+  m.Wf = h->flow_w; m.f_stride = (int64_t)flow_w_stride(c); m.f_gu = (int64_t)flow_w_gu(c);
   m.o_head = h->infer_text ? L.head_text : L.head_code; m.o_emb_code = L.emb_code; m.o_emb_text = L.emb_text;
   m.o_cos = L.rope_cos; m.o_sin = L.rope_sin;
   m.L = c.num_layers; m.I = c.intermediate_size; m.Hq = c.num_heads; m.hd = c.head_dim; m.eps = c.rms_eps;
@@ -1128,6 +1160,7 @@
   h->sampler = *sampler; h->q_noise = q_noise_dev; h->emb = emb_dev; h->mask = mask_dev;
   h->ids_out = ids_out_dev; h->hiddens_out = hiddens_out_dev;
   if ((rc = restart_decode(h, s)) || (rc = kv_reserve(h, B, T0 + max_new_token, s))) return rc;
+  if (use_flow(h) && (rc = flow_setup(h))) return rc;
   CTB_CUDA(cudaMemsetAsync(h->st, 0, sizeof(LoopState), s));
   CTB_CUDA(cudaMemsetAsync(h->seq_len, 0, sizeof(int) * h->bpad_max, s));
   CTB_CUDA(cudaMemsetAsync(h->finish, 0, h->bpad_max, s));
@@ -1880,6 +1913,16 @@
   return CTB_OK;
 }
 
+extern "C" int ctb_gpt_debug_flow_weights(ctb_gpt* h, int32_t layer, float* host_out, int64_t n) {
+  if (!h || !host_out || n < 0) return set_err(CTB_ERR_ARG, "bad argument");
+  if (layer < 0 || layer >= h->cfg.num_layers) return set_err(CTB_ERR_ARG, "layer %d outside [0,%d)", layer, h->cfg.num_layers);
+  if (!h->flow_w) return set_err(CTB_ERR_STATE, "k_flow's norm-folded weights were not built");
+  const size_t stride = flow_w_stride(h->cfg);
+  CTB_CUDA(cudaMemcpy(host_out, h->flow_w + (size_t)layer * stride, sizeof(float) * std::min((size_t)n, stride),
+                      cudaMemcpyDeviceToHost));
+  return CTB_OK;
+}
+
 extern "C" int ctb_gpt_status_query(ctb_gpt* h, ctb_gpt_status* out, int32_t* end_idx_host, uint8_t* finish_host,
                                     void* stream) {
   if (!h || !out) return set_err(CTB_ERR_ARG, "null argument");
diff --git a/include/chattts_b200.h b/include/chattts_b200.h
--- a/include/chattts_b200.h
+++ b/include/chattts_b200.h
@@ -164,6 +164,8 @@
 
 int ctb_gpt_debug_trace(ctb_gpt* h, unsigned long long* host_out, int n);
 
+int ctb_gpt_debug_flow_weights(ctb_gpt* h, int32_t layer, float* host_out, int64_t n);
+
 int ctb_gpt_embed_prompt(ctb_gpt* h, const int64_t* ids_dev, const uint8_t* text_mask_dev, int32_t B, int32_t T,
                          float* out_dev, void* stream);
 
```
